# rrahn/libspm

Measured on AMD Instinct MI355X. Metric: Gbases/s scanned, Myers k<=3 |P|=100, higher is better.
Workload: dtype u32

## Files before the change

### include/spm_hip.h

```cpp
#ifndef SPM_HIP_H
#define SPM_HIP_H

#include <stddef.h>
#include <stdint.h>

#ifdef __cplusplus
extern "C" {
#endif

typedef struct spm_ctx spm_ctx;
typedef struct spm_text spm_text;
typedef struct spm_patterns spm_patterns;
typedef struct spm_hits spm_hits;
typedef struct spm_jst spm_jst;
typedef struct spm_jst_hits spm_jst_hits;

enum spm_status {
    SPM_OK = 0,
    SPM_E_INVALID = -1,
    SPM_E_HIP = -2,
    SPM_E_NOMEM = -3,
    SPM_E_UNSUPPORTED = -4,
    SPM_E_OVERFLOW = -5,
    SPM_E_PEER = -6
};

enum spm_algo {
    SPM_ALGO_SHIFTOR = 0,
    SPM_ALGO_MYERS = 1,
    SPM_ALGO_MYERS_PREFIX = 2,
    SPM_ALGO_HORSPOOL = 3
};

enum spm_engine {
    SPM_ENGINE_AUTO = 0,
    SPM_ENGINE_BRUTE = 1,
    SPM_ENGINE_FILTER = 2
};

#define SPM_MAX_NEEDLE 2048u

typedef struct spm_hit {
    uint64_t pos;
    uint32_t pattern;
    int32_t score;
} spm_hit;

typedef struct spm_scan_opts {
    uint32_t engine;
    uint32_t left_context;
    uint64_t pos_offset;
    uint64_t max_hits;
    uint32_t flags;
    uint32_t reserved;
} spm_scan_opts;

#define SPM_SCAN_IGNORE_PACKED 1u
#define SPM_SCAN_DEFER 2u
#define SPM_SCAN_ALIGNABLE 4u

typedef struct spm_scan_stats {
    float ms_total;
    float ms_main;
    float ms_verify;
    uint32_t engine_used;
    uint32_t fell_back;
    uint64_t n_candidates;
    uint64_t n_hits;
    uint32_t main_launches;
    uint32_t n_bands;
    uint32_t fallback_spans;
    uint32_t span_symbols;
    uint64_t fallback_symbols;
} spm_scan_stats;

int spm_hip_init(int device, void *stream, spm_ctx **out);
void spm_hip_destroy(spm_ctx *ctx);
const char *spm_hip_last_error(const spm_ctx *ctx);
int spm_hip_synchronize(spm_ctx *ctx);

int spm_hip_text_upload(spm_ctx *ctx, const uint8_t *ranks, uint64_t n, uint32_t sigma, spm_text **out);
int spm_hip_text_wrap(spm_ctx *ctx, const void *device_ranks, uint64_t n, uint32_t sigma, spm_text **out);
int spm_hip_text_generate(spm_ctx *ctx, uint64_t seed, uint64_t global_begin, uint64_t n, spm_text **out);
int spm_hip_text_generate_repeats(spm_ctx *ctx, uint64_t seed, uint64_t global_begin, uint64_t n, uint32_t repeat_ppm,
                                  spm_text **out);
int spm_hip_text_pack(spm_ctx *ctx, spm_text *text);
int spm_hip_text_is_packed(const spm_text *text);
int spm_hip_text_download(spm_ctx *ctx, const spm_text *text, uint64_t begin, uint64_t n, uint8_t *out);
uint64_t spm_hip_text_length(const spm_text *text);
const void *spm_hip_text_device_ptr(const spm_text *text);
void spm_hip_text_destroy(spm_text *text);

int spm_hip_patterns_create(spm_ctx *ctx, int algo, const uint8_t *ranks_concat, const uint32_t *offsets,
                            uint32_t n_patterns, const uint16_t *k, uint32_t sigma, spm_patterns **out);
void spm_hip_patterns_destroy(spm_patterns *p);
uint64_t spm_hip_patterns_window_size(const spm_patterns *p, uint32_t pattern);
int spm_hip_patterns_filterable(const spm_patterns *p);

int spm_hip_patterns_create_stranded(spm_ctx *ctx, int algo, const uint8_t *ranks_concat, const uint32_t *offsets,
                                     uint32_t n_reads, const uint16_t *k, uint32_t sigma, spm_patterns **out);
uint32_t spm_hip_patterns_strands(const spm_patterns *p);
uint32_t spm_hip_patterns_count(const spm_patterns *p);
int spm_hip_patterns_needle(const spm_patterns *p, uint32_t pattern, uint8_t *out, uint32_t cap, uint32_t *len);

typedef struct spm_build_stats {
    float ms_total;
    float ms_tables;
    float ms_index;
    float ms_upload;
    uint32_t threads;
    uint32_t passes;
    uint32_t dense;
    uint32_t anchor_sixteenths;
    uint64_t keys;
    uint32_t stride, key_len;
    uint64_t bytes_device;
} spm_build_stats;
int spm_hip_patterns_build_stats(const spm_patterns *p, spm_build_stats *out);

size_t spm_hip_patterns_state_stride(const spm_patterns *p);
int spm_hip_patterns_state_init(const spm_patterns *p, void *state);

int spm_hip_scan(spm_ctx *ctx, const spm_text *text, uint64_t begin, uint64_t end, const spm_patterns *patterns,
                 const spm_scan_opts *opts, const void *state_in, void *state_out, spm_hits **out);

int spm_hip_scan_segments(spm_ctx *ctx, const spm_text *text, const uint64_t *seg_offsets, uint64_t n_segments,
                          const spm_patterns *patterns, const spm_scan_opts *opts, spm_hits **out);

int spm_hip_hits_view(spm_hits *hits, const spm_hit **records, uint64_t *n);
int spm_hip_hits_device(spm_hits *hits, const void **device_records, uint64_t *n);
int spm_hip_hits_copy_device(spm_hits *hits, void *device_dst, uint64_t cap, uint64_t *n);
int spm_hip_hits_copy_fused(spm_hits *hits, void *device_dst, uint64_t cap, uint64_t *n);
int spm_hip_hits_copy_fused_device(spm_hits *hits, void *device_dst, uint64_t cap);
int spm_hip_hits_stats(const spm_hits *hits, spm_scan_stats *out);
uint64_t spm_hip_hits_checksum(spm_hits *hits);
void spm_hip_hits_destroy(spm_hits *hits);

typedef struct spm_aln {
    uint64_t begin;
    uint64_t end;
    uint32_t pattern;
    int32_t score;
    uint32_t cigar_off;
    uint32_t cigar_len;
} spm_aln;
typedef struct spm_alns spm_alns;

enum spm_cigar_op { SPM_CIGAR_INS = 1, SPM_CIGAR_DEL = 2, SPM_CIGAR_EQ = 7, SPM_CIGAR_X = 8 };
#define SPM_ALIGN_BEGIN_ONLY 1u

typedef struct spm_align_stats {
    float ms_total;
    float ms_begin;
    float ms_cigar;
    float ms_host;
    uint64_t n_alns;
    uint64_t n_ops;
    uint32_t begin_lane;
    uint32_t begin_wave;
    uint32_t cigar_lane;
    uint32_t cigar_wave;
    uint32_t cigar_wave_global;
    uint32_t reserved[3];
} spm_align_stats;

int spm_hip_hits_align(spm_hits *hits, uint32_t flags, spm_alns **out);
int spm_hip_alns_view(spm_alns *a, const spm_aln **records, uint64_t *n, const uint32_t **ops, uint64_t *n_ops);
int spm_hip_alns_device(spm_alns *a, const void **records, uint64_t *n, const void **ops, uint64_t *n_ops);
int spm_hip_alns_stats(const spm_alns *a, spm_align_stats *out);
void spm_hip_alns_destroy(spm_alns *a);

#define SPM_SELECT_LOCI 1u
#define SPM_SELECT_BEST 2u
#define SPM_SELECT_STRANDS 8u
#define SPM_SELECT_WINDOW_K 0xFFFFFFFFu
typedef struct spm_select_opts {
    uint32_t flags;
    uint32_t window;
    uint32_t strata;
    uint32_t reserved;
} spm_select_opts;
typedef struct spm_select_stats {
    float ms_total;
    float ms_order;
    float ms_select;
    float ms_host;
    uint64_t n_in;
    uint64_t n_loci;
    uint64_t n_out;
    uint32_t key_bits;
    uint32_t reserved;
} spm_select_stats;
int spm_hip_hits_select(spm_hits *hits, const spm_select_opts *opts, spm_hits **out);
int spm_hip_records_select(spm_ctx *ctx, const void *device_records, uint64_t n, const spm_patterns *patterns,
                           const spm_select_opts *opts, spm_hits **out);
int spm_hip_hits_select_stats(const spm_hits *hits, spm_select_stats *out);

typedef struct spm_jst_allele {
    uint64_t pos;
    uint32_t ref_len;
    uint32_t alt_len;
    uint64_t alt_off;
} spm_jst_allele;

typedef struct spm_jst_hit {
    uint64_t pos;
    uint32_t haplotype;
    uint32_t pattern;
    int32_t score;
    uint32_t reserved;
} spm_jst_hit;

typedef struct spm_jst_stats {
    uint64_t haplotype_symbols;
    uint64_t context_symbols;
    uint64_t contexts;
    uint64_t unique_contexts;
    uint64_t n_blocks;
    uint32_t block_len;
    uint32_t window;
    float ms_index;
    float ms_scan;
    float ms_main;
    float ms_verify;
    float ms_fanout;
    uint32_t engine_used;
    uint32_t main_launches;
    uint32_t fell_back;
    uint64_t segment_hits;
    uint64_t candidates;
    uint64_t bands;
} spm_jst_stats;

int spm_hip_jst_create(spm_ctx *ctx, const spm_text *reference, const spm_jst_allele *alleles, uint64_t n_alleles,
                       const uint8_t *alt_pool, uint64_t alt_pool_len, const uint64_t *coverage,
                       uint32_t n_haplotypes, spm_jst **out);
void spm_hip_jst_destroy(spm_jst *jst);
uint64_t spm_hip_jst_haplotype_length(const spm_jst *jst, uint32_t haplotype);
int spm_hip_jst_extract(spm_jst *jst, uint32_t haplotype, uint64_t begin, uint64_t n, uint8_t *out);
int spm_hip_jst_index(spm_jst *jst, uint32_t window, uint32_t block_len, uint64_t block_begin, uint64_t block_end);
int spm_hip_jst_search(spm_jst *jst, const spm_patterns *patterns, const spm_scan_opts *opts, spm_jst_hits **out);
int spm_hip_jst_stats(const spm_jst *jst, spm_jst_stats *out);
int spm_hip_jst_hits_view(spm_jst_hits *hits, const spm_jst_hit **records, uint64_t *n);
int spm_hip_jst_hits_device(spm_jst_hits *hits, const void **device_records, uint64_t *n);
int spm_hip_jst_hits_copy_device(spm_jst_hits *hits, void *device_dst, uint64_t cap, uint64_t *n);
void spm_hip_jst_hits_destroy(spm_jst_hits *hits);

typedef struct spm_jst_aln {
    uint64_t begin;
    uint64_t end;
    uint32_t haplotype;
    uint32_t pattern;
    int32_t score;
    uint32_t cigar_off;
    uint32_t cigar_len;
    uint32_t reserved;
} spm_jst_aln;
typedef struct spm_jst_alns spm_jst_alns;

typedef struct spm_jst_align_stats {
    float ms_total;
    float ms_begin;
    float ms_cigar;
    float ms_fanout;
    float ms_host;
    float ms_worklist;
    uint64_t n_alns;
    uint64_t n_segment_alns;
    uint64_t n_ops;
    uint32_t begin_lane, begin_wave, cigar_lane, cigar_wave, cigar_wave_global;
    uint32_t reserved[3];
} spm_jst_align_stats;

int spm_hip_jst_hits_align(spm_jst_hits *hits, uint32_t flags, spm_jst_alns **out);
int spm_hip_jst_alns_view(spm_jst_alns *a, const spm_jst_aln **records, uint64_t *n, const uint32_t **ops, uint64_t *n_ops);
int spm_hip_jst_alns_device(spm_jst_alns *a, const void **records, uint64_t *n, const void **ops, uint64_t *n_ops);
int spm_hip_jst_alns_stats(const spm_jst_alns *a, spm_jst_align_stats *out);
void spm_hip_jst_alns_destroy(spm_jst_alns *a);

int spm_hip_jst_selection_align(spm_jst_hits *selection, uint32_t flags, spm_jst_alns **out);

typedef struct spm_jst_ref_aln {
    uint64_t ref_begin;
    uint64_t ref_end;
    uint32_t haplotype;
    uint32_t pattern;
    int32_t score;
// ... 183 lines not shown
```

### libspm_amd/capi.py

```python
from __future__ import annotations

import ctypes as C
import os
import subprocess

_PKG = os.path.dirname(os.path.abspath(__file__))
SO_PATH = os.path.join(_PKG, "libspm_hip.so")
CSRC = os.path.join(_PKG, "csrc")

ALGO_SHIFTOR, ALGO_MYERS, ALGO_MYERS_PREFIX, ALGO_HORSPOOL = 0, 1, 2, 3
ENGINE_AUTO, ENGINE_BRUTE, ENGINE_FILTER = 0, 1, 2
SCAN_IGNORE_PACKED = 1
SCAN_DEFER = 2
SCAN_ALIGNABLE = 4
MAX_NEEDLE = 2048


class SpmError(RuntimeError):
    pass


class Hit(C.Structure):
    _fields_ = [("pos", C.c_uint64), ("pattern", C.c_uint32), ("score", C.c_int32)]

# ... 163 lines not shown
        ("n_members", C.c_uint64),
        ("n_ops", C.c_uint64),
        ("n_multi_slot", C.c_uint64),
        ("max_run", C.c_uint64),
    ]


class JstRead(C.Structure):
    _fields_ = [("first_locus", C.c_uint32), ("n_loci", C.c_uint32), ("n_forward", C.c_uint32), ("primary", C.c_uint32),
                ("best", C.c_int32), ("best_ref_score", C.c_int32), ("n_best", C.c_uint32), ("n_next", C.c_uint32)]


class JstReadsStats(C.Structure):
    _fields_ = [
        ("ms_total", C.c_float),
        ("ms_host", C.c_float),
        ("n_reads", C.c_uint64),
        ("n_loci", C.c_uint64),
        ("n_mapped", C.c_uint64),
        ("n_unique", C.c_uint64),
        ("n_multi", C.c_uint64),
    ]


class JstPairOpts(C.Structure):
    _fields_ = [("min_tlen", C.c_uint32), ("max_tlen", C.c_uint32), ("flags", C.c_uint32), ("reserved", C.c_uint32)]


class JstPair(C.Structure):
    _fields_ = [("locus1", C.c_uint32), ("locus2", C.c_uint32), ("tlen", C.c_int32), ("best", C.c_int32),
                ("n_pairs", C.c_uint32), ("n_best", C.c_uint32), ("n_next", C.c_uint32), ("flag1", C.c_uint16), ("flag2", C.c_uint16)]


class JstPairsStats(C.Structure):
    _fields_ = [
        ("ms_total", C.c_float),
        ("ms_host", C.c_float),
        ("n_pairs", C.c_uint64),
        ("n_proper", C.c_uint64),
        ("n_unique", C.c_uint64),
        ("n_multi", C.c_uint64),
        ("n_discordant", C.c_uint64),
        ("n_one_mate", C.c_uint64),
        ("n_unmapped", C.c_uint64),
        ("max_window", C.c_uint64),
    ]


class JstNormalizeStats(C.Structure):
    _fields_ = [
        ("ms_total", C.c_float),
        ("ms_slots", C.c_float),
        ("ms_normalize", C.c_float),
        ("ms_offsets", C.c_float),
        ("ms_gather", C.c_float),
        ("ms_compact", C.c_float),
        ("ms_host", C.c_float),
        ("reserved", C.c_float),
        ("n_alns", C.c_uint64),
        ("n_slots", C.c_uint64),
        ("n_ops_in", C.c_uint64),
        ("n_ops", C.c_uint64),
        ("n_changed", C.c_uint64),
        ("n_steps", C.c_uint64),
        ("n_joined", C.c_uint64),
        ("n_pinned", C.c_uint64),
    ]


ALIGN_BEGIN_ONLY = 1


class SelectOpts(C.Structure):
    _fields_ = [("flags", C.c_uint32), ("window", C.c_uint32), ("strata", C.c_uint32), ("reserved", C.c_uint32)]


class SelectStats(C.Structure):
    _fields_ = [
        ("ms_total", C.c_float),
        ("ms_order", C.c_float),
        ("ms_select", C.c_float),
        ("ms_host", C.c_float),
        ("n_in", C.c_uint64),
        ("n_loci", C.c_uint64),
        ("n_out", C.c_uint64),
        ("key_bits", C.c_uint32),
        ("reserved", C.c_uint32),
    ]


SELECT_LOCI, SELECT_BEST = 1, 2
SELECT_ACROSS = 4
SELECT_STRANDS = 8
SELECT_WINDOW_K = 0xFFFFFFFF
CIGAR_INS, CIGAR_DEL, CIGAR_EQ, CIGAR_X = 1, 2, 7, 8


def build(force: bool = False) -> str:
    srcs = [os.path.join(CSRC, f) for f in os.listdir(CSRC) if f.endswith((".hip", ".hpp", ".cpp"))]
    srcs.append(os.path.join(_PKG, "..", "include", "spm_hip.h"))
    stale = not os.path.exists(SO_PATH) or any(os.path.getmtime(s) > os.path.getmtime(SO_PATH) for s in srcs)
    if force or stale:
        subprocess.check_call(["make", "-C", CSRC, "-s"])
    return SO_PATH


_lib = None


def lib():
    global _lib
    if _lib is not None:
        return _lib
    if not os.path.exists(SO_PATH):
        raise SpmError(f"{SO_PATH} is missing: run `python -c 'import __graft_entry__ as g; g.build()'` "
                       "(hipcc --offload-arch=gfx950). libspm_amd has no CPU fallback.")
    L = C.CDLL(SO_PATH)
    vp, u8p, u32p, u16p = C.c_void_p, C.POINTER(C.c_uint8), C.POINTER(C.c_uint32), C.POINTER(C.c_uint16)
    sig = {
        "spm_hip_init": (C.c_int, [C.c_int, vp, C.POINTER(vp)]),
        "spm_hip_destroy": (None, [vp]),
        "spm_hip_last_error": (C.c_char_p, [vp]),
        "spm_hip_synchronize": (C.c_int, [vp]),
        "spm_hip_text_upload": (C.c_int, [vp, u8p, C.c_uint64, C.c_uint32, C.POINTER(vp)]),
        "spm_hip_text_wrap": (C.c_int, [vp, vp, C.c_uint64, C.c_uint32, C.POINTER(vp)]),
        "spm_hip_text_generate": (C.c_int, [vp, C.c_uint64, C.c_uint64, C.c_uint64, C.POINTER(vp)]),
        "spm_hip_text_generate_repeats": (C.c_int, [vp, C.c_uint64, C.c_uint64, C.c_uint64, C.c_uint32, C.POINTER(vp)]),
        "spm_hip_text_pack": (C.c_int, [vp, vp]),
        "spm_hip_text_is_packed": (C.c_int, [vp]),
        "spm_hip_text_download": (C.c_int, [vp, vp, C.c_uint64, C.c_uint64, u8p]),
        "spm_hip_text_length": (C.c_uint64, [vp]),
        "spm_hip_text_device_ptr": (vp, [vp]),
        "spm_hip_text_destroy": (None, [vp]),
        "spm_hip_patterns_create": (C.c_int, [vp, C.c_int, u8p, u32p, C.c_uint32, u16p, C.c_uint32, C.POINTER(vp)]),
        "spm_hip_patterns_create_stranded": (C.c_int, [vp, C.c_int, u8p, u32p, C.c_uint32, u16p, C.c_uint32, C.POINTER(vp)]),
        "spm_hip_patterns_strands": (C.c_uint32, [vp]),
        "spm_hip_patterns_count": (C.c_uint32, [vp]),
        "spm_hip_patterns_needle": (C.c_int, [vp, C.c_uint32, u8p, C.c_uint32, u32p]),
        "spm_hip_patterns_destroy": (None, [vp]),
        "spm_hip_patterns_window_size": (C.c_uint64, [vp, C.c_uint32]),
        "spm_hip_patterns_filterable": (C.c_int, [vp]),
        "spm_hip_patterns_build_stats": (C.c_int, [vp, C.POINTER(BuildStats)]),
        "spm_hip_patterns_state_stride": (C.c_size_t, [vp]),
        "spm_hip_patterns_state_init": (C.c_int, [vp, vp]),
        "spm_hip_scan": (C.c_int, [vp, vp, C.c_uint64, C.c_uint64, vp, C.POINTER(ScanOpts), vp, vp, C.POINTER(vp)]),
        "spm_hip_scan_segments": (C.c_int, [vp, vp, C.POINTER(C.c_uint64), C.c_uint64, vp, C.POINTER(ScanOpts),
                                            C.POINTER(vp)]),
        "spm_hip_hits_view": (C.c_int, [vp, C.POINTER(C.POINTER(Hit)), C.POINTER(C.c_uint64)]),
        "spm_hip_hits_device": (C.c_int, [vp, C.POINTER(vp), C.POINTER(C.c_uint64)]),
        "spm_hip_hits_copy_device": (C.c_int, [vp, vp, C.c_uint64, C.POINTER(C.c_uint64)]),
        "spm_hip_hits_copy_fused": (C.c_int, [vp, vp, C.c_uint64, C.POINTER(C.c_uint64)]),
        "spm_hip_hits_copy_fused_device": (C.c_int, [vp, vp, C.c_uint64]),
        "spm_hip_hits_stats": (C.c_int, [vp, C.POINTER(ScanStats)]),
        "spm_hip_hits_checksum": (C.c_uint64, [vp]),
        "spm_hip_hits_destroy": (None, [vp]),
        "spm_hip_hits_align": (C.c_int, [vp, C.c_uint32, C.POINTER(vp)]),
        "spm_hip_alns_view": (C.c_int, [vp, C.POINTER(C.POINTER(Aln)), C.POINTER(C.c_uint64), C.POINTER(u32p),
                                        C.POINTER(C.c_uint64)]),
        "spm_hip_alns_device": (C.c_int, [vp, C.POINTER(vp), C.POINTER(C.c_uint64), C.POINTER(vp), C.POINTER(C.c_uint64)]),
        "spm_hip_alns_stats": (C.c_int, [vp, C.POINTER(AlignStats)]),
        "spm_hip_alns_destroy": (None, [vp]),
        "spm_hip_hits_select": (C.c_int, [vp, C.POINTER(SelectOpts), C.POINTER(vp)]),
        "spm_hip_records_select": (C.c_int, [vp, vp, C.c_uint64, vp, C.POINTER(SelectOpts), C.POINTER(vp)]),
        "spm_hip_hits_select_stats": (C.c_int, [vp, C.POINTER(SelectStats)]),
        "spm_hip_synth_pattern": (C.c_uint64, [C.c_uint64, C.c_uint64, C.c_uint64, C.c_uint32, C.c_uint32,
                                               C.c_uint32, u8p]),
        "spm_hip_synth_repeat_pattern": (C.c_uint64, [C.c_uint64, C.c_uint64, C.c_uint64, C.c_uint32, C.c_uint32,
                                                      C.c_uint32, C.c_uint32, C.c_uint32, u8p]),
        "spm_hip_synth_repeat_text": (None, [C.c_uint64, C.c_uint32, C.c_uint64, C.c_uint64, u8p]),
        "spm_hip_mix64": (C.c_uint64, [C.c_uint64]),
        "spm_hip_host_selftest": (C.c_int, [C.c_int, u8p, u32p, C.c_uint32, u16p, C.c_uint32, C.POINTER(C.c_uint64)]),
        "spm_hip_version": (C.c_char_p, []),
        "spm_hip_jst_create": (C.c_int, [vp, vp, C.POINTER(JstAllele), C.c_uint64, u8p, C.c_uint64,
                                         C.POINTER(C.c_uint64), C.c_uint32, C.POINTER(vp)]),
        "spm_hip_jst_destroy": (None, [vp]),
        "spm_hip_jst_haplotype_length": (C.c_uint64, [vp, C.c_uint32]),
        "spm_hip_jst_extract": (C.c_int, [vp, C.c_uint32, C.c_uint64, C.c_uint64, u8p]),
        "spm_hip_jst_index": (C.c_int, [vp, C.c_uint32, C.c_uint32, C.c_uint64, C.c_uint64]),
        "spm_hip_jst_search": (C.c_int, [vp, vp, C.POINTER(ScanOpts), C.POINTER(vp)]),
        "spm_hip_jst_stats": (C.c_int, [vp, C.POINTER(JstStats)]),
        "spm_hip_jst_hits_view": (C.c_int, [vp, C.POINTER(C.POINTER(JstHit)), C.POINTER(C.c_uint64)]),
        "spm_hip_jst_hits_device": (C.c_int, [vp, C.POINTER(vp), C.POINTER(C.c_uint64)]),
        "spm_hip_jst_hits_copy_device": (C.c_int, [vp, vp, C.c_uint64, C.POINTER(C.c_uint64)]),
        "spm_hip_jst_hits_destroy": (None, [vp]),
        "spm_hip_jst_hits_align": (C.c_int, [vp, C.c_uint32, C.POINTER(vp)]),
        "spm_hip_jst_selection_align": (C.c_int, [vp, C.c_uint32, C.POINTER(vp)]),
        "spm_hip_jst_alns_view": (C.c_int, [vp, C.POINTER(C.POINTER(JstAln)), C.POINTER(C.c_uint64), C.POINTER(u32p),
                                            C.POINTER(C.c_uint64)]),
        "spm_hip_jst_alns_device": (C.c_int, [vp, C.POINTER(vp), C.POINTER(C.c_uint64), C.POINTER(vp),
                                              C.POINTER(C.c_uint64)]),
        "spm_hip_jst_alns_stats": (C.c_int, [vp, C.POINTER(JstAlignStats)]),
        "spm_hip_jst_alns_destroy": (None, [vp]),
        "spm_hip_jst_alns_project": (C.c_int, [vp, C.c_uint32, C.POINTER(vp)]),
        "spm_hip_jst_ref_alns_view": (C.c_int, [vp, C.POINTER(C.POINTER(JstRefAln)), C.POINTER(C.c_uint64), C.POINTER(u32p),
                                                C.POINTER(C.c_uint64)]),
        "spm_hip_jst_ref_alns_device": (C.c_int, [vp, C.POINTER(vp), C.POINTER(C.c_uint64), C.POINTER(vp),
                                                  C.POINTER(C.c_uint64)]),
        "spm_hip_jst_ref_alns_stats": (C.c_int, [vp, C.POINTER(JstProjectStats)]),
        "spm_hip_jst_ref_alns_destroy": (None, [vp]),
        "spm_hip_jst_ref_alns_normalize": (C.c_int, [vp, C.c_uint32, C.POINTER(vp)]),
        "spm_hip_jst_ref_alns_normalize_stats": (C.c_int, [vp, C.POINTER(JstNormalizeStats)]),
        "spm_hip_jst_ref_alns_collapse": (C.c_int, [vp, C.c_uint32, C.POINTER(vp)]),
        "spm_hip_jst_ref_loci_view": (C.c_int, [vp, C.POINTER(C.POINTER(JstRefLocus)), C.POINTER(C.c_uint64), C.POINTER(u32p),
                                                C.POINTER(C.c_uint64), C.POINTER(u32p), C.POINTER(C.POINTER(C.c_int32)),
                                                C.POINTER(C.c_uint64)]),
        "spm_hip_jst_ref_loci_device": (C.c_int, [vp, C.POINTER(vp), C.POINTER(C.c_uint64), C.POINTER(vp),
                                                  C.POINTER(C.c_uint64), C.POINTER(vp), C.POINTER(vp), C.POINTER(C.c_uint64)]),
        "spm_hip_jst_ref_loci_map": (C.c_int, [vp, C.POINTER(u32p), C.POINTER(vp), C.POINTER(C.c_uint64)]),
        "spm_hip_jst_ref_loci_stats": (C.c_int, [vp, C.POINTER(JstCollapseStats)]),
        "spm_hip_jst_ref_loci_destroy": (None, [vp]),
        "spm_hip_jst_ref_loci_reads": (C.c_int, [vp, C.c_uint32, C.c_uint32, C.c_uint32, C.POINTER(vp)]),
        "spm_hip_jst_reads_view": (C.c_int, [vp, C.POINTER(C.POINTER(JstRead)), C.POINTER(C.c_uint64)]),
        "spm_hip_jst_reads_device": (C.c_int, [vp, C.POINTER(vp), C.POINTER(C.c_uint64)]),
        "spm_hip_jst_reads_stats": (C.c_int, [vp, C.POINTER(JstReadsStats)]),
        "spm_hip_jst_reads_destroy": (None, [vp]),
        "spm_hip_jst_ref_loci_pairs": (C.c_int, [vp, vp, C.POINTER(JstPairOpts), C.POINTER(vp)]),
        "spm_hip_jst_pairs_view": (C.c_int, [vp, C.POINTER(C.POINTER(JstPair)), C.POINTER(C.c_uint64)]),
        "spm_hip_jst_pairs_device": (C.c_int, [vp, C.POINTER(vp), C.POINTER(C.c_uint64)]),
        "spm_hip_jst_pairs_stats": (C.c_int, [vp, C.POINTER(JstPairsStats)]),
        "spm_hip_jst_pairs_destroy": (None, [vp]),
        "spm_hip_jst_hits_select": (C.c_int, [vp, C.POINTER(SelectOpts), C.POINTER(vp)]),
        "spm_hip_jst_records_select": (C.c_int, [vp, vp, C.c_uint64, vp, C.POINTER(SelectOpts), C.POINTER(vp)]),
        "spm_hip_jst_hits_select_stats": (C.c_int, [vp, C.POINTER(SelectStats)]),
        "spm_hip_comm_unique_id": (C.c_int, [vp]),
        "spm_hip_comm_init": (C.c_int, [vp, vp, C.c_int, C.c_int, C.POINTER(vp)]),
        "spm_hip_comm_destroy": (None, [vp]),
        "spm_hip_gatherv_hits": (C.c_int, [vp, vp, C.c_int, C.POINTER(vp), C.POINTER(C.c_uint64), C.POINTER(C.c_uint64)]),
        "spm_hip_gatherv_jst_hits": (C.c_int, [vp, vp, C.c_int, C.POINTER(vp), C.POINTER(C.c_uint64),
                                               C.POINTER(C.c_uint64)]),
        "spm_hip_gatherv_plan": (C.c_int, [C.POINTER(C.c_uint64), C.c_uint32, C.c_uint32, C.POINTER(C.c_uint64)]),
        "spm_hip_comm_selftest": (C.c_int, [C.c_int, C.c_int, C.c_int, C.c_int, C.c_uint32, C.c_uint64, C.POINTER(C.c_int)]),
        "spm_hip_jst_synth_variants": (C.c_int, [C.c_uint64, C.c_uint64, C.c_uint64, C.c_uint64, C.c_uint32,
                                                 C.POINTER(JstAllele), C.POINTER(C.c_uint64), u8p,
                                                 C.POINTER(C.c_uint64), C.POINTER(C.c_uint64)]),
    }
    for name, (res, args) in sig.items():
        fn = getattr(L, name)
        fn.restype = res
        fn.argtypes = args
    _lib = L
    return L


EXPORTS = [
    "spm_hip_init", "spm_hip_destroy", "spm_hip_last_error", "spm_hip_synchronize", "spm_hip_text_upload",
    "spm_hip_text_wrap", "spm_hip_text_generate", "spm_hip_text_generate_repeats", "spm_hip_text_pack", "spm_hip_text_is_packed",
    "spm_hip_text_download", "spm_hip_text_length",
    "spm_hip_text_device_ptr", "spm_hip_text_destroy", "spm_hip_patterns_create", "spm_hip_patterns_destroy",
    "spm_hip_patterns_create_stranded", "spm_hip_patterns_strands", "spm_hip_patterns_count", "spm_hip_patterns_needle",
    "spm_hip_patterns_window_size", "spm_hip_patterns_filterable", "spm_hip_patterns_build_stats", "spm_hip_patterns_state_stride",
    "spm_hip_patterns_state_init", "spm_hip_scan", "spm_hip_scan_segments", "spm_hip_hits_view", "spm_hip_hits_device",
    "spm_hip_hits_copy_device", "spm_hip_hits_copy_fused", "spm_hip_hits_copy_fused_device", "spm_hip_hits_stats", "spm_hip_hits_checksum", "spm_hip_hits_destroy",
    "spm_hip_hits_align", "spm_hip_alns_view", "spm_hip_alns_device", "spm_hip_alns_stats", "spm_hip_alns_destroy",
    "spm_hip_hits_select", "spm_hip_records_select", "spm_hip_hits_select_stats",
    "spm_hip_synth_pattern",
    "spm_hip_synth_repeat_pattern", "spm_hip_synth_repeat_text", "spm_hip_mix64", "spm_hip_host_selftest", "spm_hip_version",
    "spm_hip_jst_create", "spm_hip_jst_destroy", "spm_hip_jst_haplotype_length", "spm_hip_jst_extract",
    "spm_hip_jst_index", "spm_hip_jst_search", "spm_hip_jst_stats", "spm_hip_jst_hits_view", "spm_hip_jst_hits_device",
    "spm_hip_jst_hits_copy_device", "spm_hip_jst_hits_destroy", "spm_hip_jst_synth_variants",
    "spm_hip_jst_hits_align", "spm_hip_jst_selection_align", "spm_hip_jst_alns_view", "spm_hip_jst_alns_device", "spm_hip_jst_alns_stats",
    "spm_hip_jst_alns_destroy",
    "spm_hip_jst_alns_project", "spm_hip_jst_ref_alns_view", "spm_hip_jst_ref_alns_device", "spm_hip_jst_ref_alns_stats",
    "spm_hip_jst_ref_alns_destroy",
    "spm_hip_jst_ref_alns_normalize", "spm_hip_jst_ref_alns_normalize_stats",
    "spm_hip_jst_ref_alns_collapse", "spm_hip_jst_ref_loci_view", "spm_hip_jst_ref_loci_device", "spm_hip_jst_ref_loci_map",
    "spm_hip_jst_ref_loci_stats", "spm_hip_jst_ref_loci_destroy",
    "spm_hip_jst_ref_loci_reads", "spm_hip_jst_reads_view", "spm_hip_jst_reads_device", "spm_hip_jst_reads_stats",
    "spm_hip_jst_reads_destroy",
    "spm_hip_jst_ref_loci_pairs", "spm_hip_jst_pairs_view", "spm_hip_jst_pairs_device", "spm_hip_jst_pairs_stats",
    "spm_hip_jst_pairs_destroy",
    "spm_hip_jst_hits_select", "spm_hip_jst_records_select", "spm_hip_jst_hits_select_stats",
    "spm_hip_comm_unique_id", "spm_hip_comm_init", "spm_hip_comm_destroy", "spm_hip_gatherv_hits",
    "spm_hip_gatherv_jst_hits", "spm_hip_gatherv_plan", "spm_hip_comm_selftest",
]
```

### libspm_amd/csrc/common.hpp

```cpp
#pragma once

#include <hip/hip_runtime.h>

#include <algorithm>
#include <cstdint>
#include <functional>
#include <cstdio>
#include <string>
#include <utility>
#include <vector>

#include "../../include/spm_hip.h"
#include "scan_plan.hpp"

namespace spm_hip
{

constexpr int kWave = 64;

__device__ __forceinline__ uint64_t uniform_u64(uint64_t v)
{
    return ((uint64_t)(uint32_t)__builtin_amdgcn_readfirstlane((uint32_t)(v >> 32)) << 32) |
           (uint32_t)__builtin_amdgcn_readfirstlane((uint32_t)v);
}

struct error_sink
{
    std::string msg;
};

extern thread_local std::string g_init_error;

}

struct hits_block
{
    spm_hit *d_hits = nullptr;
    unsigned long long *d_count = nullptr;
    uint64_t cap = 0;
    hipEvent_t ev[4] = {nullptr, nullptr, nullptr, nullptr};
    bool zeroed = false;
    unsigned long long *h_c = nullptr;
    hipEvent_t ev_done = nullptr;
};

struct spm_ctx
{
    int device = 0;
    hipStream_t stream = nullptr;
    bool own_stream = false;
    int n_cu = 256;
    std::string err;
    void *d_scratch = nullptr;
    size_t scratch_bytes = 0;
    std::vector<hits_block> pool;
    std::vector<std::pair<void *, uint64_t>> jst_pool;
    ulonglong2 *d_band_tab = nullptr;
    uint64_t band_slots = 0;
    bool band_dirty = false;
    uint32_t *d_table_poison = nullptr;
    uint8_t *h_stage = nullptr;
    size_t stage_half = 0;
    hipEvent_t stage_ev[2] = {nullptr, nullptr};
    unsigned long long *h_counters = nullptr;
};

struct spm_text
{
    spm_ctx *ctx = nullptr;
    uint8_t *d = nullptr;
    uint64_t n = 0;
    uint64_t alloc = 0;
    uint32_t sigma = 4;
    bool owned = false;
    uint32_t *d_packed = nullptr;
    uint64_t packed_words = 0;
};

struct spm_hits : hits_block
{
    spm_ctx *ctx = nullptr;
    uint64_t cand_cap = 0;
    uint64_t band_cap = 0;
    uint64_t n = 0;
    bool counted = false;
    bool hook_final = false;
    unsigned long long fan_count = 0;
    bool sorted_host = false;
    std::vector<spm_hit> host;
    spm_scan_stats stats{};
    bool timed = false;
    void *d_aux[2] = {nullptr, nullptr};
    bool pending = false;
    bool c_on_the_way = false;
    bool d_count_cleared = false;
    const spm_text *d_text = nullptr;
    const struct spm_patterns *d_patterns = nullptr;
    uint64_t d_begin = 0, d_end = 0;
    spm_scan_opts d_opts{};
    const spm_text *al_text = nullptr;
    const struct spm_patterns *al_patterns = nullptr;
    uint64_t al_lo = 0;
    uint64_t al_pos_offset = 0;
    bool al_stateful = false;
    bool al_device_segs = false;
    std::vector<uint64_t> al_segs;
    bool selected = false;
    bool sel_records = false;
    bool sel_timed = false;
    uint64_t sel_n_patterns = 0, sel_bias = 0, sel_max_rel = 0;
    spm_select_stats sel{};
};

struct spm_jst_hits
{
    spm_ctx *ctx = nullptr;
    spm_jst_hit *d = nullptr;
    uint64_t cap = 0;
    uint64_t n = 0;
    bool sorted = false;
    std::vector<spm_jst_hit> host;
    bool alignable = false;
    spm_jst *jst = nullptr;
    const struct spm_patterns *patterns = nullptr;
    uint32_t pat_strands = 0;
    uint64_t generation = 0;
    spm_hits *seg = nullptr;
    uint64_t sel_n_hap = 1, sel_n_patterns = 1, sel_max_pos = 0;
    bool selected = false;
    bool sel_timed = false;
    hipEvent_t sel_ev[3] = {nullptr, nullptr, nullptr};
    spm_select_stats sel{};
};

inline void hits_adopt(spm_hits &h, spm_hits &from)
{
    std::swap(static_cast<hits_block &>(h), static_cast<hits_block &>(from));
    std::swap(h.h_c, from.h_c);
    std::swap(h.ev_done, from.ev_done);
    std::swap(h.d_aux, from.d_aux);
    from.d_count_cleared = h.d_count_cleared;
    h.d_count_cleared = false;
    h.n = from.n;
    h.counted = from.counted;
    h.stats = from.stats;
    h.cand_cap = from.cand_cap;
    h.band_cap = from.band_cap;
    h.timed = from.timed;
    h.sorted_host = false;
    h.host.clear();
}

#define SPM_TRY(call)                                                                                                  \
    do {                                                                                                               \
        const int _rc = (call);                                                                                        \
        if (_rc != SPM_OK)                                                                                             \
            return _rc;                                                                                                \
    } while (0)

struct pass_entry
{
    const uint4 *ht;
    uint32_t ht_mask;
    uint32_t pad;
};

struct dev_scratch
{
    std::vector<void *> owned;
    template <typename T>
    hipError_t alloc(T **p, size_t bytes)
    {
        const hipError_t e = hipMalloc(reinterpret_cast<void **>(p), bytes);
        if (e == hipSuccess)
            owned.push_back(*p);
        return e;
    }
    ~dev_scratch()
    {
        for (void *p : owned)
            hipFree(p);
    }
};

#define SPM_SET_ERR(ctx, ...)                                                                                          \
    do {                                                                                                               \
        char _b[512];                                                                                                  \
        snprintf(_b, sizeof(_b), __VA_ARGS__);                                                                         \
        if (ctx)                                                                                                       \
            (ctx)->err = _b;                                                                                           \
        else                                                                                                           \
            spm_hip::g_init_error = _b;                                                                                \
    } while (0)

#define SPM_HIP_CHECK(ctx, call)                                                                                       \
    do {                                                                                                               \
        hipError_t _e = (call);                                                                                        \
        if (_e != hipSuccess) {                                                                                        \
            SPM_SET_ERR(ctx, "%s failed: %s (%s:%d)", #call, hipGetErrorString(_e), __FILE__, __LINE__);               \
            return SPM_E_HIP;                                                                                          \
        }                                                                                                              \
    } while (0)
```

### libspm_amd/csrc/filter.hpp

```cpp
#pragma once

#include "brute.hpp"
#include "common.hpp"
#include "filter_shared.hpp"
#include "pack.hpp"
#include "hd.hpp"

namespace spm_hip
{

struct survivor
{
    uint32_t key;
    uint32_t t_lo, t_hi;
    uint32_t pad;
};
constexpr uint32_t kSurvInvalid = 0xFFFFFFFFu;

struct band_rec
{
    uint32_t slot;
    uint32_t val;
    uint32_t seg;
    uint32_t band;
};
constexpr uint32_t kBandInvalid = 0xFFFFFFFFu;
constexpr unsigned long long kBandEmpty = ~0ull;

constexpr uint32_t kChunkMax = 1024;
constexpr uint32_t kCandLdsSlot = 4;
constexpr uint32_t kCandRec = 8;

struct filter_params
{
    const uint8_t *text;
    uint64_t text_alloc;
    uint64_t lo, hi;
    uint32_t stride;
    uint32_t bitmap_words;
    uint32_t n_probes;
    uint32_t span_chunks;
    uint32_t span_unit;
    uint32_t dynamic;
    uint32_t key_len;
    uint32_t key_mask;
    uint32_t hash_variant;
    uint32_t lds_words;
    uint32_t chd_slot_mask;
    uint32_t chd_bucket_shift;
    uint32_t chd_disp_off;
    const uint32_t *bitmap;
    uint32_t span_budget;
    uint32_t pass;
    uint32_t anchor_c, anchor_cm;
    uint32_t n_pat, pat_c[kDensePatterns], pat_cm[kDensePatterns];
    uint32_t bucket_shift;
    const uint4 *buckets;
    survivor *surv;
    unsigned long long *counters;
    uint64_t surv_cap;
    uint64_t *ovf_spans;
    uint64_t ovf_cap;
};

__device__ __forceinline__ void wave_count_add(unsigned long long *counter, uint32_t v)
{
    for (int o = 32; o > 0; o >>= 1)
        v += __shfl_xor(v, o);
    if ((threadIdx.x & 63) == 0 && v)
        atomicAdd(counter, (unsigned long long)v);
}

__device__ __forceinline__ void queue_sync()
{
    __builtin_amdgcn_fence(__ATOMIC_RELEASE, "wavefront");
    __builtin_amdgcn_wave_barrier();
}

__device__ __forceinline__ uint32_t chunk_grow(uint32_t size, uint32_t n)
{
    const uint32_t next = size * 2 < kChunkMin ? kChunkMin : (size * 2 > kChunkMax ? kChunkMax : size * 2);
    return next < n ? n : next;
}

__device__ __forceinline__ uint32_t *cand_chunk_of(const filter_params &P, const uint32_t *lds)
{
    const uint32_t wave = (uint32_t)__builtin_amdgcn_readfirstlane(threadIdx.x >> 6);
    return const_cast<uint32_t *>(lds) + P.lds_words + kCandLdsSlot + kCandRec * wave;
}

__device__ __forceinline__ void span_open(const filter_params &P, const uint32_t *lds, uint32_t lane, uint64_t begin)
{
    if (lane == 0) {
        uint32_t *ck = cand_chunk_of(P, lds);
        ck[4] = 0;
        ck[5] = 0;
        ck[6] = (uint32_t)begin;
        ck[7] = (uint32_t)(begin >> 32);
    }
}

__device__ __forceinline__ void span_give_up(const filter_params &P, uint32_t *ck, uint32_t lane)
{
    if (lane == 0) {
        ck[5] = 1;
        const unsigned long long i = atomicAdd(&P.counters[kCntSpansGaveUp], 1ull);
        if (i < P.ovf_cap) {
            P.ovf_spans[2 * i] = ((uint64_t)ck[7] << 32) | ck[6];
            P.ovf_spans[2 * i + 1] = (uint64_t)P.span_chunks * (uint64_t)P.span_unit;
        } else {
            atomicAdd(&P.counters[kCntVoid], 1ull);
        }
    }
    queue_sync();
}

__device__ __forceinline__ void surv_close(const filter_params &P, const uint32_t *ck, uint32_t lane)
{
    const uint32_t used = ck[2], size = ck[3];
    const uint64_t base = ((uint64_t)ck[1] << 32) | ck[0];
    for (uint32_t i = used + lane; i < size; i += 64)
        if (base + i < P.surv_cap) {
            survivor sv;
            sv.key = 0;
            sv.t_lo = 0;
            sv.t_hi = kSurvInvalid;
            sv.pad = 0;
            P.surv[base + i] = sv;
        }
}

__device__ __forceinline__ void emit_survivors(const filter_params &P, bool has, uint32_t key, uint64_t t, uint32_t lane,
                                               const uint32_t *lds)
{
    const uint64_t m = __ballot(has);
    if (m == 0)
        return;
    uint32_t *ck = cand_chunk_of(P, lds);
    const uint32_t n = __popcll(m);
    uint32_t used = (uint32_t)__builtin_amdgcn_readfirstlane(ck[2]);
    const uint32_t size = (uint32_t)__builtin_amdgcn_readfirstlane(ck[3]);
    const uint32_t cnt = (uint32_t)__builtin_amdgcn_readfirstlane(ck[4]) + n;
    if (cnt > P.span_budget) {
        span_give_up(P, ck, lane);
        return;
    }
    if (used + n > size) {
        surv_close(P, ck, lane);
        const uint32_t next = chunk_grow(size, n);
        if (lane == 0) {
            const unsigned long long b = atomicAdd(&P.counters[kCntSurvSlots], (unsigned long long)next);
            ck[0] = (uint32_t)b;
            ck[1] = (uint32_t)(b >> 32);
            ck[2] = 0;
            ck[3] = next;
        }
        used = 0;
        queue_sync();
    }
    const uint64_t cbase = uniform_u64(((uint64_t)ck[1] << 32) | ck[0]);
    if (cbase + used + n > P.surv_cap) {
        span_give_up(P, ck, lane);
        return;
    }
    if (has) {
        survivor sv;
        sv.key = key;
        sv.t_lo = (uint32_t)t;
        sv.t_hi = (uint32_t)(t >> 32);
        sv.pad = P.pass;
        P.surv[cbase + used + __popcll(m & ((1ull << lane) - 1))] = sv;
    }
    if (lane == 0) {
        ck[2] = used + n;
        ck[4] = cnt;
    }
    queue_sync();
}

template <int S, int NWD, int HV, int SIG, bool PK, bool KM>
__device__ __forceinline__ void filter_words(const filter_params &P, const uint32_t (&w)[NWD],
                                             const uint32_t (&prev)[NWD], const uint32_t (&nv)[SIG != 4 ? NWD : 1],
                                             uint64_t gbase, uint32_t lane, const uint32_t *lds, uint32_t idx_mask)
{
    constexpr int NWIN = 16 / S;
    const uint32_t kmask = KM ? P.key_mask : 0xFFFFFFFFu;
    static_assert(NWD * NWIN <= 32, "one mask bit per window of a group");
    uint32_t pos_mask = 0;
    if constexpr (HV == 2) {
        const uint16_t *fp_tab = reinterpret_cast<const uint16_t *>(lds);
        const uint16_t *disp_tab = reinterpret_cast<const uint16_t *>(reinterpret_cast<const uint8_t *>(lds) + P.chd_disp_off);
        uint32_t xs[NWD * NWIN], ds[NWD * NWIN];
#pragma unroll
        for (int u = 0; u < NWD; ++u) {
#pragma unroll
            for (int i = 0; i < NWIN; ++i) {
                const int d = S * (i + 1);
                const uint32_t key = (d == 16 ? w[u] : alignbit(w[u], prev[u], (2 * d) & 31)) & kmask;
                const uint32_t x = chd_hash(key).x;
                xs[u * NWIN + i] = x;
                ds[u * NWIN + i] = disp_tab[x >> P.chd_bucket_shift];
            }
        }
#pragma unroll
        for (int u = 0; u < NWD; ++u) {
#pragma unroll
            for (int i = 0; i < NWIN; ++i) {
                const int d = S * (i + 1);
                const uint32_t key = (d == 16 ? w[u] : alignbit(w[u], prev[u], (2 * d) & 31)) & kmask;
                const uint32_t slot = ((xs[u * NWIN + i] >> 3) + ds[u * NWIN + i] * ((key | 1u) & 0xFFFFFFu)) &
                                      P.chd_slot_mask;
                ds[u * NWIN + i] = fp_tab[slot];
            }
        }
#pragma unroll
        for (int u = 0; u < NWD; ++u) {
#pragma unroll
// ... 84 lines not shown

__device__ __forceinline__ uint32_t anchor_select(uint32_t w, uint32_t prev, uint32_t c, uint32_t cm)
{
    const uint32_t C0 = (c & 3u) * 0x55555555u, M0 = (cm & 3u) * 0x55555555u;
    const uint32_t C1 = (c >> 2) * 0x55555555u, M1 = (cm >> 2) * 0x55555555u;
    const uint32_t X = alignbit(w, prev, 2);
    const uint32_t Y = alignbit(w, prev, 4);
    uint32_t t = ((X ^ C0) & M0) | ((Y ^ C1) & M1);
    t |= t >> 1;
    return ~t & 0x55555555u;
}

template <int NWD>
__device__ __forceinline__ void filter_words_anchored(const filter_params &P, const uint32_t (&w)[NWD], const uint32_t (&prev)[NWD],
                                                      uint64_t gbase, uint32_t lane, const uint32_t *lds)
{
    static_assert(NWD % 2 == 0 || NWD == 1, "words are taken in pairs");
    const uint16_t *fp_tab = reinterpret_cast<const uint16_t *>(lds);
    const uint16_t *disp_tab = reinterpret_cast<const uint16_t *>(reinterpret_cast<const uint8_t *>(lds) + P.chd_disp_off);
#pragma unroll
    for (int j = 0; j < NWD; j += 2) {
        uint32_t todo = anchor_select(w[j], prev[j], P.anchor_c, P.anchor_cm);
        if (j + 1 < NWD)
            todo |= anchor_select(w[j + 1 < NWD ? j + 1 : j], prev[j + 1 < NWD ? j + 1 : j], P.anchor_c, P.anchor_cm) << 1;
        while (__ballot(todo != 0) != 0) {
            const bool act = todo != 0;
            const uint32_t b = act ? (uint32_t)__ffs(todo) - 1u : 0u;
            todo &= todo - 1;
            const uint32_t u = b & 1u, d = (b >> 1) + 1u;
            const uint32_t wu = (j + 1 < NWD && u) ? w[j + 1 < NWD ? j + 1 : j] : w[j];
            const uint32_t pu = (j + 1 < NWD && u) ? prev[j + 1 < NWD ? j + 1 : j] : prev[j];
            const uint32_t key = (uint32_t)((((uint64_t)wu << 32) | pu) >> (2 * d));
            const uint32_t x = chd_hash(key).x;
            const uint32_t dsp = disp_tab[x >> P.chd_bucket_shift];
            const uint32_t slot = ((x >> 3) + dsp * ((key | 1u) & 0xFFFFFFu)) & P.chd_slot_mask;
            const uint32_t f = fp_tab[slot];
            const bool hit = act && ((f ^ key ^ (key >> 16)) & 0xFFFFu) == 0;
            if (__ballot(hit) != 0) {
                if (__builtin_amdgcn_readfirstlane(cand_chunk_of(P, lds)[5]) != 0)
                    return;
                const uint64_t wpos = gbase + (uint64_t)(j + u) * 1024 + (uint64_t)lane * 16;
                const int64_t ts = (int64_t)wpos - 16 + (int64_t)d;
                const bool has = hit && ts >= (int64_t)P.lo && (uint64_t)ts + P.key_len <= P.hi;
                emit_survivors(P, has, key, has ? (uint64_t)ts : 0, lane, lds);
            }
        }
    }
}


__device__ __forceinline__ void stream_stage(const filter_params &P, uint32_t *lds)
{
    for (uint32_t i = threadIdx.x; i < P.lds_words; i += blockDim.x)
        lds[i] = P.bitmap[i];
    if ((threadIdx.x & 63) == 0) {
        uint32_t *ck = lds + P.lds_words + kCandLdsSlot + kCandRec * (threadIdx.x >> 6);
        for (uint32_t i = 0; i < kCandRec; ++i)
            ck[i] = 0;
    }
    __syncthreads();
}

enum class span_draw
{
    run,
    idle,
    done,
};

__device__ __forceinline__ span_draw draw_span(const filter_params &P, uint32_t *lds, uint32_t lane, uint32_t wave_in_wg,
                                               uint32_t waves_per_wg, uint64_t n_spans, uint64_t &sp)
{
    if (P.dynamic == 1) {
        unsigned long long t = 0;
        if (lane == 0)
            t = atomicAdd(&P.counters[kCntSpanHead], 1ull);
        sp = uniform_u64(t);
        return sp >= n_spans ? span_draw::done : span_draw::run;
    }
    __syncthreads();
    if (threadIdx.x == 0) {
        const unsigned long long t = atomicAdd(&P.counters[kCntSpanHead], (unsigned long long)waves_per_wg);
        lds[P.lds_words] = (uint32_t)t;
        lds[P.lds_words + 1] = (uint32_t)(t >> 32);
    }
    __syncthreads();
    const uint64_t base = uniform_u64(((uint64_t)lds[P.lds_words + 1] << 32) | lds[P.lds_words]);
    if (base >= n_spans)
        return span_draw::done;
    sp = base + wave_in_wg;
    return sp >= n_spans ? span_draw::idle : span_draw::run;
}

template <int SIG>
__device__ __forceinline__ uint32_t span_carry_in(const filter_params &P, uint64_t span_base, uint32_t lane, uint32_t &carry_n)
{
    uint32_t carry_in = 0;
    carry_n = 0;
    if (span_base >= 16 && lane == 0) {
        const uint4 before = load_text16(P.text, span_base - 16, P.hi);
        carry_in = pack16_sig<SIG>(before, carry_n);
    }
    carry_n = __builtin_amdgcn_readfirstlane(carry_n);
    return __builtin_amdgcn_readfirstlane(carry_in);
}

__device__ __forceinline__ uint32_t span_carry_in(const filter_params &P, uint64_t span_base, uint32_t lane)
{
    uint32_t no_n;
    return span_carry_in<4>(P, span_base, lane, no_n);
}

__device__ __forceinline__ void pack_with_prev(const uint4 &cur, uint32_t lane, uint32_t &carry_in, uint32_t &w, uint32_t &prev)
{
    w = pack16(cur);
    prev = __builtin_amdgcn_update_dpp(0u, w, 0x138 , 0xF, 0xF, false);
    if (lane == 0)
        prev = carry_in;
    carry_in = __builtin_amdgcn_readlane(w, 63);
}

template <int S, int UU, int HV, int SIG, bool KM, bool AN = false>
__device__ __forceinline__ void filter_group(const filter_params &P, const uint4 (&cur)[UU], uint64_t gbase,
                                             uint32_t &carry_in, uint32_t &carry_n, uint32_t lane,
                                             const uint32_t *lds, uint32_t idx_mask)
{
    uint32_t w[UU], prev[UU];
    uint32_t nv[SIG != 4 ? UU : 1];
#pragma unroll
    for (int u = 0; u < UU; ++u) {
        if constexpr (SIG == 4) {
            pack_with_prev(cur[u], lane, carry_in, w[u], prev[u]);
        } else {
            uint32_t nm = 0;
            w[u] = pack16_sig<SIG>(cur[u], nm);
            prev[u] = __builtin_amdgcn_update_dpp(0u, w[u], 0x138 , 0xF, 0xF, false);
            if (lane == 0)
                prev[u] = carry_in;
            carry_in = __builtin_amdgcn_readlane(w[u], 63);
            uint32_t np = __builtin_amdgcn_update_dpp(0u, nm, 0x138, 0xF, 0xF, false);
            if (lane == 0)
                np = carry_n;
            carry_n = __builtin_amdgcn_readlane(nm, 63);
            nv[u] = (nm << 16) | np;
        }
    }
    if constexpr (AN)
        filter_words_anchored<UU>(P, w, prev, gbase, lane, lds);
    else
        filter_words<S, UU, HV, SIG, false, KM>(P, w, prev, nv, gbase, lane, lds, idx_mask);
}

template <int S, int U, int HV, int SIG, bool KM, bool AN = false>
__global__ __launch_bounds__(((S == 1 && !KM && SIG == 4) || (S == 2 && U == 2)) ? 1024 : 512) void seed_filter_kernel(const filter_params P)
{
    extern __shared__ uint32_t lds[];
    stream_stage(P, lds);

    const uint32_t lane = threadIdx.x & 63;
    const uint32_t waves_per_wg = blockDim.x >> 6;
    const uint32_t wave_in_wg = (uint32_t)__builtin_amdgcn_readfirstlane(threadIdx.x >> 6);
    const uint32_t idx_mask = P.bitmap_words * 32 - 1;

    const stream_geometry G = stream_geometry_of(P.lo, P.hi, 1024, P.span_chunks);
    const uint64_t span = P.span_chunks;
    const uint8_t *lane_text = P.text + G.base0 + (uint64_t)lane * 16;

    uint64_t sp;
    for (;;) {
        const span_draw drawn = draw_span(P, lds, lane, wave_in_wg, waves_per_wg, G.n_spans, sp);
        if (drawn == span_draw::done)
            break;
        if (drawn == span_draw::idle)
            continue;
        const uint64_t c_begin = sp * span;
        const uint64_t c_end = c_begin + span < G.n_chunks ? c_begin + span : G.n_chunks;
        span_open(P, lds, lane, G.base0 + c_begin * 1024);
        uint32_t carry_n;
        uint32_t carry_in = span_carry_in<SIG>(P, G.base0 + c_begin * 1024, lane, carry_n);
        uint64_t ch = c_begin;
        const uint64_t whole_end = c_end < G.n_whole ? c_end : G.n_whole;
        const uint64_t fast_end = c_begin + (whole_end > c_begin ? (whole_end - c_begin) / U * U : 0);
        if (ch < fast_end) {
            uint4 nxt[U];
#pragma unroll
            for (int u = 0; u < U; ++u)
                nxt[u] = load16_stream(lane_text + (ch + u) * 1024);
            for (; ch < fast_end; ch += U) {
                uint4 cur[U];
#pragma unroll
                for (int u = 0; u < U; ++u)
                    cur[u] = nxt[u];
                const bool more = ch + U < fast_end;
                const uint64_t pf = more ? ch + U : ch;
                const uint64_t ustride = more ? 1024 : 0;
#pragma unroll
                for (int u = 0; u < U; ++u)
                    nxt[u] = load16_stream(lane_text + pf * 1024 + (uint64_t)u * ustride);
                if constexpr (S <= 2)
                    __builtin_amdgcn_sched_barrier(0);
                filter_group<S, U, HV, SIG, KM, AN>(P, cur, G.base0 + ch * 1024, carry_in, carry_n, lane, lds, idx_mask);
            }
        }
        for (; ch < c_end; ++ch) {
            uint4 one[1];
            one[0] = load_text16(P.text, (G.base0 + ch * 1024) | ((uint64_t)lane * 16), P.hi);
            filter_group<S, 1, HV, SIG, KM, AN>(P, one, G.base0 + ch * 1024, carry_in, carry_n, lane, lds, idx_mask);
        }
    }
    surv_close(P, cand_chunk_of(P, lds), lane);
}

constexpr uint32_t kDenseQueueCap = 192;
constexpr int kDenseBatches = 3;

template <int NP>
__device__ __forceinline__ uint32_t dense_select(const filter_params &P, uint32_t w, uint32_t prev)
{
    const uint32_t X = alignbit(w, prev, 2);
    const uint32_t Y = alignbit(w, prev, 4);
    uint32_t sel = 0;
#pragma unroll
    for (int i = 0; i < NP; ++i) {
        const uint32_t C0 = (P.pat_c[i] & 3u) * 0x55555555u, M0 = (P.pat_cm[i] & 3u) * 0x55555555u;
        const uint32_t C1 = (P.pat_c[i] >> 2) * 0x55555555u, M1 = (P.pat_cm[i] >> 2) * 0x55555555u;
        uint32_t t = ((X ^ C0) & M0) | ((Y ^ C1) & M1);
        t |= t >> 1;
        sel |= ~t;
    }
    return sel & 0x55555555u;
}

struct dense_queue
{
    uint32_t key[kDenseQueueCap];
    uint32_t off[kDenseQueueCap];
};

__device__ __forceinline__ void dense_drain(const filter_params &P, dense_queue &Q, uint32_t &qn, bool all, uint64_t span_base,
                                            uint32_t lane, const uint32_t *lds)
{
    while (qn >= 64 || (all && qn != 0)) {
        const uint32_t nb_full = qn >> 6;
        uint32_t nb = all ? (qn + 63) >> 6 : nb_full;
        nb = nb > (uint32_t)kDenseBatches ? (uint32_t)kDenseBatches : nb;
        uint32_t key[kDenseBatches], off[kDenseBatches];
        uint4 bk[kDenseBatches];
        bool v[kDenseBatches];
#pragma unroll
        for (int b = 0; b < kDenseBatches; ++b) {
            const int32_t e = (int32_t)qn - 64 * b - 1 - (int32_t)lane;
            v[b] = (uint32_t)b < nb && e >= 0;
            key[b] = 0;
            off[b] = 0;
            bk[b] = make_uint4(0, 0, 0, 0);
            if (v[b]) {
                key[b] = Q.key[e];
                off[b] = Q.off[e];
                bk[b] = P.buckets[dense_bucket(key[b], P.bucket_shift)];
            }
        }
        qn = qn > 64 * nb ? qn - 64 * nb : 0;
#pragma unroll
        for (int b = 0; b < kDenseBatches; ++b) {
            if ((uint32_t)b >= nb)
                break;
            const uint32_t f2 = dense_fp(key[b]) * 0x00010001u;
            const uint32_t x0 = bk[b].x ^ f2, x1 = bk[b].y ^ f2, x2 = bk[b].z ^ f2, x3 = bk[b].w ^ f2;
            const uint32_t z = ((x0 - 0x00010001u) & ~x0) | ((x1 - 0x00010001u) & ~x1) | ((x2 - 0x00010001u) & ~x2) |
                               ((x3 - 0x00010001u) & ~x3);
            const bool hit = v[b] && ((z & 0x80008000u) != 0 || (bk[b].w >> 16) == kDenseAcceptAll);
            if (__ballot(hit) != 0) {
                if (__builtin_amdgcn_readfirstlane(cand_chunk_of(P, lds)[5]) == 0) {
                    const int64_t ts = (int64_t)span_base + (int64_t)off[b] - 16;
                    const bool has = hit && ts >= (int64_t)P.lo && (uint64_t)ts + P.key_len <= P.hi;
                    emit_survivors(P, has, key[b], has ? (uint64_t)ts : 0, lane, lds);
                }
            }
        }
    }
}

template <int UU, int NP, int S, bool KM>
__device__ __forceinline__ void dense_group(const filter_params &P, const uint4 (&cur)[UU], uint64_t gbase, uint64_t span_base,
                                            uint32_t &carry_in, uint32_t lane, const uint32_t *lds, dense_queue &Q, uint32_t &qn)
{
    static_assert(UU % 2 == 0 || UU == 1, "words are taken in pairs");
    uint32_t w[UU], prev[UU];
#pragma unroll
    for (int u = 0; u < UU; ++u)
        pack_with_prev(cur[u], lane, carry_in, w[u], prev[u]);
    const uint32_t goff = (uint32_t)(gbase - span_base) + lane * 16;
#pragma unroll
    for (int j = 0; j < UU; j += 2) {
        constexpr bool pair = UU > 1;
        const uint32_t w0 = w[j], p0 = prev[j], w1 = w[pair ? j + 1 : j], p1 = prev[pair ? j + 1 : j];
        const uint32_t kmask = KM ? P.key_mask : 0xFFFFFFFFu;
        static_assert(kDenseBloomBits == 20, "the word address below takes bits 5..19 of the index");
        uint32_t pm = 0;
        if constexpr (S == 0) {
            uint32_t todo = dense_select<NP>(P, w0, p0);
            if (pair)
                todo |= dense_select<NP>(P, w1, p1) << 1;
            while (todo != 0) {
                const uint32_t b = (uint32_t)__ffs(todo) - 1u;
                todo &= todo - 1;
                const bool odd = (b & 1u) != 0;
                const uint64_t both = ((uint64_t)(odd ? w1 : w0) << 32) | (odd ? p1 : p0);
                const uint32_t key = (uint32_t)(both >> ((b & ~1u) + 2u));
                const uint32_t h = key ^ (key >> 13);
                const uint32_t word = *reinterpret_cast<const uint32_t *>(reinterpret_cast<const uint8_t *>(lds) + ((h >> 3) & 0x1FFFCu));
                pm |= __builtin_amdgcn_ubfe(word, h, 1) << b;
            }
        } else {
#pragma unroll
            for (int u = 0; u < (pair ? 2 : 1); ++u) {
#pragma unroll
                for (int d = S; d <= 16; d += S) {
                    const uint32_t wu = u ? w1 : w0, pu = u ? p1 : p0;
                    const uint32_t key = (d == 16 ? wu : alignbit(wu, pu, (2 * d) & 31)) & kmask;
                    const uint32_t h = key ^ (key >> 13);
                    const uint32_t word = *reinterpret_cast<const uint32_t *>(reinterpret_cast<const uint8_t *>(lds) + ((h >> 3) & 0x1FFFCu));
                    pm |= __builtin_amdgcn_ubfe(word, h, 1) << (2 * (d - 1) + u);
                }
            }
        }
        while (__ballot(pm != 0) != 0) {
            const bool pos = pm != 0;
            const uint32_t b = pos ? (uint32_t)__ffs(pm) - 1u : 0u;
            pm &= pm - 1;
            const bool odd = (b & 1u) != 0;
            const uint64_t both = ((uint64_t)(odd ? w1 : w0) << 32) | (odd ? p1 : p0);
            const uint32_t key = (uint32_t)(both >> ((b & ~1u) + 2u)) & kmask;
            const uint64_t mm = __ballot(pos);
            if (pos) {
                const uint32_t q = qn + __popcll(mm & ((1ull << lane) - 1));
                Q.key[q] = key;
                Q.off[q] = goff + (uint32_t)j * 1024u + (odd ? 1024u : 0u) + (b >> 1) + 1u;
            }
            qn += __popcll(mm);
            queue_sync();
            if (qn > kDenseQueueCap - 64)
                dense_drain(P, Q, qn, false, span_base, lane, lds);
        }
    }
}

template <int U, int NP, int S = 0, bool KM = false>
__global__ __launch_bounds__(1024) void seed_filter_dense_kernel(const filter_params P)
{
    extern __shared__ uint32_t lds[];
    stream_stage(P, lds);

    const uint32_t lane = threadIdx.x & 63;
    const uint32_t waves_per_wg = blockDim.x >> 6;
    const uint32_t wave_in_wg = (uint32_t)__builtin_amdgcn_readfirstlane(threadIdx.x >> 6);
    dense_queue &Q = *reinterpret_cast<dense_queue *>(lds + P.lds_words + kCandLdsSlot + kCandRec * 16 +
                                                      (sizeof(dense_queue) / 4) * wave_in_wg);
    uint32_t qn = 0;

    const stream_geometry G = stream_geometry_of(P.lo, P.hi, 1024, P.span_chunks);
// ... 8 lines not shown
        if (drawn == span_draw::idle)
            continue;
        const uint64_t c_begin = sp * span;
        const uint64_t c_end = c_begin + span < G.n_chunks ? c_begin + span : G.n_chunks;
        const uint64_t span_base = G.base0 + c_begin * 1024;
        span_open(P, lds, lane, span_base);
        uint32_t carry_in = span_carry_in(P, span_base, lane);
        uint64_t ch = c_begin;
        const uint64_t whole_end = c_end < G.n_whole ? c_end : G.n_whole;
        const uint64_t fast_end = c_begin + (whole_end > c_begin ? (whole_end - c_begin) / U * U : 0);
        if (ch < fast_end) {
            uint4 nxt[U];
#pragma unroll
            for (int u = 0; u < U; ++u)
                nxt[u] = load16_stream(lane_text + (ch + u) * 1024);
            for (; ch < fast_end; ch += U) {
                uint4 cur[U];
#pragma unroll
                for (int u = 0; u < U; ++u)
                    cur[u] = nxt[u];
                const bool more = ch + U < fast_end;
                const uint64_t pf = more ? ch + U : ch;
                const uint64_t ustride = more ? 1024 : 0;
#pragma unroll
                for (int u = 0; u < U; ++u)
                    nxt[u] = load16_stream(lane_text + pf * 1024 + (uint64_t)u * ustride);
                __builtin_amdgcn_sched_barrier(0);
                dense_group<U, NP, S, KM>(P, cur, G.base0 + ch * 1024, span_base, carry_in, lane, lds, Q, qn);
            }
        }
        for (; ch < c_end; ++ch) {
            uint4 one[1];
            one[0] = load_text16(P.text, G.base0 + ch * 1024 + (uint64_t)lane * 16, P.hi);
            dense_group<1, NP, S, KM>(P, one, G.base0 + ch * 1024, span_base, carry_in, lane, lds, Q, qn);
        }
        dense_drain(P, Q, qn, true, span_base, lane, lds);
    }
    surv_close(P, cand_chunk_of(P, lds), lane);
}

template <int S, int U2, int HV, bool KM>
__global__ __launch_bounds__(1024) void seed_filter_packed_kernel(const filter_params P, const uint4 *__restrict__ shadow)
{
    extern __shared__ uint32_t lds[];
    stream_stage(P, lds);

    constexpr int NWD = 4 * U2;
    const uint32_t lane = threadIdx.x & 63;
    const uint32_t waves_per_wg = blockDim.x >> 6;
    const uint32_t wave_in_wg = (uint32_t)__builtin_amdgcn_readfirstlane(threadIdx.x >> 6);
    const uint32_t idx_mask = P.bitmap_words * 32 - 1;

    const stream_geometry G = stream_geometry_of(P.lo, P.hi, 4096, P.span_chunks);
    const uint64_t span = P.span_chunks;
    const uint4 *lane_src = shadow + (G.base0 / 64) + lane;

    uint64_t sp;
    for (;;) {
        const span_draw drawn = draw_span(P, lds, lane, wave_in_wg, waves_per_wg, G.n_spans, sp);
        if (drawn == span_draw::done)
            break;
        if (drawn == span_draw::idle)
            continue;
        const uint64_t c_begin = sp * span;
        const uint64_t c_end = c_begin + span < G.n_chunks ? c_begin + span : G.n_chunks;
        const uint64_t fast_end = c_begin + (c_end - c_begin + U2 - 1) / U2 * U2;
        span_open(P, lds, lane, G.base0 + c_begin * 4096);
        uint32_t carry_in = 0;
        {
            const uint64_t first_word = (G.base0 + c_begin * 4096) / 16;
            if (first_word > 0 && lane == 0)
                carry_in = reinterpret_cast<const uint32_t *>(shadow)[first_word - 1];
            carry_in = __builtin_amdgcn_readfirstlane(carry_in);
        }
        uint4 nxt[U2];
#pragma unroll
        for (int u = 0; u < U2; ++u)
            nxt[u] = load16_stream(reinterpret_cast<const uint8_t *>(lane_src + (c_begin + u) * 64));
        for (uint64_t ch = c_begin; ch < fast_end; ch += U2) {
            uint4 cur[U2];
#pragma unroll
            for (int u = 0; u < U2; ++u)
                cur[u] = nxt[u];
            const bool more = ch + U2 < fast_end;
            const uint64_t pf = more ? ch + U2 : ch;
            const uint64_t ustride = more ? 64 : 0;
#pragma unroll
            for (int u = 0; u < U2; ++u)
                nxt[u] = load16_stream(reinterpret_cast<const uint8_t *>(lane_src + pf * 64 + (uint64_t)u * ustride));
            __builtin_amdgcn_sched_barrier(0);
            uint32_t w[NWD], prev[NWD];
            const uint32_t nv[1] = {0};
#pragma unroll
            for (int u = 0; u < U2; ++u) {
                w[4 * u + 0] = cur[u].x;
                w[4 * u + 1] = cur[u].y;
                w[4 * u + 2] = cur[u].z;
                w[4 * u + 3] = cur[u].w;
                uint32_t p0 = __builtin_amdgcn_update_dpp(0u, cur[u].w, 0x138 , 0xF, 0xF, false);
                if (lane == 0)
                    p0 = carry_in;
                carry_in = __builtin_amdgcn_readlane(cur[u].w, 63);
                prev[4 * u + 0] = p0;
                prev[4 * u + 1] = cur[u].x;
                prev[4 * u + 2] = cur[u].y;
                prev[4 * u + 3] = cur[u].z;
            }
            filter_words<S, NWD, HV, 4, true, KM>(P, w, prev, nv, G.base0 + ch * 4096, lane, lds, idx_mask);
        }
    }
    surv_close(P, cand_chunk_of(P, lds), lane);
}

struct verify_params
{
    const uint8_t *text;
    uint64_t text_alloc;
    uint64_t ctx_begin;
    uint64_t scan_begin;
    uint64_t scan_end;
    uint64_t pos_offset;
    const band_rec *bands;
    const unsigned long long *counters;
    uint32_t band_counter;
    uint32_t preselected;
    uint64_t band_cap;
    ulonglong2 *band_tab;
    uint32_t table_mask, band_bits;
    uint32_t runs;
    const uint8_t *surplus;
    uint32_t Bw;
    uint32_t overlap;
    uint32_t max_m;
    const uint32_t *peq32;
    uint32_t sigma;
    uint32_t nw_table;
    uint32_t max_k;
    const int32_t *m;
    const int32_t *k;
    uint32_t report_begin;
    uint32_t max_span;
    uint32_t wave_text;
    unsigned long long *seen;
    uint32_t seen_mask;
    spm_hit *hits;
    unsigned long long *hit_counter;
    uint64_t hit_cap;
    unsigned long long *overflow;
    const uint64_t *seg_offsets;
    uint64_t n_segments;
    const uint32_t *seg_owned;
};

struct resolve_params
{
    const survivor *surv;
    unsigned long long *counters;
    uint64_t surv_cap;
    const pass_entry *passes;
    const uint4 *entries;
    uint32_t key_len;
    uint32_t flank_check;
    uint32_t pieces_check;
    const uint8_t *text;
    uint64_t text_alloc;
    const uint8_t *needle_ranks;
    const uint32_t *needle_offsets;
    const uint16_t *seed_q;
    const int32_t *m, *k;
    uint64_t hay_begin, hay_end;
    const uint64_t *seg_offsets;
    uint64_t n_segments;
    uint32_t Bw, overlap, max_m;
    uint32_t band_bits;
    ulonglong2 *band_tab;
    uint32_t table_mask;
    band_rec *bands;
    uint64_t band_cap;
    const uint32_t *needle_pk;
    const uint32_t *pk_offsets;
    uint32_t exact_hits;
    uint32_t report_begin;
    uint64_t scan_begin, scan_end;
    uint64_t pos_offset;
    const uint32_t *seg_owned;
    unsigned long long *seen;
    uint32_t seen_mask;
    spm_hit *hits;
    unsigned long long *hit_counter, *overflow;
    uint64_t hit_cap;
    uint32_t *table_poison;
};

__device__ __forceinline__ unsigned long long band_value(unsigned long long stored, bool counting)
{
    return counting ? (unsigned long long)(uint32_t)(stored + 1ull) : ~stored;
}
__device__ __forceinline__ void band_release(ulonglong2 *tab, uint32_t slot)
{
    tab[slot] = make_ulonglong2(kBandEmpty, ~0ull);
}

__device__ __forceinline__ uint4 load_bytes16(const uint8_t *p)
{
    uint4 v;
    __builtin_memcpy(&v, p, 16);
    return v;
}

__device__ __forceinline__ uint4 load_bytes16_guarded(const uint8_t *base, uint64_t idx, uint64_t limit)
{
    if (idx + 16 <= limit)
        return load_bytes16(base + idx);
    uint32_t w[4] = {0xFFFFFFFFu, 0xFFFFFFFFu, 0xFFFFFFFFu, 0xFFFFFFFFu};
    for (int b = 0; b < 16; ++b)
        if (idx + b < limit)
            w[b >> 2] = (w[b >> 2] & ~(0xFFu << (8 * (b & 3)))) | ((uint32_t)base[idx + b] << (8 * (b & 3)));
    return make_uint4(w[0], w[1], w[2], w[3]);
}

__device__ __forceinline__ uint32_t diff16(const uint4 a, const uint4 b, uint32_t n)
{
    const uint32_t d[4] = {a.x ^ b.x, a.y ^ b.y, a.z ^ b.z, a.w ^ b.w};
    uint32_t r = 0;
#pragma unroll
    for (uint32_t i = 0; i < 4; ++i) {
        const uint32_t have = n > 4 * i ? n - 4 * i : 0;
        const uint32_t mask = have >= 4 ? 0xFFFFFFFFu : (have == 0 ? 0u : (1u << (8 * have)) - 1);
        r |= d[i] & mask;
    }
    return r;
}

__device__ __forceinline__ bool seed_intact(const resolve_params &P, uint64_t t, uint32_t val, uint32_t r, uint32_t q_whole,
                                            int64_t hay_b, int64_t hay_e)
{
    if (!P.needle_ranks)
        return true;
    const uint32_t pat = val >> 11, x = val & 0x7FF;
    struct
    {
        uint32_t q;
    } sp{q_whole ? q_whole : P.seed_q[pat]};
    const uint32_t o = x - r;
    const int64_t ts = (int64_t)t - (int64_t)r;
    if (ts < hay_b || ts + (int64_t)sp.q > hay_e)
        return false;
    const uint8_t *nd = P.needle_ranks + P.needle_offsets[pat] + o;
    for (uint32_t i = 0; i < sp.q; i += 16) {
        const uint32_t n = sp.q - i < 16 ? sp.q - i : 16;
        if (diff16(load_bytes16_guarded(P.text, (uint64_t)ts + i, P.text_alloc), load_bytes16(nd + i), n))
            return false;
    }
    return true;
}

constexpr uint32_t kPieceRoundsShift = 21, kPieceMissingShift = 28;

__device__ __forceinline__ bool pieces_apply(const resolve_params &P, uint64_t t, uint32_t val, uint32_t m, uint32_t k, int64_t hay_b,
                                             int64_t hay_e)
{
    if (!P.pieces_check || k == 0 || k > 7 || m < 32)
        return false;
    const int64_t d = (int64_t)t - (int64_t)(val & 0x7FF);
    return d - (int64_t)k >= hay_b && d + (int64_t)(m + k) <= hay_e;
}

__device__ __forceinline__ uint32_t pieces_visit(const resolve_params &P, uint64_t t, uint32_t val, uint32_t &rng, uint32_t m, uint32_t k)
{
    const uint32_t pat = val >> 11, x = val & 0x7FF;
    const uint32_t n_rounds = m >> 4;
    uint32_t done = (rng >> kPieceRoundsShift) & 0x7F, missing = (rng >> kPieceMissingShift) & 7;
    const bool ascending = 2 * x >= m;
    const uint32_t todo = n_rounds - done < 2 ? n_rounds - done : 2;
    const uint32_t r_lo = ascending ? done : n_rounds - done - todo;
    const uint32_t *pk = P.needle_pk + P.pk_offsets[pat] + r_lo;
    const uint32_t nw0 = pk[0], nw1 = todo == 2 ? pk[1] : 0;
    const uint64_t w0 = (uint64_t)((int64_t)t - (int64_t)x + (int64_t)(16 * r_lo) - (int64_t)k);
    const uint32_t c0 = pack16(load_bytes16_guarded(P.text, w0, P.text_alloc));
    const uint32_t c1 = pack16(load_bytes16_guarded(P.text, w0 + 16, P.text_alloc));
    const uint32_t c2 = todo == 2 ? pack16(load_bytes16_guarded(P.text, w0 + 32, P.text_alloc)) : 0;
#pragma unroll
    for (uint32_t rr = 0; rr < 2; ++rr) {
        if (rr < todo) {
            const uint32_t two = rr ? nw1 : nw0;
            const uint64_t win = rr ? ((uint64_t)c1 | ((uint64_t)c2 << 32)) : ((uint64_t)c0 | ((uint64_t)c1 << 32));
#pragma unroll
            for (uint32_t j = 0; j < 2; ++j) {
                const uint32_t piece = (two >> (16 * j)) & 0xFFFFu;
                bool found = false;
                for (uint32_t sh = 0; sh <= 2 * k; ++sh)
                    found = found || (((uint32_t)(win >> (2 * (8 * j + sh))) & 0xFFFFu) == piece);
                missing += found ? 0u : 1u;
            }
        }
    }
    if (missing > k)
        return 0;
    done += todo;
    if (done >= n_rounds)
        return 2;
    rng = (rng & ~((0x7Fu << kPieceRoundsShift) | (7u << kPieceMissingShift))) | (done << kPieceRoundsShift) |
          (missing << kPieceMissingShift);
    return 1;
}

struct text64
{
    uint64_t lo, hi;
    bool ok;
};

__device__ __forceinline__ uint32_t syms16(const text64 &W, uint32_t first)
{
    if (first >= 32)
        return (uint32_t)(W.hi >> (2 * (first - 32)));
    return (uint32_t)(W.lo >> (2 * first)) | (first ? (uint32_t)(W.hi << (2 * (32 - first)) ) : 0u);
}

__device__ __forceinline__ bool seed_sig_ok(const text64 &W, uint32_t sig, uint32_t r, uint32_t n, uint32_t H)
{
    if (n == 0)
        return true;
    const uint32_t rb = r < 16 ? r : 16;
    const uint32_t nl = rb < n ? rb : n;
    uint32_t got = nl ? syms16(W, 16 - rb) : 0u;
    if (nl < 16) {
        got &= (1u << (2 * nl)) - 1;
        got |= syms16(W, 16 + H) << (2 * nl);
    }
    const uint32_t mask = n >= 16 ? 0xFFFFFFFFu : ((1u << (2 * n)) - 1);
    return ((got ^ sig) & mask) == 0;
}

constexpr uint32_t kPairCap = 128;
struct pair_queue
{
    uint32_t t_lo[kPairCap], t_hi[kPairCap], val[kPairCap], rng[kPairCap], seg[kPairCap];
};
struct band_queue
{
    uint32_t key_lo[kPairCap], key_hi[kPairCap], run_lo[kPairCap], run_hi[kPairCap];
    uint32_t elect[128];
};

struct band_chunk
{
    uint64_t base;
    uint32_t used, size, draws;
};
constexpr uint32_t kDenseDraws = 4;

__device__ __forceinline__ void insert_bands(const resolve_params &R, band_queue &B, uint32_t first, uint32_t n,
                                             uint32_t lane, band_chunk &C)
{
    bool act = lane < n;
    unsigned long long bkey = 0, run = 0;
    if (act)
        bkey = ((unsigned long long)B.key_hi[first + lane] << 32) | B.key_lo[first + lane];
    if (!R.overlap) {
        const uint32_t h = (uint32_t)mix64(bkey) & 127u;
        if (act)
            B.elect[h] = lane;
        queue_sync();
        const uint32_t w = act ? B.elect[h] : lane;
        const unsigned long long wkey = ((unsigned long long)B.key_hi[first + w] << 32) | B.key_lo[first + w];
        const bool follower = act && w != lane && wkey == bkey;
        if (follower) {
            atomicOr(&B.run_lo[first + w], B.run_lo[first + lane]);
            atomicOr(&B.run_hi[first + w], B.run_hi[first + lane]);
            act = false;
        }
        queue_sync();
    }
    if (act)
        run = ((unsigned long long)B.run_hi[first + lane] << 32) | B.run_lo[first + lane];
    bool claimed = false;
    uint32_t s2 = (uint32_t)mix64(bkey) & R.table_mask;
    if (act) {
        bool placed = false;
        for (uint32_t tries = 0; tries < 8192 && !placed; ++tries) {
            if ((tries & 31u) == 31u && __hip_atomic_load(&R.counters[kCntVoid], __ATOMIC_RELAXED, __HIP_MEMORY_SCOPE_AGENT) != 0)
                break;
            const unsigned long long o = atomicCAS(&R.band_tab[s2].x, kBandEmpty, bkey);
            if (o == kBandEmpty) {
                claimed = true;
                placed = true;
            } else if (o == bkey) {
                placed = true;
            } else {
                s2 = (s2 + 1) & R.table_mask;
            }
        }
        if (!placed) {
            atomicAdd(&R.counters[kCntVoid], 1ull);
            *R.table_poison = 1u;
        }
        else if (R.overlap)
            atomicAdd(&R.band_tab[s2].y, 1ull);
        else
            atomicAnd(&R.band_tab[s2].y, ~run);
    }
    const uint64_t mm = __ballot(claimed);
    if (mm == 0)
        return;
    const uint32_t nn = __popcll(mm);
    if (C.used + nn > C.size) {
        for (uint32_t q = C.used + lane; q < C.size; q += 64)
            if (C.base + q < R.band_cap)
                R.bands[C.base + q].val = kBandInvalid;
        uint32_t next = chunk_grow(C.size, nn);
        if (C.draws < kDenseDraws) {
            next = nn;
            ++C.draws;
        }
        unsigned long long b = 0;
        if (lane == 0)
            b = atomicAdd(&R.counters[kCntBandSlots], (unsigned long long)next);
        C.base = uniform_u64(b);
        C.used = 0;
        C.size = next;
    }
    if (claimed) {
        const uint64_t idx = C.base + C.used + __popcll(mm & ((1ull << lane) - 1));
        if (idx < R.band_cap) {
            band_rec br;
            br.slot = s2;
            br.val = (uint32_t)(bkey >> 43) << 11;
            br.seg = (uint32_t)((bkey & ((1ull << 43) - 1)) >> R.band_bits);
            br.band = (uint32_t)(bkey & ((1ull << R.band_bits) - 1));
            R.bands[idx] = br;
        } else {
            atomicAdd(&R.counters[kCntVoid], 1ull);
            *R.table_poison = 1u;
        }
    }
    C.used += nn;
}

__device__ __forceinline__ unsigned long long wave_reserve_hits(unsigned long long *counter, uint32_t mine)
{
    const uint32_t lane = threadIdx.x & 63;
    uint32_t incl = mine;
#pragma unroll
    for (int o = 1; o < 64; o <<= 1) {
        const uint32_t up = (uint32_t)__shfl_up((int)incl, o);
        if (lane >= (uint32_t)o)
            incl += up;
    }
    const uint32_t total = (uint32_t)__shfl((int)incl, 63);
    unsigned long long base = 0;
    if (total != 0) {
        if (lane == 0)
            base = atomicAdd(counter, (unsigned long long)total);
        base = uniform_u64(base);
    }
    return base + (incl - mine);
}

__device__ __forceinline__ bool seen_insert_raw(unsigned long long *seen, uint32_t seen_mask, unsigned long long *overflow,
                                                uint32_t pat, int64_t e)
{
    const unsigned long long key = ((unsigned long long)pat << 40) | (unsigned long long)e;
    uint32_t slot = (uint32_t)(mix64(key)) & seen_mask;
    for (uint32_t tries = 0; tries < 64; ++tries) {
        if (tries == 4 && __hip_atomic_load(overflow, __ATOMIC_RELAXED, __HIP_MEMORY_SCOPE_AGENT) != 0)
            return false;
        const unsigned long long old = atomicCAS(&seen[slot], ~0ull, key);
        if (old == ~0ull)
            return true;
        if (old == key)
            return false;
        slot = (slot + 1) & seen_mask;
    }
    atomicAdd(overflow, 1ull);
    return false;
}

struct resolve_wave
{
    pair_queue *Q;
    band_queue *B;
    uint32_t qn, bn;
    band_chunk C;
    uint32_t n_cand;
};

__device__ __forceinline__ void check_pairs(const resolve_params &R, resolve_wave &S, uint32_t n, uint32_t lane)
{
    pair_queue &Q = *S.Q;
    band_queue &B = *S.B;
    S.qn -= n;
    const uint32_t first = S.qn;
    bool live = lane < n;
    uint64_t t = 0, seg = 0;
    uint32_t val = 0, rng = 0;
    int64_t sb = (int64_t)R.hay_begin, se = (int64_t)R.hay_end;
    if (live) {
        const uint32_t i = first + lane;
        t = ((uint64_t)Q.t_hi[i] << 32) | Q.t_lo[i];
        val = Q.val[i];
        rng = Q.rng[i];
        seg = Q.seg[i];
        if (R.seg_offsets) {
            sb = (int64_t)R.seg_offsets[seg];
            se = (int64_t)R.seg_offsets[seg + 1];
        }
    }
    queue_sync();
    bool through = live;
    const uint32_t pat = val >> 11;
    if (live && !(rng & kRngRun)) {
        if (!(rng & kSeedChecked)) {
            live = seed_intact(R, t, val, (rng >> 16) & 0x1F, (rng & kRngWhole) ? R.key_len + ((rng >> 5) & 0x1F) : 0u, sb, se);
            rng |= kSeedChecked;
        }
        through = live;
        if (live && R.pieces_check) {
            const uint32_t m = (uint32_t)R.m[pat], k = (uint32_t)R.k[pat];
            if (pieces_apply(R, t, val, m, k, sb, se)) {
                const uint32_t v = pieces_visit(R, t, val, rng, m, k);
                live = v != 0;
                through = v == 2;
            }
        }
    }
    {
        const bool back = live && !through;
        const uint64_t mm = __ballot(back);
        if (back) {
            const uint32_t q = S.qn + __popcll(mm & ((1ull << lane) - 1));
            Q.t_lo[q] = (uint32_t)t;
            Q.t_hi[q] = (uint32_t)(t >> 32);
            Q.val[q] = val;
            Q.rng[q] = rng;
            Q.seg[q] = (uint32_t)seg;
        }
        S.qn += __popcll(mm);
    }
    int64_t b_cur = 0, b_last = -1, d_lo = 0, d_hi = 0;
    if (R.exact_hits) {
        bool fresh = false;
        int64_t e = 0;
        if (live && through) {
            ++S.n_cand;
            e = (int64_t)t - (int64_t)(val & 0x7FF) + (int64_t)R.m[pat];
            int64_t own_b = (int64_t)R.scan_begin, own_e = (int64_t)R.scan_end;
            if (R.seg_offsets) {
                own_b = R.seg_owned ? sb + (int64_t)R.seg_owned[seg] : sb;
                own_e = se;
            }
            fresh = e >= own_b + 1 && e <= own_e && (!R.seen || seen_insert_raw(R.seen, R.seen_mask, R.overflow, pat, e));
        }
        const unsigned long long idx = wave_reserve_hits(R.hit_counter, fresh ? 1u : 0u);
        if (fresh && idx < R.hit_cap) {
            spm_hit h;
            h.pos = (R.report_begin ? (uint64_t)(e - (int64_t)R.m[pat]) : (uint64_t)e) + R.pos_offset;
            h.pattern = pat;
            h.score = 0;
            R.hits[idx] = h;
        }
        queue_sync();
        return;
    }
    if (live && through) {
        ++S.n_cand;
        d_hi = (int64_t)t - (int64_t)(val & 0x7FF) - sb + (int64_t)R.max_m;
        d_lo = d_hi - (int64_t)((rng & kRngRun) ? (rng & 0x7FF) : 0u);
        b_cur = d_lo / (int64_t)R.Bw;
        b_last = d_hi / (int64_t)R.Bw;
        if (R.overlap && b_cur > 0 && d_lo - b_cur * (int64_t)R.Bw <= (int64_t)R.k[pat])
            --b_cur;
        if ((uint64_t)b_last >> R.band_bits) {
            atomicAdd(&R.counters[kCntVoid], 1ull);
            b_last = b_cur - 1;
        }
    }
    for (;;) {
        const bool have = b_cur <= b_last;
        const uint64_t mm = __ballot(have);
        if (mm == 0)
            break;
        if (have) {
            const unsigned long long bkey =
                ((unsigned long long)pat << 43) | ((unsigned long long)seg << R.band_bits) | (unsigned long long)b_cur;
            const int64_t b0 = b_cur * (int64_t)R.Bw;
            const uint32_t o_lo = (uint32_t)(d_lo > b0 ? d_lo - b0 : 0);
            const uint32_t o_hi = (uint32_t)(d_hi < b0 + (int64_t)R.Bw - 1 ? d_hi - b0 : (int64_t)R.Bw - 1);
            const unsigned long long run = (o_hi - o_lo >= 63 ? ~0ull : ((1ull << (o_hi - o_lo + 1)) - 1)) << o_lo;
            const uint32_t q = S.bn + __popcll(mm & ((1ull << lane) - 1));
            B.key_lo[q] = (uint32_t)bkey;
            B.key_hi[q] = (uint32_t)(bkey >> 32);
            B.run_lo[q] = (uint32_t)run;
            B.run_hi[q] = (uint32_t)(run >> 32);
        }
        S.bn += __popcll(mm);
        queue_sync();
        if (S.bn >= 64) {
            S.bn -= 64;
            insert_bands(R, B, S.bn, 64, lane, S.C);
            queue_sync();
        }
        ++b_cur;
    }
    queue_sync();
}

__global__ __launch_bounds__(256) void resolve_kernel(const resolve_params R)
{
    __shared__ pair_queue pair_queues[4];
    __shared__ band_queue band_queues[4];
    unsigned long long n = R.counters[kCntSurvSlots];
    if (blockIdx.x == 0 && threadIdx.x == 0) {
        atomicAdd(&R.counters[kCntUnreadSurvSum], n);
        atomicMax(&R.counters[kCntUnreadSurvMax], n);
    }
    if (n > R.surv_cap)
        n = R.surv_cap;
    if (!R.exact_hits && __hip_atomic_load(R.table_poison, __ATOMIC_RELAXED, __HIP_MEMORY_SCOPE_AGENT) != 0) {
        if (blockIdx.x == 0 && threadIdx.x == 0)
            atomicAdd(&R.counters[kCntVoid], 1ull);
        return;
    }
    const uint32_t lane = threadIdx.x & 63;
    resolve_wave S;
    S.Q = &pair_queues[threadIdx.x >> 6];
    S.B = &band_queues[threadIdx.x >> 6];
    S.qn = 0;
    S.bn = 0;
// ... 769 lines not shown
```

### libspm_amd/csrc/hits.hip

```cpp
#include "internal.hpp"
#include "hd.hpp"

static int hits_count(spm_hits *h)
{
    spm_ctx *ctx = h->ctx;
    if (h->pending) {
        const int rc = spm_complete_deferred(h);
        if (rc != SPM_OK)
            return rc;
    }
    if (!h->counted) {
        unsigned long long *c = ctx->h_counters;
        SPM_HIP_CHECK(ctx, hipMemcpyAsync(c, h->d_count, kCntReadBackCount * sizeof(unsigned long long), hipMemcpyDeviceToHost, ctx->stream));
        SPM_HIP_CHECK(ctx, hipStreamSynchronize(ctx->stream));
        h->n = c[kCntHits];
        h->counted = true;
    }
    if (h->n > h->cap) {
        SPM_SET_ERR(ctx, "scan produced %llu hits but the buffer holds %llu; raise spm_scan_opts.max_hits",
                    (unsigned long long)h->n, (unsigned long long)h->cap);
        return SPM_E_OVERFLOW;
    }
    return SPM_OK;
}
// ... 8 lines not shown
    if (!h->sorted_host) {
        h->host.resize(h->n);
        if (h->n) {
            SPM_HIP_CHECK(h->ctx, hipMemcpyAsync(h->host.data(), h->d_hits, h->n * sizeof(spm_hit),
                                                 hipMemcpyDeviceToHost, h->ctx->stream));
            SPM_HIP_CHECK(h->ctx, hipStreamSynchronize(h->ctx->stream));
        }
        std::sort(h->host.begin(), h->host.end(), [](const spm_hit &a, const spm_hit &b) {
            return a.pattern != b.pattern ? a.pattern < b.pattern : (int64_t)a.pos < (int64_t)b.pos;
        });
        h->sorted_host = true;
    }
    *records = h->host.data();
    *n = h->n;
    return SPM_OK;
}

extern "C" int spm_hip_hits_device(spm_hits *h, const void **device_records, uint64_t *n)
{
    if (!h || !device_records || !n)
        return SPM_E_INVALID;
    int rc = hits_count(h);
    if (rc != SPM_OK)
        return rc;
    *device_records = h->d_hits;
    *n = h->n;
    return SPM_OK;
}

extern "C" int spm_hip_hits_copy_device(spm_hits *h, void *device_dst, uint64_t cap, uint64_t *n)
{
    if (!h || !n || (cap && !device_dst))
        return SPM_E_INVALID;
    int rc = hits_count(h);
    if (rc != SPM_OK)
        return rc;
    *n = h->n;
    const uint64_t c = std::min(h->n, cap);
    if (c)
        SPM_HIP_CHECK(h->ctx, hipMemcpyAsync(device_dst, h->d_hits, c * sizeof(spm_hit), hipMemcpyDeviceToDevice,
                                             h->ctx->stream));
    return SPM_OK;
}

__global__ __launch_bounds__(256) void hits_fused_copy_kernel(uint4 *__restrict__ dst, const uint4 *__restrict__ src,
                                                                unsigned long long n, unsigned long long n_copy)
{
    const uint64_t i = (uint64_t)blockIdx.x * blockDim.x + threadIdx.x;
    if (i == 0)
        dst[0] = make_uint4((uint32_t)n, (uint32_t)(n >> 32), 0u, 0u);
    for (uint64_t r = i; r < n_copy; r += (uint64_t)gridDim.x * blockDim.x)
        dst[1 + r] = src[r];
}

extern "C" int spm_hip_hits_copy_fused(spm_hits *h, void *device_dst, uint64_t cap, uint64_t *n)
{
    if (!h || !n || !device_dst)
        return SPM_E_INVALID;
    int rc = hits_count(h);
    if (rc != SPM_OK)
        return rc;
    *n = h->n;
    if ((uintptr_t)device_dst & 15) {
        SPM_SET_ERR(h->ctx, "spm_hip_hits_copy_fused: the destination must be 16-byte aligned");
        return SPM_E_INVALID;
    }
    const uint64_t c = std::min(h->n, cap);
    const unsigned grid = (unsigned)std::max<uint64_t>(1, std::min<uint64_t>((c + 255) / 256, (uint64_t)h->ctx->n_cu * 4));
    hipLaunchKernelGGL(hits_fused_copy_kernel, dim3(grid), dim3(256), 0, h->ctx->stream, static_cast<uint4 *>(device_dst),
                       reinterpret_cast<const uint4 *>(h->d_hits), (unsigned long long)h->n, (unsigned long long)c);
    SPM_HIP_CHECK(h->ctx, hipGetLastError());
    return SPM_OK;
}

__global__ __launch_bounds__(256) void hits_fused_copy_device_kernel(uint4 *__restrict__ dst, const uint4 *__restrict__ src,
                                                                       unsigned long long *__restrict__ counters,
                                                                       unsigned long long *__restrict__ host_c,
                                                                       unsigned long long cap, unsigned long long hit_cap,
                                                                       unsigned long long cand_cap)
{
    const unsigned long long n = counters[kCntHits];
    const unsigned long long status = scan_needs_host(counters, cand_cap, n, hit_cap) ? 1ull : 0ull;
    const unsigned long long n_copy = n < cap ? (n < hit_cap ? n : hit_cap) : cap;
    const uint64_t i = (uint64_t)blockIdx.x * blockDim.x + threadIdx.x;
    if (i == 0)
        dst[0] = make_uint4((uint32_t)n, (uint32_t)(n >> 32), (uint32_t)status, 0u);
    if (blockIdx.x == 0 && threadIdx.x < kCntReadBack && host_c)
        host_c[threadIdx.x] = counters[threadIdx.x];
    for (uint64_t r = i; r < n_copy; r += (uint64_t)gridDim.x * blockDim.x)
        dst[1 + r] = src[r];
    if (host_c) {
        __syncthreads();
        __shared__ unsigned int last;
        if (threadIdx.x == 0) {
            __threadfence();
            last = atomicAdd(&counters[kCntTicket], 1ull) == (unsigned long long)gridDim.x - 1 ? 1u : 0u;
        }
        __syncthreads();
        if (last && threadIdx.x < kCntBlock)
            counters[threadIdx.x] = 0;
    }
}

extern "C" int spm_hip_hits_copy_fused_device(spm_hits *h, void *device_dst, uint64_t cap)
{
    if (!h || !device_dst || ((uintptr_t)device_dst & 15))
        return SPM_E_INVALID;
    if (h->pending && h->c_on_the_way) {
        const int rc = hits_count(h);
        if (rc != SPM_OK && rc != SPM_E_OVERFLOW)
            return rc;
    }
    if (!h->pending && h->counted) {
        const uint64_t c = std::min(h->n, std::min<uint64_t>(cap, h->cap));
        const unsigned g1 = (unsigned)std::max<uint64_t>(1, std::min<uint64_t>((c + 255) / 256, (uint64_t)h->ctx->n_cu * 4));
        hipLaunchKernelGGL(hits_fused_copy_kernel, dim3(g1), dim3(256), 0, h->ctx->stream, static_cast<uint4 *>(device_dst),
                           reinterpret_cast<const uint4 *>(h->d_hits), (unsigned long long)h->n, (unsigned long long)c);
        SPM_HIP_CHECK(h->ctx, hipGetLastError());
        return SPM_OK;
    }
    const unsigned grid = (unsigned)std::max<uint64_t>(1, std::min<uint64_t>((std::min<uint64_t>(cap, h->cap) + 255) / 256, (uint64_t)h->ctx->n_cu));
    unsigned long long *host_c = h->pending ? h->h_c : nullptr;
    hipLaunchKernelGGL(hits_fused_copy_device_kernel, dim3(grid), dim3(256), 0, h->ctx->stream, static_cast<uint4 *>(device_dst),
                       reinterpret_cast<const uint4 *>(h->d_hits), h->d_count, host_c, (unsigned long long)cap,
                       (unsigned long long)h->cap, (unsigned long long)(h->cand_cap ? h->cand_cap : ~0ull));
    SPM_HIP_CHECK(h->ctx, hipGetLastError());
    if (host_c) {
        SPM_HIP_CHECK(h->ctx, hipEventRecord(h->ev_done, h->ctx->stream));
        h->c_on_the_way = true;
        h->d_count_cleared = true;
    }
    return SPM_OK;
}

extern "C" int spm_hip_hits_stats(const spm_hits *hc, spm_scan_stats *out)
{
    if (!hc || !out)
        return SPM_E_INVALID;
    spm_hits *h = const_cast<spm_hits *>(hc);
    int rc = hits_count(h);
    if (rc != SPM_OK && rc != SPM_E_OVERFLOW)
        return rc;
    if (h->timed) {
        SPM_HIP_CHECK(h->ctx, hipEventSynchronize(h->ev[3]));
        hipEventElapsedTime(&h->stats.ms_total, h->ev[0], h->ev[3]);
        hipEventElapsedTime(&h->stats.ms_main, h->ev[1], h->ev[2]);
        hipEventElapsedTime(&h->stats.ms_verify, h->ev[2], h->ev[3]);
    }
    h->stats.n_hits = h->n;
    *out = h->stats;
    return SPM_OK;
}

extern "C" uint64_t spm_hip_hits_checksum(spm_hits *h)
{
    const spm_hit *r = nullptr;
    uint64_t n = 0;
    if (spm_hip_hits_view(h, &r, &n) != SPM_OK)
        return 0;
    uint64_t s = 0;
    for (uint64_t i = 0; i < n; ++i)
        s += mix64(r[i].pos ^ ((uint64_t)r[i].pattern << 40) ^ ((uint64_t)(uint32_t)r[i].score << 58));
    return s;
}

extern "C" void spm_hip_hits_destroy(spm_hits *h)
{
    if (!h)
        return;
    if (h->pending)
        (void)spm_complete_deferred(h);
    if (h->d_aux[0] || h->d_aux[1]) {
        if (h->ctx)
            hipStreamSynchronize(h->ctx->stream);
        hipFree(h->d_aux[0]);
        hipFree(h->d_aux[1]);
    }
    if (h->ctx && h->d_hits && h->d_count && h->ev[3] && h->ctx->pool.size() < 8) {
        hits_block b = *h;
        b.zeroed = h->d_count_cleared || hipMemsetAsync(b.d_count, 0, kCntBlock * sizeof(unsigned long long), h->ctx->stream) == hipSuccess;
        h->ctx->pool.push_back(b);
    } else {
        if (h->ctx)
            hipStreamSynchronize(h->ctx->stream);
        hipFree(h->d_hits);
        hipFree(h->d_count);
        for (int i = 0; i < 4; ++i)
            if (h->ev[i])
                hipEventDestroy(h->ev[i]);
        if (h->h_c)
            hipHostFree(h->h_c);
        if (h->ev_done)
            hipEventDestroy(h->ev_done);
    }
    delete h;
}


void spm_warm_hits_kernels()
{
    hipFuncAttributes a;
    (void)hipFuncGetAttributes(&a, (const void *)hits_fused_copy_kernel);
}
```

### libspm_amd/csrc/internal.hpp

```cpp
#pragma once

#include <algorithm>
#include <chrono>
#include <cmath>
#include <cstdlib>
#include <cstring>
#include <memory>

#include "common.hpp"
#include "index_types.hpp"

using namespace spm_hip;

struct spm_patterns : spm_hip::seed_index
{
    spm_ctx *ctx = nullptr;
    int algo = 0;
    uint32_t n = 0;
    uint32_t strands = 1;
    uint32_t sigma = 4;
    std::vector<uint8_t> ranks;
    std::vector<uint32_t> offsets;
    std::vector<int32_t> m, k;
    uint32_t n_groups = 0;
    uint32_t max_m = 0;
    uint32_t max_window = 0;
    uint32_t max_k = 0;
    uint32_t NW = 1;
    bool is_myers() const { return algo == SPM_ALGO_MYERS || algo == SPM_ALGO_MYERS_PREFIX; }
    void *d_arena = nullptr;
    uint32_t *d_peq = nullptr;
    uint32_t *d_peq_bot = nullptr;
    uint32_t *d_peq_verify = nullptr;
    uint32_t *d_hp0 = nullptr;
    int32_t *d_m = nullptr;
    int32_t *d_k = nullptr;
    mutable uint64_t cand_hint = 0;
    uint8_t *d_surplus = nullptr;
    uint8_t *d_ranks = nullptr;
    uint32_t *d_offsets = nullptr;
    uint32_t *d_needle_pk = nullptr;
    uint32_t *d_pk_offsets = nullptr;
    uint16_t *d_seed_q = nullptr;
    pass_entry *d_pass_tab = nullptr;
    uint4 *d_entries = nullptr;
    mutable uint64_t hit_hint = 0;
    mutable bool scanned = false;
    mutable int exact_whole = -1;
    mutable uint64_t band_hint = 0;
    spm_build_stats build{};
    mutable void *d_align = nullptr;
    mutable const uint64_t *d_al_rpeq = nullptr;
    mutable const uint32_t *d_al_rpeq_off = nullptr;
    mutable const uint8_t *d_al_ranks = nullptr;
    mutable const uint32_t *d_al_offsets = nullptr;
};

using clk = std::chrono::steady_clock;
inline float ms_since(clk::time_point t) { return std::chrono::duration<float, std::milli>(clk::now() - t).count(); }
inline hipError_t select_stats_close(bool &timed, hipEvent_t begin, hipEvent_t ordered, hipEvent_t end, spm_select_stats &s)
{
    const hipError_t e = timed ? hipEventSynchronize(end) : hipSuccess;
    if (!timed || e != hipSuccess)
        return e;
    hipEventElapsedTime(&s.ms_total, begin, end);
    hipEventElapsedTime(&s.ms_order, begin, ordered);
    hipEventElapsedTime(&s.ms_select, ordered, end);
    timed = false;
    return hipSuccess;
}

inline bool spm_trace_on() { return trace_on(); }


struct scan_tuning
{
    int cand_cap = 0;
    int brute_cutoff = 1;
    int verify_wave_min_words = 8;
    int span_budget = 0;
    int verify_runs = 1;
    int verify_runs_min_bands = 65536;
    int band_cap = 0;
    static scan_tuning from_env()
    {
        scan_tuning T;
        T.cand_cap = env_int("SPM_HIP_FILTER_CAND_CAP", 0);
        T.brute_cutoff = env_int("SPM_HIP_BRUTE_CUTOFF", 1);
        T.verify_wave_min_words = env_int("SPM_HIP_VERIFY_WAVE_MIN_WORDS", 8);
        T.span_budget = env_int("SPM_HIP_FILTER_SPAN_BUDGET", 0);
        T.verify_runs = env_int("SPM_HIP_VERIFY_RUNS", 1);
        T.verify_runs_min_bands = env_int("SPM_HIP_VERIFY_RUNS_MIN_BANDS", 65536);
        T.band_cap = env_int("SPM_HIP_FILTER_BAND_CAP", 0);
        return T;
    }
};

struct scan_args
{
    spm_ctx *ctx;
    const spm_text *text;
    uint64_t begin, end, ctx_begin;
    const spm_patterns *ps;
    spm_scan_opts opts;
    spm_hits *hits;
    scan_tuning tune;
    const uint64_t *seg_offsets = nullptr;
    uint64_t n_segments = 0;
    const uint64_t *d_seg_offsets = nullptr;
    const uint32_t *d_seg_owned = nullptr;
};

struct scan_state
{
    retry_state retry;
    filter_result filt;
    const uint64_t *segs = nullptr;
    std::vector<uint64_t> seg_host;
    const std::vector<uint64_t> *tiles = nullptr;
};

void state_to_internal(const spm_patterns *p, const void *state, std::vector<uint32_t> &out);
void state_from_internal(const spm_patterns *p, const std::vector<uint32_t> &in, void *state);
int text_alloc(spm_ctx *ctx, uint64_t n, uint32_t sigma, spm_text **out);
int ensure_scratch(spm_ctx *ctx, size_t bytes);
int run_brute(const scan_args &A, const scan_state &S, uint64_t begin, uint64_t end, uint64_t ctx_begin,
              const uint32_t *d_state_in, uint32_t *d_state_out, bool report, bool single_tile);
int run_filter(const scan_args &A, const retry_state &R, filter_result &out);
int scan_impl(spm_ctx *ctx, const spm_text *text, uint64_t begin, uint64_t end, const spm_patterns *patterns,
              const spm_scan_opts *opts_in, const void *state_in, void *state_out, const uint64_t *seg_offsets,
              uint64_t n_segments, spm_hits **out, const uint64_t *d_seg_offsets = nullptr,
              const uint32_t *d_seg_owned = nullptr, const std::function<int(spm_hits *)> *after_launch = nullptr);

struct align_work
{
    const spm_patterns *ps = nullptr;
    const spm_text *text = nullptr;
    uint64_t pos_offset = 0;
    const spm_hit *hits = nullptr;
    uint64_t n = 0;
    const uint64_t *lo = nullptr;
    const uint32_t *cig_off = nullptr;
    bool begin_only = false;
    spm_aln *d_recs = nullptr;
    uint32_t *d_ops = nullptr;
    uint64_t n_ops = 0;
    spm_aln *h_recs = nullptr;
    uint32_t *h_ops = nullptr;
    const char *who = "";
};
int align_run(spm_ctx *ctx, const align_work &W, spm_align_stats &stats);
int spm_align_tables(const spm_patterns *ps);

template <class R, class W = uint32_t, class S = int32_t> struct pool_src
{
    const R *recs;
    uint64_t n;
    const W *ops;
    uint64_t n_ops;
    const W *members = nullptr;
    const S *member_scores = nullptr;
    uint64_t n_members = 0;
};
template <class R, class W, class S>
int pool_out(const pool_src<R, W, S> &src, const R **records, uint64_t *n, const W **ops, uint64_t *n_ops,
             const W **members = nullptr, const S **member_scores = nullptr, uint64_t *n_members = nullptr)
{
    if (!records || !n)
        return SPM_E_INVALID;
    *records = src.recs;
    *n = src.n;
    if (ops)
        *ops = src.ops;
    if (n_ops)
        *n_ops = src.n_ops;
    if (members)
        *members = src.members;
    if (member_scores)
        *member_scores = src.member_scores;
    if (n_members)
        *n_members = src.n_members;
    return SPM_OK;
}

void spm_warm_text_kernels();
void spm_warm_brute_kernels();
void spm_warm_filter_kernels();
void spm_warm_hits_kernels();
void spm_warm_jst_kernels();
void spm_warm_align_kernels();

int spm_complete_deferred(spm_hits *h);
```

### libspm_amd/csrc/scan.hip

```cpp
#include "internal.hpp"
#include "filter_shared.hpp"

int ensure_scratch(spm_ctx *ctx, size_t bytes)
{
    if (ctx->scratch_bytes >= bytes)
        return SPM_OK;
    const auto t0 = clk::now();
    if (ctx->d_scratch) {
        SPM_HIP_CHECK(ctx, hipStreamSynchronize(ctx->stream));
        SPM_HIP_CHECK(ctx, hipFree(ctx->d_scratch));
        ctx->d_scratch = nullptr;
        ctx->scratch_bytes = 0;
    }
    size_t want = bytes + bytes / 4;
    hipError_t e = hipMalloc(&ctx->d_scratch, want);
    if (e != hipSuccess) {
        (void)hipGetLastError();
        want = bytes;
        SPM_HIP_CHECK(ctx, hipMalloc(&ctx->d_scratch, want));
    }
    ctx->scratch_bytes = want;
    if (spm_trace_on())
        fprintf(stderr, "[spm_hip] scratch (survivor / band lists, dedupe set) grows to %.1f MiB: %.2f ms\n", want / 1048576.0, ms_since(t0));
    return SPM_OK;
}

extern "C" int spm_hip_scan(spm_ctx *ctx, const spm_text *text, uint64_t begin, uint64_t end,
                            const spm_patterns *patterns, const spm_scan_opts *opts_in, const void *state_in,
                            void *state_out, spm_hits **out)
{
    return scan_impl(ctx, text, begin, end, patterns, opts_in, state_in, state_out, nullptr, 0, out);
}

extern "C" int spm_hip_scan_segments(spm_ctx *ctx, const spm_text *text, const uint64_t *seg_offsets,
                                     uint64_t n_segments, const spm_patterns *patterns, const spm_scan_opts *opts_in,
                                     spm_hits **out)
{
    if (!ctx || !text || !seg_offsets || n_segments == 0) {
        SPM_SET_ERR(ctx, "spm_hip_scan_segments: invalid argument");
        return SPM_E_INVALID;
    }
    for (uint64_t s = 0; s < n_segments; ++s)
        if (seg_offsets[s + 1] < seg_offsets[s] || seg_offsets[s + 1] > text->n) {
            SPM_SET_ERR(ctx, "spm_hip_scan_segments: offsets must ascend and stay inside the text");
            return SPM_E_INVALID;
        }
    spm_scan_opts o{};
    if (opts_in)
        o = *opts_in;
    o.left_context = 0;
    return scan_impl(ctx, text, seg_offsets[0], seg_offsets[n_segments], patterns, &o, nullptr, nullptr, seg_offsets,
                     n_segments, out);
}

namespace
{
int acquire_hits(spm_ctx *ctx, spm_hits *H)
{
    for (size_t i = 0; i < ctx->pool.size(); ++i)
        if (ctx->pool[i].cap == H->cap) {
            static_cast<hits_block &>(*H) = ctx->pool[i];
            ctx->pool.erase(ctx->pool.begin() + i);
            if (!H->zeroed)
                SPM_HIP_CHECK(ctx, hipMemsetAsync(H->d_count, 0, kCntBlock * sizeof(unsigned long long), ctx->stream));
            return SPM_OK;
        }
    const auto ta = clk::now();
    SPM_HIP_CHECK(ctx, hipMalloc(&H->d_hits, std::max<uint64_t>(H->cap, 1) * sizeof(spm_hit)));
    if (spm_trace_on())
        fprintf(stderr, "[spm_hip] a new hit buffer (%llu records): %.2f ms\n", (unsigned long long)H->cap, ms_since(ta));
    SPM_HIP_CHECK(ctx, hipMalloc(&H->d_count, kCntBlock * sizeof(unsigned long long)));
    for (int i = 0; i < 4; ++i)
        SPM_HIP_CHECK(ctx, hipEventCreate(&H->ev[i]));
    SPM_HIP_CHECK(ctx, hipMemsetAsync(H->d_count, 0, kCntBlock * sizeof(unsigned long long), ctx->stream));
    return SPM_OK;
}

int choose_engine(spm_ctx *ctx, const spm_patterns *patterns, const spm_scan_opts &opts, uint64_t range, bool stateful,
                  bool segmented, uint64_t state_prefix, bool &use_filter)
{
    const bool want_filter = opts.engine == SPM_ENGINE_FILTER || (opts.engine == SPM_ENGINE_AUTO && !patterns->fidx.empty());
    if (opts.engine == SPM_ENGINE_FILTER && patterns->fidx.empty()) {
        SPM_SET_ERR(ctx, "spm_hip_scan: the seed filter does not apply to this needle set");
        return SPM_E_UNSUPPORTED;
    }
    use_filter = want_filter && patterns->n > 0 && range > 0;
    if (stateful && use_filter &&
        (segmented || range <= state_prefix || (opts.engine != SPM_ENGINE_FILTER && range < (1u << 18))))
        use_filter = false;
    if (opts.engine == SPM_ENGINE_FILTER && !use_filter && patterns->n > 0 && range > 0) {
        SPM_SET_ERR(ctx, "spm_hip_scan: the seed filter does not apply to this stateful scan (chunk shorter than a window)");
        return SPM_E_UNSUPPORTED;
    }
    return SPM_OK;
}

void take_stats(spm_hits *h, const unsigned long long *c)
{
    h->stats.n_candidates = c[kCntPairs];
    h->stats.n_bands = (uint32_t)std::min<unsigned long long>(c[kCntBandsVerified], 0xFFFFFFFFull);
}

struct scan_call
{
    const scan_args &A;
    spm_ctx *ctx;
    const spm_patterns *ps;
    spm_hits *H;
    uint64_t begin, end;
    const void *state_in;
    void *state_out;
    bool has_state, stateful, segmented;
    uint64_t state_prefix, tail_begin;
    const std::function<int(spm_hits *)> *after_launch;
    scan_state S{};

    int finish_trivial()
    {
        SPM_HIP_CHECK(ctx, hipEventRecord(H->ev[1], ctx->stream));
        SPM_HIP_CHECK(ctx, hipEventRecord(H->ev[2], ctx->stream));
        SPM_HIP_CHECK(ctx, hipEventRecord(H->ev[3], ctx->stream));
        H->stats.engine_used = SPM_ENGINE_BRUTE;
        if (state_in && state_out && state_out != state_in)
            memcpy(state_out, state_in, spm_hip_patterns_state_stride(ps) * ps->n);
        else if (state_out && !state_in)
            spm_hip_patterns_state_init(ps, state_out);
        return SPM_OK;
    }

    int clear_counters(bool forget_launches = true)
    {
        SPM_HIP_CHECK(ctx, hipMemsetAsync(H->d_count, 0, kCntBlock * sizeof(unsigned long long), ctx->stream));
        if (forget_launches)
            H->stats.main_launches = 0;
        return SPM_OK;
    }

    int host_segments()
    {
        if (S.segs || !A.d_seg_offsets)
            return SPM_OK;
        S.seg_host.resize(A.n_segments + 1);
        SPM_HIP_CHECK(ctx, hipMemcpyAsync(S.seg_host.data(), A.d_seg_offsets, (A.n_segments + 1) * sizeof(uint64_t),
                                          hipMemcpyDeviceToHost, ctx->stream));
        SPM_HIP_CHECK(ctx, hipStreamSynchronize(ctx->stream));
        S.segs = S.seg_host.data();
        return SPM_OK;
    }

    int defer_completion()
    {
        if (!H->h_c)
            SPM_HIP_CHECK(ctx, hipHostMalloc(&H->h_c, kCntBlock * sizeof(unsigned long long), hipHostMallocDefault));
        if (!H->ev_done)
            SPM_HIP_CHECK(ctx, hipEventCreateWithFlags(&H->ev_done, hipEventDisableTiming));
        H->pending = true;
        H->c_on_the_way = false;
        H->d_count_cleared = false;
        ctx->band_dirty = false;
        H->d_text = A.text;
        H->d_patterns = ps;
        H->d_begin = begin;
        H->d_end = end;
        H->d_opts = A.opts;
        return SPM_OK;
    }

    int span_fallback(unsigned long long *c)
    {
        const uint64_t n_ovf = c[kCntSpansGaveUp];
        std::vector<uint64_t> ov(2 * n_ovf);
        SPM_HIP_CHECK(ctx, hipMemcpyAsync(ov.data(), S.filt.d_ovf, ov.size() * sizeof(uint64_t), hipMemcpyDeviceToHost, ctx->stream));
        SPM_HIP_CHECK(ctx, hipStreamSynchronize(ctx->stream));
        const fallback_plan F = plan_fallback(ov.data(), n_ovf, A.begin, end, ps->max_window, (uint64_t)ctx->n_cu, ps->n_groups);
        if (segmented)
            SPM_TRY(host_segments());
        std::vector<uint64_t> tab;
        fallback_tiles(F, A.ctx_begin, segmented ? S.segs : nullptr, A.n_segments, tab);
        H->stats.fallback_spans = (uint32_t)std::min<uint64_t>(n_ovf, 0xFFFFFFFFu);
        if (!tab.empty()) {
            if (tab.size() / 3 > 0xFFFFFFFFull) {
                SPM_SET_ERR(ctx, "span-local fallback: too many tiles");
                return SPM_E_UNSUPPORTED;
            }
            S.tiles = &tab;
            const int rc = run_brute(A, S, begin, end, A.ctx_begin, nullptr, nullptr, true, false);
            S.tiles = nullptr;
            SPM_TRY(rc);
            H->stats.main_launches--;
            SPM_HIP_CHECK(ctx, hipEventRecord(H->ev[3], ctx->stream));
            SPM_HIP_CHECK(ctx, hipMemcpyAsync(c, H->d_count, kCntReadBackRescan * sizeof(unsigned long long), hipMemcpyDeviceToHost, ctx->stream));
            SPM_HIP_CHECK(ctx, hipStreamSynchronize(ctx->stream));
        }
        H->stats.fallback_symbols = F.total;
        return SPM_OK;
    }

    int filter_attempts(bool &use_filter, bool &deferred)
    {
        unsigned long long *c = ctx->h_counters;
        for (int round = 0, attempt = 0; round < 3;) {
            SPM_TRY(run_filter(A, S.retry, S.filt));
            H->cand_cap = S.filt.cand_cap;
            H->band_cap = S.filt.band_cap;
            if ((A.opts.flags & SPM_SCAN_DEFER) && round == 0 && attempt == 0 && !stateful && !segmented && !after_launch) {
                deferred = true;
                return defer_completion();
            }
            if (after_launch && !stateful)
                SPM_TRY((*after_launch)(H));
            SPM_HIP_CHECK(ctx, hipMemcpyAsync(c, H->d_count, kCntReadBack * sizeof(unsigned long long), hipMemcpyDeviceToHost, ctx->stream));
            SPM_HIP_CHECK(ctx, hipStreamSynchronize(ctx->stream));
            if (c[kCntVoid] == 0)
                ctx->band_dirty = false;
            scan_decision d = decide_scan(c, S.filt, H->cap, S.retry, attempt, A.tune.cand_cap);
            if (d.what == scan_outcome::more_room) {
                if (spm_trace_on())
                    fprintf(stderr, "[spm_hip] scan attempt %d starts over:%s%s%s (survivor slots drawn %llu of %llu, band slots %llu of %llu, "
                                    "overflow flags %llu, spans that gave up %llu)\n",
                            attempt, d.more_surv ? " survivor list too small" : "", d.more_bands ? " band list too small" : "",
                            d.more_seen ? " dedupe set too small" : "", c[kCntSurvSlots], (unsigned long long)H->cand_cap,
                            c[kCntBandSlots], (unsigned long long)H->band_cap, c[kCntVoid], c[kCntSpansGaveUp]);
                S.retry = d.next;
                ++attempt;
                SPM_TRY(clear_counters());
                continue;
            }
            take_stats(H, c);
            if (scan_clean(c, H->cand_cap))
                raise_hints(*ps, c);
            const bool rescan = d.what == scan_outcome::span_fallback;
            if (rescan) {
                SPM_TRY(span_fallback(c));
                d = decide_scan(c, S.filt, H->cap, S.retry, attempt, A.tune.cand_cap, true);
            }
            S.retry = d.next;
            switch (d.what) {
            case scan_outcome::brute_fallback:
                H->stats.fell_back = 1;
                use_filter = false;
                return clear_counters(false);
            case scan_outcome::with_seen:
            case scan_outcome::with_full_seen:
                SPM_TRY(clear_counters());
                ++round;
                attempt = 0;
                continue;
            case scan_outcome::final_hits:
            case scan_outcome::caller_overflow:
                H->n = c[kCntHits];
                H->counted = true;
                if (!rescan && d.what == scan_outcome::final_hits && after_launch && !stateful) {
                    H->hook_final = true;
                    H->fan_count = c[kCntFanOut];
                }
                return SPM_OK;
            case scan_outcome::more_room:
            case scan_outcome::span_fallback:
                return SPM_E_INVALID;
            }
        }
        return SPM_OK;
    }

    dev_scratch state_mem;
    uint32_t *d_in = nullptr, *d_out = nullptr;
    size_t st_words = 0;
    std::vector<uint32_t> h_in;
    int state_open()
    {
        if (!stateful)
            return SPM_OK;
        st_words = (size_t)ps->n_groups * (ps->is_myers() ? 2 * ps->NW + 1 : ps->NW) * 64;
        SPM_HIP_CHECK(ctx, state_mem.alloc(&d_in, st_words * 4 * 2));
        d_out = d_in + st_words;
        if (has_state) {
            state_to_internal(ps, state_in, h_in);
            SPM_HIP_CHECK(ctx, hipMemcpyAsync(d_in, h_in.data(), st_words * 4, hipMemcpyHostToDevice, ctx->stream));
        }
        return SPM_OK;
    }
    int state_close(bool have, bool aside)
    {
        if (state_out && !have) {
            SPM_TRY(run_brute(A, S, tail_begin, end, tail_begin, has_state && tail_begin == begin ? d_in : nullptr, d_out, false, true));
            H->stats.main_launches -= aside ? 1 : 0;
        }
        SPM_HIP_CHECK(ctx, hipEventRecord(H->ev[3], ctx->stream));
        std::vector<uint32_t> h_out(state_out ? st_words : 0);
        if (state_out)
            SPM_HIP_CHECK(ctx, hipMemcpyAsync(h_out.data(), d_out, st_words * 4, hipMemcpyDeviceToHost, ctx->stream));
        if (d_in)
            SPM_HIP_CHECK(ctx, hipStreamSynchronize(ctx->stream));
        if (state_out)
            state_from_internal(ps, h_out, state_out);
        return SPM_OK;
    }

    int stateful_remainder()
    {
        SPM_TRY(state_open());
        if (has_state) {
            SPM_TRY(run_brute(A, S, begin, begin + state_prefix, begin, d_in, nullptr, true, true));
            H->stats.main_launches--;
            H->counted = false;
        }
        return state_close(false, true);
    }

    int brute_engine()
    {
        H->stats.engine_used = SPM_ENGINE_BRUTE;
        H->stats.span_symbols = 0;
        SPM_TRY(state_open());
        SPM_HIP_CHECK(ctx, hipEventRecord(H->ev[1], ctx->stream));
        const uint64_t range = end - begin;
        const bool prefix = ps->algo == SPM_ALGO_MYERS_PREFIX;
        const uint64_t warm = ps->max_window > 0 ? ps->max_window - 1 : 0;
        const uint64_t pass_begin = begin - std::min(warm, begin - A.ctx_begin);
        const bool one_pass_state = state_out && (prefix || (range <= (1u << 16) && (has_state || pass_begin <= tail_begin)));
        SPM_TRY(host_segments());
        SPM_TRY(run_brute(A, S, begin, end, A.ctx_begin, has_state ? d_in : nullptr, one_pass_state ? d_out : nullptr, true,
                          one_pass_state));
        SPM_HIP_CHECK(ctx, hipEventRecord(H->ev[2], ctx->stream));
        return state_close(one_pass_state, false);
    }

    void trace(clk::time_point t_call) const
    {
        spm_scan_stats st{};
        spm_hip_hits_stats(H, &st);
        fprintf(stderr, "[spm_hip] scan [%llu, %llu)%s: engine %s%s, %u main launch(es); %.3f ms (main %.3f, verification %.3f); "
                        "%llu seed-checked pairs, %u bands, %llu hits%s; host %.3f ms\n",
                (unsigned long long)begin, (unsigned long long)end, segmented ? " segmented" : "",
                st.engine_used == SPM_ENGINE_FILTER ? (ps->filter_dense ? "filter (dense pass)" : "filter") : "brute",
                st.fell_back ? " after a whole-scan fallback" : "", st.main_launches, st.ms_total, st.ms_main, st.ms_verify,
                (unsigned long long)st.n_candidates, st.n_bands, (unsigned long long)st.n_hits,
                st.fallback_spans ? " (spans re-scanned by the brute-force kernel)" : "", ms_since(t_call));
    }
};

}

int scan_impl(spm_ctx *ctx, const spm_text *text, uint64_t begin, uint64_t end, const spm_patterns *patterns,
              const spm_scan_opts *opts_in, const void *state_in, void *state_out, const uint64_t *seg_offsets,
              uint64_t n_segments, spm_hits **out, const uint64_t *d_seg_offsets, const uint32_t *d_seg_owned,
              const std::function<int(spm_hits *)> *after_launch)
{
    if (!ctx || !text || !patterns || !out || begin > end || end > text->n) {
        SPM_SET_ERR(ctx, "spm_hip_scan: invalid argument");
        return SPM_E_INVALID;
    }
    if (patterns->sigma != text->sigma) {
        SPM_SET_ERR(ctx, "spm_hip_scan: text sigma %u != pattern sigma %u", text->sigma, patterns->sigma);
        return SPM_E_INVALID;
    }
    spm_scan_opts opts{};
    if (opts_in)
        opts = *opts_in;
    const auto t_call = clk::now();
    SPM_HIP_CHECK(ctx, hipSetDevice(ctx->device));

    std::unique_ptr<spm_hits, void (*)(spm_hits *)> H(new spm_hits, spm_hip_hits_destroy);
    H->ctx = ctx;
    H->cap = opts.max_hits ? opts.max_hits : (1ull << 20);
    SPM_TRY(acquire_hits(ctx, H.get()));
    H->al_text = text;
    H->al_patterns = patterns;
    H->al_lo = opts.left_context ? 0 : begin;
    H->al_pos_offset = opts.pos_offset;
    H->al_stateful = state_in != nullptr;
    H->al_device_segs = d_seg_offsets != nullptr && seg_offsets == nullptr;
    if (seg_offsets)
        H->al_segs.assign(seg_offsets, seg_offsets + n_segments + 1);

    const bool has_state = state_in != nullptr, stateful = has_state || state_out != nullptr;
    const bool segmented = seg_offsets || d_seg_offsets;
    const uint64_t state_prefix = has_state && patterns->max_window > 0 ? patterns->max_window - 1 : 0;
    bool use_filter = false;
    SPM_TRY(choose_engine(ctx, patterns, opts, end - begin, stateful, segmented, state_prefix, use_filter));
    const bool chunk = use_filter && has_state;
    const scan_args A{ctx, text, chunk ? begin + state_prefix : begin, end, chunk || !opts.left_context ? begin : 0, patterns, opts,
                      H.get(), scan_tuning::from_env(), seg_offsets, n_segments, d_seg_offsets, d_seg_owned};
    const uint64_t tail_len = 2ull * patterns->max_m + 4;
    const uint64_t tail_begin = std::max(has_state ? begin : A.ctx_begin, end > tail_len ? end - tail_len : 0);
    scan_call C{A, ctx, patterns, H.get(), begin, end, state_in, state_out, has_state, stateful, segmented, state_prefix, tail_begin,
                after_launch};
    C.S.segs = seg_offsets;

    SPM_HIP_CHECK(ctx, hipEventRecord(H->ev[0], ctx->stream));
    H->timed = true;
    const bool past_prefix_hits = patterns->algo == SPM_ALGO_MYERS_PREFIX && !stateful &&
                                  begin - A.ctx_begin >= patterns->max_window;
    if (patterns->n == 0 || past_prefix_hits || (end == begin && (has_state || !state_out || A.ctx_begin == begin))) {
        SPM_TRY(C.finish_trivial());
        *out = H.release();
        return SPM_OK;
    }
    if (use_filter) {
        H->stats.engine_used = SPM_ENGINE_FILTER;
        bool deferred = false;
        SPM_TRY(C.filter_attempts(use_filter, deferred));
        if (deferred) {
            *out = H.release();
            return SPM_OK;
        }
    }
    if (use_filter && stateful)
        SPM_TRY(C.stateful_remainder());
    if (!use_filter)
        SPM_TRY(C.brute_engine());
    if (spm_trace_on())
        C.trace(t_call);
    *out = H.release();
    return SPM_OK;
}


int spm_complete_deferred(spm_hits *h)
{
    if (!h->pending)
        return SPM_OK;
    spm_ctx *ctx = h->ctx;
    h->pending = false;
    if (!h->c_on_the_way) {
        SPM_HIP_CHECK(ctx, hipMemcpyAsync(h->h_c, h->d_count, kCntReadBack * sizeof(unsigned long long), hipMemcpyDeviceToHost, ctx->stream));
        SPM_HIP_CHECK(ctx, hipEventRecord(h->ev_done, ctx->stream));
        h->c_on_the_way = true;
    }
    SPM_HIP_CHECK(ctx, hipEventSynchronize(h->ev_done));
    const unsigned long long *c = h->h_c;
    take_stats(h, c);
    const bool clean = scan_clean(c, h->cand_cap);
    if (c[kCntVoid] != 0)
        ctx->band_dirty = true;
    if (clean || (c[kCntHits] > h->cap && c[kCntVoid] == 0)) {
        if (clean)
            raise_hints(*h->d_patterns, c);
        h->n = c[kCntHits];
        h->counted = true;
        return SPM_OK;
    }
    spm_scan_opts o = h->d_opts;
    o.flags &= ~SPM_SCAN_DEFER;
    spm_hits *again = nullptr;
    const int rc = scan_impl(ctx, h->d_text, h->d_begin, h->d_end, h->d_patterns, &o, nullptr, nullptr, nullptr, 0, &again);
    if (rc != SPM_OK)
        return rc;
    hits_adopt(*h, *again);
    spm_hip_hits_destroy(again);
    return SPM_OK;
}
```

### libspm_amd/csrc/scan_filter.hip

```cpp
#include "internal.hpp"
#include "filter.hpp"

namespace
{
template <typename K, typename... Args>
void launch(K kernel, dim3 grid, uint32_t threads, size_t lds, hipStream_t s, Args... args)
{
    hipFuncSetAttribute((const void *)kernel, hipFuncAttributeMaxDynamicSharedMemorySize, (int)lds);
    hipLaunchKernelGGL(kernel, grid, dim3(threads), lds, s, args...);
}

using filter_kernel = void (*)(filter_params);
using packed_kernel = void (*)(filter_params, const uint4 *);

template <int S, int U, bool KM>
filter_kernel sparse_kernel(uint32_t hv, uint32_t sigma)
{
    if (hv == 2 && sigma == 5)
        return seed_filter_kernel<S, U, 2, 5, KM>;
    if (hv == 2 && sigma == 15)
        return seed_filter_kernel<S, U, 2, 15, KM>;
    if (hv == 1 && sigma == 4)
        return seed_filter_kernel<S, U, 1, 4, KM>;
    if constexpr (S >= 4)
        if (hv == 2 && sigma == 4)
            return seed_filter_kernel<S, U, 2, 4, KM>;
    return nullptr;
}

filter_kernel select_filter_kernel(const filter_index &F, uint32_t sigma, bool km)
{
    if (F.dense) {
        switch (F.n_pat) {
        case 0:
        case 1: return seed_filter_dense_kernel<4, 1>;
        case 2: return seed_filter_dense_kernel<4, 2>;
        case 3: return seed_filter_dense_kernel<4, 3>;
        default: return nullptr;
        }
    }
    if (F.hash_variant == 4) {
        if (F.stride == 1)
            return km ? seed_filter_dense_kernel<4, 1, 1, true> : seed_filter_dense_kernel<4, 1, 1, false>;
        if (F.stride == 2)
            return km ? seed_filter_dense_kernel<4, 1, 2, true> : seed_filter_dense_kernel<4, 1, 2, false>;
        return nullptr;
    }
    switch (F.stride) {
    case 16: return km ? nullptr : sparse_kernel<16, 8, false>(F.hash_variant, sigma);
    case 8: return km ? nullptr : sparse_kernel<8, 8, false>(F.hash_variant, sigma);
    case 4: return km ? nullptr : sparse_kernel<4, 8, false>(F.hash_variant, sigma);
    case 2: return km ? sparse_kernel<2, 2, true>(F.hash_variant, sigma) : sparse_kernel<2, 2, false>(F.hash_variant, sigma);
    case 1:
        if (F.anchor_cm != 0 && F.hash_variant == 2 && sigma == 4 && !km)
            return seed_filter_kernel<1, 4, 2, 4, false, true>;
        return km ? sparse_kernel<1, 2, true>(F.hash_variant, sigma) : sparse_kernel<1, 2, false>(F.hash_variant, sigma);
    default: return nullptr;
    }
}

packed_kernel select_packed_kernel(uint32_t stride, bool km)
{
    if (km)
        return nullptr;
    switch (stride) {
    case 16: return seed_filter_packed_kernel<16, 4, 2, false>;
    case 8: return seed_filter_packed_kernel<8, 4, 2, false>;
    case 4: return seed_filter_packed_kernel<4, 2, 2, false>;
    default: return nullptr;
    }
}

template <int NWN>
void launch_verify_nw(const verify_params &V, dim3 grid, hipStream_t s)
{
    uint32_t threads = 256;
    const size_t per_thread = (size_t)(V.sigma + 1) * NWN * 4 + 2 * 16;
    while (threads > 64 && per_thread * threads > 128 * 1024)
        threads >>= 1;
    const size_t lds = per_thread * threads + (size_t)(threads / 64) * kHitStage * sizeof(spm_hit);
    launch(verify_kernel<NWN>, grid, threads, lds, s, V);
}

template <int G>
void launch_verify_wave_g(verify_params V, const uint32_t *peq_bot, uint32_t max_m, dim3 grid, hipStream_t s)
{
    grid.x *= 4;
    const uint32_t n_slots = 2 * V.max_k + 1 + V.max_span;
    V.wave_text = ((max_m + V.max_k + n_slots + 16 + 15) & ~15u) + 16;
    const size_t per_group = ((n_slots * 2 + 15) & ~15u) + V.wave_text;
    launch(verify_wave_kernel<G, 1>, grid, 64, (64 / G) * per_group, s, V, peq_bot);
}

void launch_verify_wave(uint32_t n_blocks, const verify_params &V, const uint32_t *peq_bot, uint32_t max_m, dim3 grid,
                        hipStream_t s)
{
    if (n_blocks <= 8)
        launch_verify_wave_g<8>(V, peq_bot, max_m, grid, s);
    else if (n_blocks <= 16)
        launch_verify_wave_g<16>(V, peq_bot, max_m, grid, s);
    else if (n_blocks <= 32)
        launch_verify_wave_g<32>(V, peq_bot, max_m, grid, s);
    else
        launch_verify_wave_g<64>(V, peq_bot, max_m, grid, s);
}

void launch_verify(uint32_t nwn, const verify_params &V, dim3 grid, hipStream_t s)
{
    switch (nwn) {
    case 1: launch_verify_nw<1>(V, grid, s); break;
    case 2: launch_verify_nw<2>(V, grid, s); break;
    case 3: launch_verify_nw<3>(V, grid, s); break;
    case 4: launch_verify_nw<4>(V, grid, s); break;
    case 5: launch_verify_nw<5>(V, grid, s); break;
    case 6: launch_verify_nw<6>(V, grid, s); break;
    case 7: launch_verify_nw<7>(V, grid, s); break;
    case 8: launch_verify_nw<8>(V, grid, s); break;
    case 16: launch_verify_nw<16>(V, grid, s); break;
    case 32: launch_verify_nw<32>(V, grid, s); break;
    default: launch_verify_nw<64>(V, grid, s); break;
    }
}

}

int ensure_band_table(spm_ctx *ctx, uint64_t slots)
{
    if (ctx->band_slots >= slots && !ctx->band_dirty)
        return SPM_OK;
    if (ctx->band_slots < slots) {
        const auto t0 = clk::now();
        if (ctx->d_band_tab) {
            SPM_HIP_CHECK(ctx, hipStreamSynchronize(ctx->stream));
            hipFree(ctx->d_band_tab);
            ctx->d_band_tab = nullptr;
            ctx->band_slots = 0;
        }
        SPM_HIP_CHECK(ctx, hipMalloc(&ctx->d_band_tab, slots * sizeof(ulonglong2)));
        ctx->band_slots = slots;
        if (spm_trace_on())
            fprintf(stderr, "[spm_hip] band table grows to %.1f MiB: %.2f ms\n", slots * sizeof(ulonglong2) / 1048576.0, ms_since(t0));
    }
    SPM_HIP_CHECK(ctx, hipMemsetAsync(ctx->d_band_tab, 0xFF, ctx->band_slots * sizeof(ulonglong2), ctx->stream));
    SPM_HIP_CHECK(ctx, hipMemsetAsync(ctx->d_table_poison, 0, 4, ctx->stream));
    ctx->band_dirty = false;
    return SPM_OK;
}

namespace
{
static_assert(sizeof(survivor) == kSurvivorBytes && sizeof(band_rec) == kBandRecBytes, "scan_plan.hpp sizes the lists");

struct filter_run
{
    const scan_args &A;
    const retry_state &retry;
    spm_ctx *ctx;
    const spm_patterns *ps;
    spm_hits *H;
    filter_sizes Z;
    survivor *surv = nullptr;
    unsigned long long *seen = nullptr;
    band_rec *bands = nullptr;
    uint64_t *ovf = nullptr;
    const uint64_t *d_seg = nullptr;
    uint64_t n_seg = 0;
    uint32_t seg_bits = 0;
    bool exact_hits = false, skip_seen = false;

    int lay_out()
    {
        SPM_TRY(ensure_scratch(ctx, Z.surv_bytes + Z.seen_bytes + Z.band_bytes + Z.ovf_bytes));
        exact_hits = ps->max_k == 0 && !Z.overlap && ps->filter_max_range == 0 && ps->d_ranks;
        if (exact_hits && ps->exact_whole < 0) {
            bool whole = true;
            for (uint32_t p = 0; p < ps->n && whole; ++p)
                whole = ps->seed_n[p] == 1 && ps->seed_q[p] == (uint32_t)ps->m[p];
            ps->exact_whole = whole ? 1 : 0;
        }
        exact_hits = exact_hits && ps->exact_whole == 1;
        if (!exact_hits)
            SPM_TRY(ensure_band_table(ctx, Z.band_slots));
        surv = (survivor *)ctx->d_scratch;
        seen = (unsigned long long *)((uint8_t *)surv + Z.surv_bytes);
        bands = (band_rec *)((uint8_t *)seen + Z.seen_bytes);
        ovf = (uint64_t *)((uint8_t *)bands + Z.band_bytes);
        skip_seen = exact_hits && !retry.need_seen;
        if (!skip_seen)
            SPM_HIP_CHECK(ctx, hipMemsetAsync(seen, 0xFF, Z.seen_bytes, ctx->stream));
        if (!exact_hits)
            ctx->band_dirty = true;
        return SPM_OK;
    }

    int launch_passes()
    {
        filter_params P{};
        P.text = A.text->d;
        P.text_alloc = A.text->owned ? A.text->alloc : A.text->n;
        const uint64_t reach = ps->max_window;
        P.lo = A.begin >= A.ctx_begin + reach ? A.begin - reach : A.ctx_begin;
        P.hi = A.end;
        P.surv = surv;
        P.counters = H->d_count;
        P.surv_cap = Z.surv_cap;
        P.ovf_spans = ovf;
        P.ovf_cap = kOvfCap;
        for (size_t fi = 0; fi < ps->fidx.size(); ++fi) {
            const filter_index &F = ps->fidx[fi];
            P.stride = F.stride;
            P.key_len = F.key_len;
            P.key_mask = F.key_len >= 16 ? 0xFFFFFFFFu : ((1u << (2 * F.key_len)) - 1);
            P.bitmap_words = F.hash_variant == 2 ? 1024 : F.bitmap_words;
            P.lds_words = F.lds_words;
            P.chd_slot_mask = F.chd_slot_mask;
            P.chd_bucket_shift = F.chd_bucket_shift;
            P.chd_disp_off = F.chd_disp_off;
            P.n_probes = F.n_probes;
            P.bitmap = F.d_bitmap;
            P.pass = (uint32_t)fi;
            P.anchor_c = F.anchor_c;
            P.anchor_cm = F.anchor_cm;
            P.n_pat = F.n_pat;
            for (uint32_t i = 0; i < kDensePatterns; ++i) {
                P.pat_c[i] = F.pat_c[i];
                P.pat_cm[i] = F.pat_cm[i];
            }
            P.bucket_shift = F.bucket_shift;
            P.buckets = reinterpret_cast<const uint4 *>(F.d_buckets);
            if (fi > 0)
                SPM_HIP_CHECK(ctx, hipMemsetAsync(H->d_count + kCntSpanHead, 0, sizeof(unsigned long long), ctx->stream));
            const bool km = F.key_len < 16;
            const bool bits = F.hash_variant == 4;
            const bool use_packed = F.hash_variant == 2 && A.text->d_packed && ps->sigma == 4 && F.stride >= 2 &&
                                    !(A.opts.flags & SPM_SCAN_IGNORE_PACKED);
            const bool wide_ok = use_packed || F.stride == 2 || (F.stride == 1 && !km && ps->sigma == 4);
            const uint32_t threads = (F.dense || bits || wide_ok) ? 1024 : 512;
            const size_t lds = (size_t)F.lds_words * 4 + 16 + 16 * kCandRec * 4 + ((F.dense || bits) ? 16 * sizeof(dense_queue) : 0);
            const uint32_t wg_per_cu = (uint32_t)std::max<size_t>(1, std::min<size_t>((160 * 1024) / lds, 2048 / threads));
            const uint32_t grid = ctx->n_cu * wg_per_cu;
            const uint64_t n_waves = (uint64_t)grid * (threads / 64);
            const span_plan span = plan_span(stream_geometry_of(P.lo, P.hi, 1024).n_chunks, n_waves, 1024);
            P.span_chunks = span.span_chunks;
            P.span_unit = 1024;
            const int sb = A.tune.span_budget;
            P.span_budget = sb > 0 ? (uint32_t)sb : (uint32_t)std::max<uint64_t>(256, (uint64_t)span.span_chunks * 1024 / 4);
            P.dynamic = span.dynamic;
            P.hash_variant = F.hash_variant;
            H->stats.span_symbols = P.span_chunks * P.span_unit;
            if (use_packed) {
                filter_params Q = P;
                const span_plan pspan = plan_span(stream_geometry_of(Q.lo, Q.hi, 4096).n_chunks, n_waves, 4096);
                Q.span_chunks = pspan.span_chunks;
                Q.span_unit = 4096;
                if (sb <= 0)
                    Q.span_budget = (uint32_t)std::max<uint64_t>(256, (uint64_t)pspan.span_chunks * 4096 / 4);
                Q.dynamic = pspan.dynamic;
                H->stats.span_symbols = Q.span_chunks * Q.span_unit;
                const packed_kernel k = select_packed_kernel(F.stride, km);
                if (!k) {
                    SPM_SET_ERR(ctx, "internal: no packed filter kernel for stride %u, key length %u", F.stride, F.key_len);
                    return SPM_E_UNSUPPORTED;
                }
                launch(k, dim3(grid), threads, lds, ctx->stream, Q, reinterpret_cast<const uint4 *>(A.text->d_packed));
            } else {
                const filter_kernel k = select_filter_kernel(F, ps->sigma, km);
                if (!k) {
                    SPM_SET_ERR(ctx, "internal: no filter kernel for stride %u, key length %u, sigma %u, hash variant %u, %u patterns",
                                F.stride, F.key_len, ps->sigma, F.hash_variant, F.n_pat);
                    return SPM_E_UNSUPPORTED;
                }
                launch(k, dim3(grid), threads, lds, ctx->stream, P);
            }
            SPM_HIP_CHECK(ctx, hipGetLastError());
            H->stats.main_launches++;
        }
        return SPM_OK;
    }

    template <typename Params>
    void fill_shared(Params &X) const
    {
        X.text = A.text->d;
        X.text_alloc = A.text->owned ? A.text->alloc : A.text->n;
        X.scan_begin = A.begin;
        X.scan_end = A.end;
        X.pos_offset = A.opts.pos_offset;
        X.counters = H->d_count;
        X.bands = bands;
        X.band_cap = Z.band_cap;
        X.band_tab = ctx->d_band_tab;
        X.table_mask = (uint32_t)(Z.band_slots - 1);
        X.band_bits = 43 - seg_bits;
        X.Bw = Z.Bw;
        X.overlap = Z.overlap ? 1u : 0u;
        X.max_m = ps->max_m;
        X.m = ps->d_m;
        X.k = ps->d_k;
        X.report_begin = ps->is_myers() ? 0 : 1;
        X.seen_mask = (uint32_t)(Z.seen_slots - 1);
        X.hits = H->d_hits;
        X.hit_counter = H->d_count + kCntHits;
        X.overflow = H->d_count + kCntVoid;
        X.hit_cap = H->cap;
        X.seg_offsets = d_seg;
        X.n_segments = n_seg;
        X.seg_owned = A.d_seg_owned;
    }

    int launch_resolve()
    {
        if (A.d_seg_offsets) {
            d_seg = A.d_seg_offsets;
            n_seg = A.n_segments;
        } else if (A.seg_offsets) {
            uint64_t *d = nullptr;
            SPM_HIP_CHECK(ctx, hipMalloc(&d, (A.n_segments + 1) * sizeof(uint64_t)));
            hipFree(H->d_aux[1]);
            H->d_aux[1] = d;
            SPM_HIP_CHECK(ctx, hipMemcpyAsync(d, A.seg_offsets, (A.n_segments + 1) * sizeof(uint64_t),
                                              hipMemcpyHostToDevice, ctx->stream));
            d_seg = d;
            n_seg = A.n_segments;
        }
        while (n_seg && (1ull << seg_bits) < n_seg + 1)
            ++seg_bits;
        resolve_params R{};
        fill_shared(R);
        R.surv = surv;
        R.surv_cap = Z.surv_cap;
        R.passes = ps->d_pass_tab;
        R.entries = ps->d_entries;
        R.key_len = ps->filter_key_len;
        R.needle_ranks = ps->d_ranks;
        R.needle_offsets = ps->d_offsets;
        R.seed_q = ps->d_seed_q;
        R.flank_check = (ps->sigma == 4 && !Z.overlap && R.needle_ranks) ? 1u : 0u;
        R.pieces_check = R.flank_check;
        R.hay_begin = A.ctx_begin;
        R.hay_end = A.end;
        R.needle_pk = ps->d_needle_pk;
        R.pk_offsets = ps->d_pk_offsets;
        R.exact_hits = exact_hits ? 1u : 0u;
        R.seen = skip_seen ? nullptr : seen;
        R.table_poison = ctx->d_table_poison;
        const uint64_t surv_expect = ps->cand_hint ? 2 * ps->cand_hint : Z.surv_cap;
        const uint64_t rmax = (uint64_t)ctx->n_cu * 5;
        const uint64_t per_wg = (surv_expect + 255) / 256 <= rmax ? 256 : 1024;
        const uint32_t rgrid = (uint32_t)std::min<uint64_t>(rmax, std::max<uint64_t>(ctx->n_cu / 2, (surv_expect + per_wg - 1) / per_wg));
        hipLaunchKernelGGL(resolve_kernel, dim3(rgrid), dim3(256), 0, ctx->stream, R);
        SPM_HIP_CHECK(ctx, hipGetLastError());
        return SPM_OK;
    }

    int launch_bands(bool runs)
    {
        verify_params V{};
        fill_shared(V);
        V.ctx_begin = A.ctx_begin;
        V.surplus = ps->d_surplus;
        V.peq32 = ps->d_peq_verify ? ps->d_peq_verify : ps->d_peq;
        V.sigma = ps->sigma;
        V.nw_table = ps->NW;
        V.max_k = ps->max_k;
        V.max_span = Z.max_span;
        V.seen = seen;
        V.band_counter = kCntBandSlots;
        band_rec *kept = bands + Z.band_cap;
        if (runs) {
            hipLaunchKernelGGL(band_runs_kernel, dim3(ctx->n_cu * 8), dim3(256), 0, ctx->stream, V, bands, kept, H->d_count + kCntRunHeads);
            SPM_HIP_CHECK(ctx, hipGetLastError());
            V.runs = 1;
            V.bands = kept;
            V.band_counter = kCntRunHeads;
        }
        if (Z.overlap) {
            hipLaunchKernelGGL(band_select_kernel, dim3(ctx->n_cu * 2), dim3(256), 0, ctx->stream, V, kept, H->d_count + kCntBandsSelected);
            SPM_HIP_CHECK(ctx, hipGetLastError());
            V.bands = kept;
            V.band_counter = kCntBandsSelected;
            V.preselected = 1;
        }
        if (exact_hits) {
        } else if (Z.use_wave) {
            launch_verify_wave(Z.nwn, V, ps->d_peq_bot, ps->max_m, dim3(ctx->n_cu * 16), ctx->stream);
        } else {
            const uint32_t nwn = Z.nwn > 8 ? ps->NW : Z.nwn;
            const uint64_t band_expect = ps->band_hint ? 2 * ps->band_hint : Z.band_cap;
            const uint32_t vgrid = (uint32_t)std::min<uint64_t>((uint64_t)ctx->n_cu * 4, std::max<uint64_t>(ctx->n_cu / 2, (band_expect + 255) / 256));
            launch_verify(nwn, V, dim3(vgrid), ctx->stream);
        }
        SPM_HIP_CHECK(ctx, hipGetLastError());
        if (runs) {
            hipLaunchKernelGGL(band_release_kernel, dim3(ctx->n_cu * 8), dim3(256), 0, ctx->stream, V, bands, (uint32_t)kCntBandSlots);
            SPM_HIP_CHECK(ctx, hipGetLastError());
        }
        return SPM_OK;
    }
};

}

int run_filter(const scan_args &A, const retry_state &R, filter_result &out)
{
    spm_ctx *ctx = A.ctx;
    spm_hits *H = A.hits;
    filter_run F{A, R, ctx, A.ps, H, size_filter(*A.ps, A.tune, A.end - A.begin, (uint64_t)ctx->n_cu, H->cap, R)};
    const filter_sizes &Z = F.Z;
    SPM_TRY(F.lay_out());
    const bool runs = !Z.overlap && !F.exact_hits && !Z.use_wave && Z.Bw <= 32 && !R.need_seen && A.tune.verify_runs != 0 &&
                      A.ps->band_hint >= (uint64_t)std::max(0, A.tune.verify_runs_min_bands);
    out = {F.seen, (uint32_t)(Z.seen_slots - 1), F.ovf, F.skip_seen || runs, Z.surv_cap, Z.band_cap};
    SPM_HIP_CHECK(ctx, hipEventRecord(H->ev[1], ctx->stream));
    SPM_TRY(F.launch_passes());
    SPM_HIP_CHECK(ctx, hipEventRecord(H->ev[2], ctx->stream));
    SPM_TRY(F.launch_resolve());
    SPM_TRY(F.launch_bands(runs));
    SPM_HIP_CHECK(ctx, hipEventRecord(H->ev[3], ctx->stream));
    return SPM_OK;
}


void spm_warm_filter_kernels()
{
    hipFuncAttributes a;
    (void)hipFuncGetAttributes(&a, (const void *)resolve_kernel);
}
```

### libspm_amd/csrc/scan_plan.hpp

```cpp
#pragma once

#include <algorithm>
#include <cassert>
#include <cmath>
#include <cstddef>
#include <utility>
#include <vector>

#include "hd.hpp"

namespace spm_hip
{

enum scan_counter : int
{
    kCntHits = 0,
    kCntSurvSlots = 1,
    kCntVoid = 2,
    kCntBandSlots = 3,
    kCntSpanHead = 4,
    kCntPairs = 5,
    kCntSpansGaveUp = 6,
    kCntBandsVerified = 7,
    kCntUnreadSurvSum = 8,
    kCntUnreadSurvMax = 9,
    kCntBandsSelected = 10,
    kCntRunHeads = 11,
    kCntFanOut = 12,
    kCntStateOnly = 13,
    kCntTicket = 15,
};
constexpr int kCntBlock = 16;
constexpr int kCntReadBack = 13;
constexpr int kCntReadBackRescan = 8;
constexpr int kCntReadBackCount = 4;
constexpr int kLandFanOut = 13;

SPM_HD inline bool scan_needs_host(const unsigned long long *c, unsigned long long cand_cap, const unsigned long long &n = 0,
                                   unsigned long long hit_cap = 0)
{
    return c[kCntVoid] != 0 || c[kCntSpansGaveUp] != 0 || c[kCntSurvSlots] > cand_cap || n > hit_cap;
}
SPM_HD inline bool scan_clean(const unsigned long long *c, unsigned long long cand_cap) { return !scan_needs_host(c, cand_cap); }

template <typename Set>
inline void raise_hints(const Set &ps, const unsigned long long *c)
{
    ps.cand_hint = std::max<uint64_t>(ps.cand_hint, c[kCntSurvSlots]);
    ps.hit_hint = std::max<uint64_t>(ps.hit_hint, c[kCntHits]);
    ps.band_hint = std::max<uint64_t>(ps.band_hint, c[kCntBandSlots]);
    ps.scanned = true;
}

struct retry_state
{
    uint64_t cand_cap_override = 0;
    uint64_t band_scale = 0;
    bool seen_full = false;
    bool need_seen = false;
};
struct filter_result
{
    unsigned long long *d_seen = nullptr;
    uint32_t seen_mask = 0;
    uint64_t *d_ovf = nullptr;
    bool seen_skipped = false;
    uint64_t cand_cap = 0, band_cap = 0;
};
enum class scan_outcome
{
    final_hits,
    caller_overflow,
    more_room,
    with_seen,
    with_full_seen,
    span_fallback,
    brute_fallback,
};
struct scan_decision
{
    scan_outcome what = scan_outcome::final_hits;
    retry_state next;
    bool more_surv = false, more_bands = false, more_seen = false;
};
constexpr uint64_t kSurvMax = 1ull << 27;
constexpr uint64_t kBandMax = 1ull << 28;

inline scan_decision decide_scan(const unsigned long long *c, const filter_result &ran, uint64_t hit_cap, const retry_state &rs,
                                 int attempt, int cand_cap_knob, bool rescanned = false)
{
    scan_decision d;
    d.next = rs;
    if (c[kCntHits] <= hit_cap && attempt < 2 && !rescanned) {
        d.more_surv = c[kCntSurvSlots] > ran.cand_cap && ran.cand_cap < kSurvMax && !cand_cap_knob;
        d.more_bands = c[kCntVoid] != 0 && c[kCntBandSlots] > ran.band_cap && ran.band_cap < kBandMax;
        d.more_seen = c[kCntVoid] != 0 && !rs.seen_full && !d.more_bands && c[kCntBandSlots] <= ran.band_cap;
        if (d.more_surv || d.more_bands || d.more_seen) {
            d.what = scan_outcome::more_room;
            if (d.more_surv)
                d.next.cand_cap_override = std::min<uint64_t>(
                    kSurvMax, std::max<uint64_t>(c[kCntSurvSlots] + c[kCntSurvSlots] / 8 + 4096, 4 * ran.cand_cap));
            if (d.more_bands)
                d.next.band_scale = std::max<uint64_t>(1, rs.band_scale) *
                                    std::max<uint64_t>(2, (c[kCntBandSlots] + ran.band_cap - 1) / ran.band_cap + 1);
            if (d.more_seen || c[kCntHits] > ((uint64_t)ran.seen_mask + 1) / 8)
                d.next.seen_full = true;
            return d;
        }
    }
    if (c[kCntHits] > hit_cap)
        d.what = scan_outcome::caller_overflow;
    else if (c[kCntVoid] != 0 && rescanned && !rs.seen_full) {
        d.what = scan_outcome::with_full_seen;
        d.next.seen_full = true;
    } else if (c[kCntVoid] != 0)
        d.what = scan_outcome::brute_fallback;
    else if (c[kCntSpansGaveUp] != 0 && !rescanned) {
        d.what = ran.seen_skipped ? scan_outcome::with_seen : scan_outcome::span_fallback;
        d.next.need_seen |= ran.seen_skipped;
    }
    return d;
}

inline void append_tiles(std::vector<uint64_t> &tab, uint64_t lo, uint64_t hi, uint64_t hay_lo, uint64_t warm, uint64_t tile)
{
    for (; lo < hi; lo += tile) {
        tab.push_back(lo >= hay_lo + warm ? lo - warm : hay_lo);
        tab.push_back(lo);
        tab.push_back(std::min(lo + tile, hi));
    }
}

constexpr uint64_t kOvfCap = 1ull << 17;

struct fallback_plan
{
    std::vector<std::pair<uint64_t, uint64_t>> ranges;
    uint64_t total = 0;
    uint64_t warm = 0, tile = 0;
};
inline fallback_plan plan_fallback(const uint64_t *ov, uint64_t n_ovf, uint64_t begin, uint64_t end, uint32_t max_window,
                                   uint64_t n_cu, uint32_t n_groups)
{
    fallback_plan F;
    std::vector<std::pair<uint64_t, uint64_t>> rg;
    rg.reserve(n_ovf);
    for (uint64_t i = 0; i < n_ovf; ++i) {
        const uint64_t b = ov[2 * i], len = ov[2 * i + 1];
        const uint64_t lo = std::max<uint64_t>(begin, b >= 16 ? b - 16 : 0);
        const uint64_t hi = std::min<uint64_t>(end, b + len + max_window);
        if (lo < hi)
            rg.emplace_back(lo, hi);
    }
    std::sort(rg.begin(), rg.end());
    for (const auto &r : rg) {
        if (!F.ranges.empty() && r.first <= F.ranges.back().second)
            F.ranges.back().second = std::max(F.ranges.back().second, r.second);
        else
            F.ranges.push_back(r);
    }
    for (const auto &r : F.ranges)
        F.total += r.second - r.first;
    F.warm = max_window > 0 ? max_window - 1 : 0;
    const uint64_t want_tiles = n_cu * 32 / std::max(1u, n_groups) + 1;
    F.tile = std::max<uint64_t>(std::max<uint64_t>(1024, (F.warm * 8 + 255) & ~255ull), (F.total / want_tiles + 255) & ~255ull);
    F.tile = std::min<uint64_t>(F.tile, 1u << 20);
    return F;
}
inline void fallback_tiles(const fallback_plan &F, uint64_t ctx_begin, const uint64_t *segs, uint64_t n_segments,
                           std::vector<uint64_t> &tab)
{
    for (const auto &r : F.ranges) {
        if (!segs) {
            append_tiles(tab, r.first, r.second, ctx_begin, F.warm, F.tile);
            continue;
        }
        uint64_t sidx = (uint64_t)(std::upper_bound(segs, segs + n_segments + 1, r.first) - segs);
        sidx = sidx ? sidx - 1 : 0;
        for (; sidx < n_segments && segs[sidx] < r.second; ++sidx)
            append_tiles(tab, std::max(r.first, segs[sidx]), std::min(r.second, segs[sidx + 1]), segs[sidx], F.warm, F.tile);
    }
}

struct stream_geometry
{
    uint64_t base0;
    uint64_t n_chunks;
    uint64_t n_whole;
    uint64_t n_spans;
};
SPM_HD inline stream_geometry stream_geometry_of(uint64_t lo, uint64_t hi, uint32_t unit, uint32_t span_chunks = 1)
{
    stream_geometry G;
    G.base0 = lo & ~(uint64_t)(unit - 1);
    G.n_chunks = (hi - G.base0 + (unit - 1)) / unit;
    G.n_whole = (hi - G.base0) / unit;
    G.n_spans = (G.n_chunks + span_chunks - 1) / span_chunks;
    return G;
}

struct span_plan
{
    uint32_t span_chunks = 0;
    uint32_t dynamic = 0;
};
inline span_plan plan_span(uint64_t n_chunks, uint64_t n_waves, uint32_t unit)
{
    assert(unit == 1024 || unit == 4096);
    span_plan S;
    if (unit == 4096) {
        uint64_t pspan = n_chunks / (n_waves * 8) + 1;
        pspan = std::min<uint64_t>(std::max<uint64_t>(pspan, 4), 4096);
        pspan = (pspan + 3) & ~3ull;
        S.span_chunks = (uint32_t)pspan;
        S.dynamic = pspan >= 48 ? 1u : 2u;
        assert(S.dynamic == 1 || S.dynamic == 2);
        return S;
    }
    uint64_t span = n_chunks / (n_waves * 32) + 1;
    if (span < 64)
        span = std::max<uint64_t>(span, std::min<uint64_t>(64, n_chunks / (n_waves * 4) + 1));
    span = std::min<uint64_t>(std::max<uint64_t>(span, 8), 4096);
    span = (span + 7) & ~7ull;
    S.span_chunks = (uint32_t)span;
    S.dynamic = span >= 192 ? 1u : 2u;
    assert(S.dynamic == 1 || S.dynamic == 2);
    return S;
}

constexpr uint32_t kChunkMin = 32;
constexpr size_t kSurvivorBytes = 16, kBandRecBytes = 16;

struct filter_sizes
{
    uint64_t surv_cap = 0, band_cap = 0, band_slots = 0, seen_slots = 0;
    uint32_t nwn = 1, Bw = 32, max_span = 31;
    bool use_wave = false;
    bool overlap = false;
    size_t surv_bytes = 0, seen_bytes = 0, band_bytes = 0, ovf_bytes = 0;
};

template <typename Set, typename Tune>
inline filter_sizes size_filter(const Set &ps, const Tune &tune, uint64_t symbols, uint64_t n_cu, uint64_t hit_cap, const retry_state &R)
{
    filter_sizes Z;
    const uint64_t kmax = ps.max_k;
    uint64_t est = std::max<uint64_t>(4096, 8ull * ps.n * (kmax + 1));
    est = std::max<uint64_t>(est, symbols / (ps.scanned ? 4096 : 2048));
    double chance = 0;
    for (const auto &F : ps.fidx)
        chance += (double)symbols / std::max(1u, F.stride) * (double)F.n_keys / std::pow(4.0, (double)F.key_len);
    est = std::max<uint64_t>(est, (uint64_t)(2.0 * chance));
    est = std::max<uint64_t>(est, ps.cand_hint + ps.cand_hint / 4);
    Z.surv_cap = std::min(2 * est + n_cu * 16 * kChunkMin, kSurvMax);
    if (R.cand_cap_override)
        Z.surv_cap = R.cand_cap_override;
    if (tune.cand_cap > 0)
        Z.surv_cap = (uint64_t)tune.cand_cap;
    const uint64_t band_want = std::max<uint64_t>(Z.surv_cap / 4, 2 * ps.band_hint);
    Z.band_cap = std::max<uint64_t>(band_want, 4096) * (R.band_scale ? R.band_scale : 1) + n_cu * 32 * kChunkMin;
    if (tune.band_cap > 0 && !R.band_scale)
        Z.band_cap = (uint64_t)tune.band_cap;
    Z.band_slots = 1u << 12;
    while (Z.band_slots < 2 * Z.band_cap)
        Z.band_slots <<= 1;
    Z.nwn = std::max(1u, (ps.max_m + 31) / 32);
    const int wave_min = tune.verify_wave_min_words;
    Z.use_wave = ps.d_peq_bot && wave_min > 0 && Z.nwn >= (uint32_t)wave_min && ps.sigma <= 5;
    Z.overlap = ps.d_surplus != nullptr;
    Z.Bw = 32;
    if (Z.overlap) {
        Z.Bw = (ps.max_k + 1) * (Z.use_wave ? 4 : 1);
        if (Z.Bw + ps.max_k > 2047)
            Z.Bw = ps.max_k + 1;
    }
    Z.max_span = Z.Bw - 1 + (Z.overlap ? ps.max_k + 1 : 0);
    uint64_t want_seen = std::min<uint64_t>(Z.band_cap * (2 * kmax + 1 + Z.max_span), std::max<uint64_t>(hit_cap, 1));
    if (!R.seen_full)
        want_seen = std::min<uint64_t>(want_seen, ps.scanned ? std::max<uint64_t>(1u << 18, 4 * ps.hit_hint) : (1ull << 22));
    Z.seen_slots = 1u << 16;
    while (Z.seen_slots < 2 * want_seen)
        Z.seen_slots <<= 1;
    Z.surv_bytes = Z.surv_cap * kSurvivorBytes;
    Z.seen_bytes = Z.seen_slots * sizeof(unsigned long long);
    Z.band_bytes = Z.band_cap * kBandRecBytes * 2;
    Z.ovf_bytes = kOvfCap * 2 * sizeof(uint64_t);
    return Z;
}

}
```

### libspm_amd/engine.py

```python
from __future__ import annotations

import ctypes as C

import numpy as np

from . import capi

HIT_DTYPE = np.dtype([("pos", "<u8"), ("pattern", "<u4"), ("score", "<i4")])
ALN_DTYPE = np.dtype([("begin", "<u8"), ("end", "<u8"), ("pattern", "<u4"), ("score", "<i4"), ("cigar_off", "<u4"),
                      ("cigar_len", "<u4")])
_CIGAR_CHAR = {capi.CIGAR_INS: "I", capi.CIGAR_DEL: "D", capi.CIGAR_EQ: "=", capi.CIGAR_X: "X"}


def _check(rc, ctx_handle):
    if rc != 0:
        msg = capi.lib().spm_hip_last_error(ctx_handle)
        raise capi.SpmError(f"libspm_hip error {rc}: {msg.decode() if msg else ''}")


class Context:
    def __init__(self, device: int = 0, stream: int | None = None):
        self._h = C.c_void_p()
        rc = capi.lib().spm_hip_init(device, C.c_void_p(stream) if stream else None, C.byref(self._h))
        if rc != 0:
# ... 60 lines not shown
        h = C.c_void_p()
        create = capi.lib().spm_hip_patterns_create_stranded if both_strands else capi.lib().spm_hip_patterns_create
        _check(create(self._h, algo, cat.ctypes.data_as(C.POINTER(C.c_uint8)), offs.ctypes.data_as(C.POINTER(C.c_uint32)),
                      len(needles), ks.ctypes.data_as(C.POINTER(C.c_uint16)), sigma, C.byref(h)), self._h)
        return PatternSet(self, h, algo, (2 if both_strands else 1) * len(needles))


class Text:
    def __init__(self, ctx, h, sigma):
        self.ctx, self._h, self.sigma = ctx, h, sigma
        self._keepalive = None

    def __len__(self):
        return int(capi.lib().spm_hip_text_length(self._h))

    @property
    def device_ptr(self) -> int:
        return int(capi.lib().spm_hip_text_device_ptr(self._h) or 0)

    def pack(self):
        _check(capi.lib().spm_hip_text_pack(self.ctx._h, self._h), self.ctx._h)
        return self

    @property
    def packed(self) -> bool:
        return bool(capi.lib().spm_hip_text_is_packed(self._h))

    def download(self, begin: int, n: int) -> np.ndarray:
        out = np.empty(n, dtype=np.uint8)
        _check(capi.lib().spm_hip_text_download(self.ctx._h, self._h, begin, n,
                                                out.ctypes.data_as(C.POINTER(C.c_uint8))), self.ctx._h)
        return out

    def close(self):
        if self._h:
            if self.ctx._h:
                capi.lib().spm_hip_text_destroy(self._h)
            self._h = C.c_void_p()

    def __del__(self):
        try:
            self.close()
        except Exception:
            pass


class PatternSet:
    def __init__(self, ctx, h, algo, n):
        self.ctx, self._h, self.algo, self.n = ctx, h, algo, n

    def __len__(self):
        return int(capi.lib().spm_hip_patterns_count(self._h))

    @property
    def strands(self) -> int:
        return int(capi.lib().spm_hip_patterns_strands(self._h))

    def needle(self, p: int) -> np.ndarray:
        n = C.c_uint32()
        capi.lib().spm_hip_patterns_needle(self._h, p, None, 0, C.byref(n))
        out = np.empty(n.value, dtype=np.uint8)
        rc = capi.lib().spm_hip_patterns_needle(self._h, p, out.ctypes.data_as(C.POINTER(C.c_uint8)), n.value, C.byref(n))
        if rc != 0:
            raise capi.SpmError(f"spm_hip_patterns_needle: no needle {p} in a set of {len(self)}")
        return out

    def window_size(self, p: int = 0) -> int:
        return int(capi.lib().spm_hip_patterns_window_size(self._h, p))

    @property
    def filterable(self) -> bool:
        return bool(capi.lib().spm_hip_patterns_filterable(self._h))

    def build_stats(self) -> capi.BuildStats:
        st = capi.BuildStats()
        _check(capi.lib().spm_hip_patterns_build_stats(self._h, C.byref(st)), self.ctx._h)
        return st

    def state_stride(self) -> int:
        return int(capi.lib().spm_hip_patterns_state_stride(self._h))

    def initial_state(self) -> np.ndarray:
        st = np.zeros(self.state_stride() * max(1, self.n), dtype=np.uint8)
        _check(capi.lib().spm_hip_patterns_state_init(self._h, st.ctypes.data), self.ctx._h)
        return st

    def close(self):
        if self._h:
            if self.ctx._h:
                capi.lib().spm_hip_patterns_destroy(self._h)
            self._h = C.c_void_p()

    def __del__(self):
        try:
            self.close()
        except Exception:
            pass


class Hits:
    def __init__(self, ctx, h, text=None, pats=None):
        self.ctx, self._h, self._text, self._pats = ctx, h, text, pats

    def view(self) -> np.ndarray:
        rec = C.POINTER(capi.Hit)()
        n = C.c_uint64()
        _check(capi.lib().spm_hip_hits_view(self._h, C.byref(rec), C.byref(n)), self.ctx._h)
        if n.value == 0:
            return np.zeros(0, dtype=HIT_DTYPE)
        buf = (capi.Hit * n.value).from_address(C.addressof(rec.contents))
        return np.frombuffer(buf, dtype=HIT_DTYPE).copy()

    def device(self):
        p = C.c_void_p()
        n = C.c_uint64()
        _check(capi.lib().spm_hip_hits_device(self._h, C.byref(p), C.byref(n)), self.ctx._h)
        return int(p.value or 0), int(n.value)

    def copy_to(self, device_ptr: int, cap: int) -> int:
        n = C.c_uint64()
        _check(capi.lib().spm_hip_hits_copy_device(self._h, C.c_void_p(device_ptr), cap, C.byref(n)), self.ctx._h)
        return int(n.value)

    def copy_fused(self, device_ptr: int, cap: int) -> int:
        n = C.c_uint64()
        _check(capi.lib().spm_hip_hits_copy_fused(self._h, C.c_void_p(device_ptr), cap, C.byref(n)), self.ctx._h)
        return int(n.value)

    def copy_fused_device(self, device_ptr: int, cap: int) -> None:
        _check(capi.lib().spm_hip_hits_copy_fused_device(self._h, C.c_void_p(device_ptr), cap), self.ctx._h)

    def align(self, begin_only: bool = False) -> "Alignments":
        a = C.c_void_p()
        _check(capi.lib().spm_hip_hits_align(self._h, capi.ALIGN_BEGIN_ONLY if begin_only else 0, C.byref(a)),
               self.ctx._h)
        return Alignments(self.ctx, a)

    def select(self, loci: bool = True, window: int | None = None, best: int | None = None, strands: bool = False) -> "Hits":
        opts = _select_opts(loci, window, best, strands=strands)
        h = C.c_void_p()
        _check(capi.lib().spm_hip_hits_select(self._h, C.byref(opts), C.byref(h)), self.ctx._h)
        return Hits(self.ctx, h, self._text, self._pats)

    def select_stats(self) -> capi.SelectStats:
        s = capi.SelectStats()
        _check(capi.lib().spm_hip_hits_select_stats(self._h, C.byref(s)), self.ctx._h)
        return s

    def stats(self) -> capi.ScanStats:
        s = capi.ScanStats()
        _check(capi.lib().spm_hip_hits_stats(self._h, C.byref(s)), self.ctx._h)
        return s

    def checksum(self) -> int:
        return int(capi.lib().spm_hip_hits_checksum(self._h))

    def close(self):
        if self._h:
            if self.ctx._h:
                capi.lib().spm_hip_hits_destroy(self._h)
            self._h = C.c_void_p()

    def __del__(self):
        try:
            self.close()
        except Exception:
            pass


def _as_array(ptr, n, ctype, dtype):
    if n == 0:
        return np.zeros(0, dtype=dtype)
    buf = (ctype * n).from_address(C.addressof(ptr.contents))
    return np.frombuffer(buf, dtype=dtype).copy()


class _RecordPool:
    _PREFIX = _REC = _DTYPE = _STATS = None

    def __init__(self, ctx, h):
        self.ctx, self._h = ctx, h

    def _call(self, name, *args):
        _check(getattr(capi.lib(), f"spm_hip_{self._PREFIX}_{name}")(self._h, *args), self.ctx._h)

    def _raw(self):
        rec, ops = C.POINTER(self._REC)(), C.POINTER(C.c_uint32)()
        n, n_ops = C.c_uint64(), C.c_uint64()
        self._call("view", C.byref(rec), C.byref(n), C.byref(ops), C.byref(n_ops))
        return rec, n.value, ops, n_ops.value

    def __len__(self):
        return self._raw()[1]

    def view(self) -> np.ndarray:
        r = self._raw()
        return _as_array(r[0], r[1], self._REC, self._DTYPE)

    @property
    def ops(self) -> np.ndarray:
        r = self._raw()
        return _as_array(r[2], r[3], C.c_uint32, np.uint32)

    def _device(self):
        r, o = C.c_void_p(), C.c_void_p()
        n, n_ops = C.c_uint64(), C.c_uint64()
        self._call("device", C.byref(r), C.byref(n), C.byref(o), C.byref(n_ops))
        return int(r.value or 0), int(n.value), int(o.value or 0), int(n_ops.value)

    def _cigar(self, i, records, ops) -> str:
        r = (self.view() if records is None else records)[i]
        o = self.ops if ops is None else ops
        words = o[int(r["cigar_off"]):int(r["cigar_off"]) + int(r["cigar_len"])]
        return "".join(f"{int(w) >> 4}{_CIGAR_CHAR[int(w) & 15]}" for w in words)

    def _stats(self):
        s = self._STATS()
        self._call("stats", C.byref(s))
        return s

    def close(self):
        if self._h:
            if self.ctx._h:
                getattr(capi.lib(), f"spm_hip_{self._PREFIX}_destroy")(self._h)
            self._h = C.c_void_p()

    def __del__(self):
        try:
            self.close()
        except Exception:
            pass


class Alignments(_RecordPool):
    _PREFIX, _REC, _DTYPE, _STATS = "alns", capi.Aln, ALN_DTYPE, capi.AlignStats

    def device(self):
        return self._device()

    def cigar(self, i: int, records: np.ndarray | None = None, ops: np.ndarray | None = None) -> str:
        return self._cigar(i, records, ops)

    def stats(self) -> capi.AlignStats:
        return self._stats()


def scan(ctx: Context, text: Text, pats: PatternSet, begin: int = 0, end: int | None = None, *,
         engine: int = capi.ENGINE_AUTO, left_context: bool = False, pos_offset: int = 0, max_hits: int = 0,
         state_in: np.ndarray | None = None, want_state: bool = False, flags: int = 0):
    end = len(text) if end is None else end
    opts = capi.ScanOpts(engine=engine, left_context=1 if left_context else 0, pos_offset=pos_offset,
                         max_hits=max_hits, flags=flags, reserved=0)
    h = C.c_void_p()
    st_in = state_in.ctypes.data if state_in is not None else None
    st_out = None
    if want_state:
        st_out = np.zeros(pats.state_stride() * max(1, pats.n), dtype=np.uint8)
    _check(capi.lib().spm_hip_scan(ctx._h, text._h, begin, end, pats._h, C.byref(opts), st_in,
                                   st_out.ctypes.data if st_out is not None else None, C.byref(h)), ctx._h)
    hits = Hits(ctx, h, text, pats)
    return (hits, st_out) if want_state else hits


def _select_opts(loci, window, best, across=False, strands=False) -> capi.SelectOpts:
    flags = ((capi.SELECT_LOCI if loci else 0) | (capi.SELECT_BEST if best is not None else 0)
             | (capi.SELECT_ACROSS if across else 0) | (capi.SELECT_STRANDS if strands else 0))
    return capi.SelectOpts(flags=flags, window=capi.SELECT_WINDOW_K if window is None else int(window),
                           strata=0 if best is None else int(best), reserved=0)


def select_records(ctx: Context, device_ptr: int, n: int, pats: PatternSet | None = None, *, loci: bool = True,
                   window: int | None = None, best: int | None = None, strands: bool = False) -> Hits:
    opts = _select_opts(loci, window, best, strands=strands)
    h = C.c_void_p()
    _check(capi.lib().spm_hip_records_select(ctx._h, C.c_void_p(device_ptr), n, pats._h if pats is not None else None,
                                             C.byref(opts), C.byref(h)), ctx._h)
    return Hits(ctx, h, None, pats)


def scan_segments(ctx: Context, text: Text, pats: PatternSet, seg_offsets, *, engine: int = capi.ENGINE_AUTO,
                  max_hits: int = 0, flags: int = 0) -> Hits:
    offs = np.ascontiguousarray(seg_offsets, dtype=np.uint64)
    opts = capi.ScanOpts(engine=engine, left_context=0, pos_offset=0, max_hits=max_hits, flags=flags, reserved=0)
    h = C.c_void_p()
    _check(capi.lib().spm_hip_scan_segments(ctx._h, text._h, offs.ctypes.data_as(C.POINTER(C.c_uint64)),
                                            len(offs) - 1, pats._h, C.byref(opts), C.byref(h)), ctx._h)
    return Hits(ctx, h, text, pats)


def synth_pattern(seed_text: int, seed_pat: int, n_total: int, p: int, L: int, kmax: int):
    out = np.empty(L, dtype=np.uint8)
    o = capi.lib().spm_hip_synth_pattern(seed_text, seed_pat, n_total, p, L, kmax,
                                         out.ctypes.data_as(C.POINTER(C.c_uint8)))
    return out, int(o)


def synth_repeat_pattern(seed_text: int, seed_pat: int, n_total: int, p: int, L: int, kmax: int, repeat_ppm: int,
                         across_every: int = 8):
    out = np.empty(L, dtype=np.uint8)
    o = capi.lib().spm_hip_synth_repeat_pattern(seed_text, seed_pat, n_total, p, L, kmax, repeat_ppm, across_every,
                                                out.ctypes.data_as(C.POINTER(C.c_uint8)))
    return out, int(o)


def synth_repeat_text(seed: int, repeat_ppm: int, begin: int, n: int) -> np.ndarray:
    out = np.empty(n, dtype=np.uint8)
# ... 369 lines not shown
```

Baseline: 6436.

## Finish seed survivors inline in filter kernel with wave-level Myers verification

Adds an inline finish step to the seed filter kernel for stride>=4, hash variant 2, sigma 4 instances. At the end of each span, a wave reads back its own recent survivors, does the hash lookup, seed and piece checks, groups diagonals, and runs a small Myers verification directly on the text, writing hits. The aim is to skip the separate resolve and band-verify passes and their global survivor and band traffic for simple single-pass scans. The cost is extra registers and code in the filter kernel, and a gate that restricts the path to small patterns (<=4 words, k<=15), few survivors and no overlap or runs.

```diff
diff --git a/include/spm_hip.h b/include/spm_hip.h
--- a/include/spm_hip.h
+++ b/include/spm_hip.h
@@ -133,6 +133,7 @@
 int spm_hip_hits_copy_fused(spm_hits *hits, void *device_dst, uint64_t cap, uint64_t *n);
 int spm_hip_hits_copy_fused_device(spm_hits *hits, void *device_dst, uint64_t cap);
 int spm_hip_hits_stats(const spm_hits *hits, spm_scan_stats *out);
+int spm_hip_hits_inline_pairs(const spm_hits *hits, uint64_t *out);
 uint64_t spm_hip_hits_checksum(spm_hits *hits);
 void spm_hip_hits_destroy(spm_hits *hits);
 
diff --git a/libspm_amd/capi.py b/libspm_amd/capi.py
--- a/libspm_amd/capi.py
+++ b/libspm_amd/capi.py
@@ -339,6 +339,7 @@
         "spm_hip_hits_copy_fused": (C.c_int, [vp, vp, C.c_uint64, C.POINTER(C.c_uint64)]),
         "spm_hip_hits_copy_fused_device": (C.c_int, [vp, vp, C.c_uint64]),
         "spm_hip_hits_stats": (C.c_int, [vp, C.POINTER(ScanStats)]),
+        "spm_hip_hits_inline_pairs": (C.c_int, [vp, C.POINTER(C.c_uint64)]),
         "spm_hip_hits_checksum": (C.c_uint64, [vp]),
         "spm_hip_hits_destroy": (None, [vp]),
         "spm_hip_hits_align": (C.c_int, [vp, C.c_uint32, C.POINTER(vp)]),
@@ -437,7 +438,7 @@
     "spm_hip_patterns_create_stranded", "spm_hip_patterns_strands", "spm_hip_patterns_count", "spm_hip_patterns_needle",
     "spm_hip_patterns_window_size", "spm_hip_patterns_filterable", "spm_hip_patterns_build_stats", "spm_hip_patterns_state_stride",
     "spm_hip_patterns_state_init", "spm_hip_scan", "spm_hip_scan_segments", "spm_hip_hits_view", "spm_hip_hits_device",
-    "spm_hip_hits_copy_device", "spm_hip_hits_copy_fused", "spm_hip_hits_copy_fused_device", "spm_hip_hits_stats", "spm_hip_hits_checksum", "spm_hip_hits_destroy",
+    "spm_hip_hits_copy_device", "spm_hip_hits_copy_fused", "spm_hip_hits_copy_fused_device", "spm_hip_hits_stats", "spm_hip_hits_inline_pairs", "spm_hip_hits_checksum", "spm_hip_hits_destroy",
     "spm_hip_hits_align", "spm_hip_alns_view", "spm_hip_alns_device", "spm_hip_alns_stats", "spm_hip_alns_destroy",
     "spm_hip_hits_select", "spm_hip_records_select", "spm_hip_hits_select_stats",
     "spm_hip_synth_pattern",
diff --git a/libspm_amd/csrc/common.hpp b/libspm_amd/csrc/common.hpp
--- a/libspm_amd/csrc/common.hpp
+++ b/libspm_amd/csrc/common.hpp
@@ -89,6 +89,7 @@
     bool sorted_host = false;
     std::vector<spm_hit> host;
     spm_scan_stats stats{};
+    uint64_t n_inline = 0;
     bool timed = false;
     void *d_aux[2] = {nullptr, nullptr};
     bool pending = false;
@@ -144,6 +145,7 @@
     h.n = from.n;
     h.counted = from.counted;
     h.stats = from.stats;
+    h.n_inline = from.n_inline;
     h.cand_cap = from.cand_cap;
     h.band_cap = from.band_cap;
     h.timed = from.timed;
diff --git a/libspm_amd/csrc/filter.hpp b/libspm_amd/csrc/filter.hpp
--- a/libspm_amd/csrc/filter.hpp
+++ b/libspm_amd/csrc/filter.hpp
@@ -30,6 +30,46 @@
 constexpr uint32_t kChunkMax = 1024;
 constexpr uint32_t kCandLdsSlot = 4;
 constexpr uint32_t kCandRec = 8;
+
+struct resolve_params
+{
+    const survivor *surv;
+    unsigned long long *counters;
+    uint64_t surv_cap;
+    const pass_entry *passes;
+    const uint4 *entries;
+    uint32_t key_len;
+    uint32_t flank_check;
+    uint32_t pieces_check;
+    const uint8_t *text;
+    uint64_t text_alloc;
+    const uint8_t *needle_ranks;
+    const uint32_t *needle_offsets;
+    const uint16_t *seed_q;
+    const int32_t *m, *k;
+    uint64_t hay_begin, hay_end;
+    const uint64_t *seg_offsets;
+    uint64_t n_segments;
+    uint32_t Bw, overlap, max_m;
+    uint32_t band_bits;
+    ulonglong2 *band_tab;
+    uint32_t table_mask;
+    band_rec *bands;
+    uint64_t band_cap;
+    const uint32_t *needle_pk;
+    const uint32_t *pk_offsets;
+    uint32_t exact_hits;
+    uint32_t report_begin;
+    uint64_t scan_begin, scan_end;
+    uint64_t pos_offset;
+    const uint32_t *seg_owned;
+    unsigned long long *seen;
+    uint32_t seen_mask;
+    spm_hit *hits;
+    unsigned long long *hit_counter, *overflow;
+    uint64_t hit_cap;
+    uint32_t *table_poison;
+};
 
 struct filter_params
 {
@@ -63,6 +103,20 @@
     uint64_t ovf_cap;
 };
 
+struct filter_params_inline : filter_params
+{
+    uint32_t inline_finish;
+    uint32_t fin_nw_table;
+    const uint32_t *fin_peq32;
+    resolve_params fin;
+};
+template <int S, int HV, int SIG, bool KM, bool AN>
+constexpr bool kInlineInstance = S >= 4 && HV == 2 && SIG == 4 && !KM && !AN;
+template <int S, int HV, int SIG, bool KM, bool AN>
+using filter_params_of = std::conditional_t<kInlineInstance<S, HV, SIG, KM, AN>, filter_params_inline, filter_params>;
+
+__device__ void span_finish();
+
 __device__ __forceinline__ void wave_count_add(unsigned long long *counter, uint32_t v)
 {
     for (int o = 32; o > 0; o >>= 1)
@@ -453,7 +507,7 @@
 }
 
 template <int S, int U, int HV, int SIG, bool KM, bool AN = false>
-__global__ __launch_bounds__(((S == 1 && !KM && SIG == 4) || (S == 2 && U == 2)) ? 1024 : 512) void seed_filter_kernel(const filter_params P)
+__global__ __launch_bounds__(((S == 1 && !KM && SIG == 4) || (S == 2 && U == 2)) ? 1024 : 512) void seed_filter_kernel(const filter_params_of<S, HV, SIG, KM, AN> P)
 {
     extern __shared__ uint32_t lds[];
     stream_stage(P, lds);
@@ -508,6 +562,8 @@
             one[0] = load_text16(P.text, (G.base0 + ch * 1024) | ((uint64_t)lane * 16), P.hi);
             filter_group<S, 1, HV, SIG, KM, AN>(P, one, G.base0 + ch * 1024, carry_in, carry_n, lane, lds, idx_mask);
         }
+        if constexpr (kInlineInstance<S, HV, SIG, KM, AN>)
+            span_finish();
     }
     surv_close(P, cand_chunk_of(P, lds), lane);
 }
@@ -822,45 +878,6 @@
     const uint32_t *seg_owned;
 };
 
-struct resolve_params
-{
-    const survivor *surv;
-    unsigned long long *counters;
-    uint64_t surv_cap;
-    const pass_entry *passes;
-    const uint4 *entries;
-    uint32_t key_len;
-    uint32_t flank_check;
-    uint32_t pieces_check;
-    const uint8_t *text;
-    uint64_t text_alloc;
-    const uint8_t *needle_ranks;
-    const uint32_t *needle_offsets;
-    const uint16_t *seed_q;
-    const int32_t *m, *k;
-    uint64_t hay_begin, hay_end;
-    const uint64_t *seg_offsets;
-    uint64_t n_segments;
-    uint32_t Bw, overlap, max_m;
-    uint32_t band_bits;
-    ulonglong2 *band_tab;
-    uint32_t table_mask;
-    band_rec *bands;
-    uint64_t band_cap;
-    const uint32_t *needle_pk;
-    const uint32_t *pk_offsets;
-    uint32_t exact_hits;
-    uint32_t report_begin;
-    uint64_t scan_begin, scan_end;
-    uint64_t pos_offset;
-    const uint32_t *seg_owned;
-    unsigned long long *seen;
-    uint32_t seen_mask;
-    spm_hit *hits;
-    unsigned long long *hit_counter, *overflow;
-    uint64_t hit_cap;
-    uint32_t *table_poison;
-};
 
 __device__ __forceinline__ unsigned long long band_value(unsigned long long stored, bool counting)
 {
@@ -1145,6 +1162,257 @@
     }
     atomicAdd(overflow, 1ull);
     return false;
+}
+
+__device__ __forceinline__ uint32_t wave_max_u32(uint32_t v)
+{
+    for (int o = 32; o > 0; o >>= 1)
+        v = max(v, (uint32_t)__shfl_xor((int)v, o));
+    return (uint32_t)__builtin_amdgcn_readfirstlane(v);
+}
+
+__device__ __forceinline__ int64_t shfl_i64(int64_t v, int src)
+{
+    const uint32_t lo = (uint32_t)__shfl((int)(uint32_t)v, src), hi = (uint32_t)__shfl((int)(uint32_t)((uint64_t)v >> 32), src);
+    return (int64_t)(((uint64_t)hi << 32) | lo);
+}
+
+__device__ __forceinline__ void span_finish_open(const filter_params_inline &P, const uint32_t *lds, uint32_t lane);
+
+__device__ __forceinline__ void span_finish()
+{
+    auto args = __builtin_amdgcn_kernarg_segment_ptr();
+    asm volatile("" : "+s"(args));
+    const filter_params_inline &P = *(const filter_params_inline *)args;
+    if (__builtin_expect(P.inline_finish != 0, 0)) {
+        extern __shared__ uint32_t lds[];
+        span_finish_open(P, lds, threadIdx.x & 63);
+    }
+}
+
+__device__ __forceinline__ void span_finish_open(const filter_params_inline &P, const uint32_t *lds, uint32_t lane)
+{
+    const resolve_params &R = P.fin;
+    const uint32_t *ck = cand_chunk_of(P, lds);
+    const uint32_t cnt = (uint32_t)__builtin_amdgcn_readfirstlane(ck[4]);
+    if (__builtin_amdgcn_readfirstlane(ck[5]) != 0 || cnt == 0 || cnt > kInlineMaxSurvivors)
+        return;
+    const uint32_t used = (uint32_t)__builtin_amdgcn_readfirstlane(ck[2]);
+    const uint64_t cbase = uniform_u64(((uint64_t)ck[1] << 32) | ck[0]);
+    const uint32_t take = cnt < used ? cnt : used;
+    const uint64_t slot = cbase + used - take + lane;
+    bool mine = lane < take && slot < P.surv_cap;
+    __builtin_amdgcn_fence(__ATOMIC_RELEASE, "agent");
+    uint32_t key = 0, pad = 0;
+    uint64_t t = 0;
+    if (mine) {
+        uint32_t *sv = reinterpret_cast<uint32_t *>(P.surv + slot);
+        key = __hip_atomic_load(sv + 0, __ATOMIC_RELAXED, __HIP_MEMORY_SCOPE_AGENT);
+        const uint32_t t_lo = __hip_atomic_load(sv + 1, __ATOMIC_RELAXED, __HIP_MEMORY_SCOPE_AGENT);
+        const uint32_t t_hi = __hip_atomic_load(sv + 2, __ATOMIC_RELAXED, __HIP_MEMORY_SCOPE_AGENT);
+        pad = __hip_atomic_load(sv + 3, __ATOMIC_RELAXED, __HIP_MEMORY_SCOPE_AGENT);
+        t = ((uint64_t)t_hi << 32) | t_lo;
+        mine = t_hi != kSurvInvalid;
+    }
+    const int64_t hay_b = (int64_t)R.hay_begin, hay_e = (int64_t)R.hay_end;
+    text64 W;
+    W.lo = 0;
+    W.hi = 0;
+    W.ok = false;
+    uint32_t first = 0, ecnt = 0;
+    if (mine) {
+        if (R.flank_check && (int64_t)t - 16 >= hay_b && (int64_t)t + 48 <= hay_e && t + 48 <= R.text_alloc) {
+            const uint8_t *p = R.text + (t - 16);
+            W.lo = (uint64_t)pack16(load_bytes16(p)) | ((uint64_t)pack16(load_bytes16(p + 16)) << 32);
+            W.hi = (uint64_t)pack16(load_bytes16(p + 32)) | ((uint64_t)pack16(load_bytes16(p + 48)) << 32);
+            W.ok = true;
+        }
+        const pass_entry T = R.passes[pad];
+        uint32_t hs = ht_hash(key) & T.ht_mask;
+        for (;;) {
+            const uint4 d = T.ht[hs];
+            if (d.z == 0)
+                break;
+            if (d.x == key) {
+                first = d.y;
+                ecnt = d.z;
+                break;
+            }
+            hs = (hs + 1) & T.ht_mask;
+        }
+        if (ecnt > kInlineMaxEntries)
+            mine = false;
+        for (uint32_t j = 0; mine && j < ecnt; ++j)
+            if (R.entries[first + j].z & kRngRun)
+                mine = false;
+    }
+    if (!mine)
+        ecnt = 0;
+    uint32_t n_pairs = 0, n_groups = 0;
+    const uint32_t jmax = wave_max_u32(ecnt);
+    for (uint32_t j = 0; j < jmax; ++j) {
+        bool through = false;
+        uint32_t val = 0;
+        if (j < ecnt) {
+            const uint4 e = R.entries[first + j];
+            val = e.x;
+            const uint32_t r0 = e.z & 0x1F, ns = (e.z >> 5) & 0x1F;
+            const bool whole = (e.z & kRngWhole) != 0;
+            bool live = true, checked = false;
+            if (W.ok) {
+                live = seed_sig_ok(W, e.y, r0, ns, R.key_len);
+                checked = live && whole;
+            }
+            if (live && !checked)
+                live = seed_intact(R, t, val, r0, whole ? R.key_len + ns : 0u, hay_b, hay_e);
+            if (live && R.pieces_check) {
+                const uint32_t m = (uint32_t)R.m[val >> 11], k = (uint32_t)R.k[val >> 11];
+                if (pieces_apply(R, t, val, m, k, hay_b, hay_e)) {
+                    uint32_t progress = 0, v;
+                    do
+                        v = pieces_visit(R, t, val, progress, m, k);
+                    while (v == 1);
+                    live = v == 2;
+                }
+            }
+            through = live;
+        }
+        n_pairs += through ? 1u : 0u;
+        const uint32_t pat = val >> 11;
+        const int64_t d = (int64_t)t - (int64_t)(val & 0x7FF);
+        if (R.exact_hits) {
+            const int64_t e = d + (through ? (int64_t)R.m[pat] : 0);
+            const bool fresh = through && e >= (int64_t)R.scan_begin + 1 && e <= (int64_t)R.scan_end &&
+                               (!R.seen || seen_insert_raw(R.seen, R.seen_mask, R.overflow, pat, e));
+            const unsigned long long idx = wave_reserve_hits(R.hit_counter, fresh ? 1u : 0u);
+            if (fresh && idx < R.hit_cap) {
+                spm_hit h;
+                h.pos = (R.report_begin ? (uint64_t)(e - (int64_t)R.m[pat]) : (uint64_t)e) + R.pos_offset;
+                h.pattern = pat;
+                h.score = 0;
+                R.hits[idx] = h;
+            }
+            continue;
+        }
+        const uint64_t live_mask = __ballot(through);
+        if (live_mask == 0)
+            continue;
+        int64_t g_lo = d, g_hi = d;
+        for (;;) {
+            bool grew = false;
+            for (uint64_t mm = live_mask; mm != 0; mm &= mm - 1) {
+                const int o = __ffsll((unsigned long long)mm) - 1;
+                const uint32_t o_pat = (uint32_t)__shfl((int)pat, o);
+                const int64_t o_d = shfl_i64(d, o);
+                if (through && o_pat == pat && inline_group_joins(g_lo, g_hi, o_d, R.Bw)) {
+                    grew = grew || o_d < g_lo || o_d > g_hi;
+                    g_lo = o_d < g_lo ? o_d : g_lo;
+                    g_hi = o_d > g_hi ? o_d : g_hi;
+                }
+            }
+            if (__ballot(grew) == 0)
+                break;
+        }
+        bool head = through;
+        for (uint64_t mm = live_mask; mm != 0; mm &= mm - 1) {
+            const int o = __ffsll((unsigned long long)mm) - 1;
+            const uint32_t o_pat = (uint32_t)__shfl((int)pat, o);
+            const int64_t o_lo = shfl_i64(g_lo, o);
+            if ((uint32_t)o < lane && o_pat == pat && o_lo == g_lo)
+                head = false;
+        }
+        const int64_t m = head ? (int64_t)R.m[pat] : 1, k = head ? (int64_t)R.k[pat] : 0;
+        inline_range rg;
+        const bool active = inline_end_range(g_lo, g_hi, m, k, (int64_t)R.scan_begin, (int64_t)R.scan_end, hay_b, rg) && head;
+        n_groups += active ? 1u : 0u;
+        const int64_t e_lo = rg.e_lo, e_hi = active ? rg.e_hi : rg.ws, ws = rg.ws;
+        constexpr int NWI = (int)kInlineMaxWords;
+        uint32_t E[5][NWI];
+#pragma unroll
+        for (int r = 0; r < 5; ++r)
+#pragma unroll
+            for (int w = 0; w < NWI; ++w) {
+                const int32_t tw = (int32_t)P.fin_nw_table - NWI + w;
+                E[r][w] = 0xFFFFFFFFu;
+                if (active && tw >= 0)
+                    E[r][w] = P.fin_peq32[(((size_t)(pat >> 6) * 5 + r) * P.fin_nw_table + (uint32_t)tw) * 64 + (pat & 63)];
+            }
+        myers_lane<NWI, false> L;
+        {
+            const int32_t off = NWI * 32 - (int32_t)m;
+#pragma unroll
+            for (int w = 0; w < NWI; ++w) {
+                const int32_t lo = off - w * 32;
+                L.VP[w] = lo <= 0 ? 0xFFFFFFFFu : (lo >= 32 ? 0u : (0xFFFFFFFFu << lo));
+                L.VN[w] = 0;
+            }
+            L.score = (int32_t)m;
+        }
+        const int64_t blk0 = ws & ~15ll;
+        uint4 nxt = make_uint4(0, 0, 0, 0);
+        if (active)
+            nxt = load_text16(R.text, (uint64_t)blk0, R.text_alloc);
+        const uint32_t n_cols = (uint32_t)(e_hi - ws);
+        const uint32_t rel_lo = (uint32_t)(e_lo - 1 - ws);
+        uint32_t rel0 = (uint32_t)(blk0 - ws);
+        const uint32_t my_blocks = active ? (uint32_t)((e_hi - blk0 + 15) >> 4) : 0u;
+        const uint32_t max_blocks = wave_max_u32(my_blocks);
+        for (uint32_t bi = 0; bi < max_blocks; ++bi, rel0 += 16) {
+            const int64_t blk = blk0 + 16 * (int64_t)bi;
+            uint32_t hitmask = 0;
+            uint64_t scores = 0;
+            if (bi < my_blocks) {
+                const uint4 cur = nxt;
+                if (bi + 1 < my_blocks)
+                    nxt = load_text16(R.text, (uint64_t)(blk + 16), R.text_alloc);
+                const uint32_t words[4] = {cur.x, cur.y, cur.z, cur.w};
+#pragma unroll
+                for (int i = 0; i < 16; ++i) {
+                    const uint32_t rel = rel0 + (uint32_t)i;
+                    if (rel >= n_cols)
+                        continue;
+                    const uint32_t sym = (words[i >> 2] >> (8 * (i & 3))) & 0xFF;
+                    const uint32_t s0 = 0u - (sym & 1u), s1 = 0u - ((sym >> 1) & 1u), s4 = sym < 4 ? 0xFFFFFFFFu : 0u;
+                    uint32_t eq[NWI];
+#pragma unroll
+                    for (int w = 0; w < NWI; ++w) {
+                        const uint32_t lo2 = (E[1][w] & s0) | (E[0][w] & ~s0), hi2 = (E[3][w] & s0) | (E[2][w] & ~s0);
+                        eq[w] = (((hi2 & s1) | (lo2 & ~s1)) & s4) | (E[4][w] & ~s4);
+                    }
+                    L.step_strided(eq, 1);
+                    if (L.score <= (int32_t)k && rel >= rel_lo) {
+                        hitmask |= 1u << i;
+                        scores |= (uint64_t)(uint32_t)L.score << (4 * i);
+                    }
+                }
+            }
+            if (__ballot(hitmask != 0) == 0)
+                continue;
+            uint32_t keep = 0;
+            for (uint32_t mm = hitmask; mm != 0; mm &= mm - 1) {
+                const uint32_t i = (uint32_t)__ffs(mm) - 1u;
+                if (seen_insert_raw(R.seen, R.seen_mask, R.overflow, pat, blk + (int64_t)i + 1))
+                    keep |= 1u << i;
+            }
+            unsigned long long idx = wave_reserve_hits(R.hit_counter, (uint32_t)__popc(keep));
+            for (uint32_t mm = keep; mm != 0; mm &= mm - 1, ++idx) {
+                const uint32_t i = (uint32_t)__ffs(mm) - 1u;
+                const int64_t e = blk + (int64_t)i + 1;
+                if (idx < R.hit_cap) {
+                    spm_hit h;
+                    h.pos = (R.report_begin ? (uint64_t)(e - m) : (uint64_t)e) + R.pos_offset;
+                    h.pattern = pat;
+                    h.score = (int32_t)((scores >> (4 * i)) & 0xF);
+                    R.hits[idx] = h;
+                }
+            }
+        }
+    }
+    wave_count_add(R.counters + kCntPairs, n_pairs);
+    wave_count_add(R.counters + kCntInline, n_pairs);
+    wave_count_add(R.counters + kCntBandsVerified, n_groups);
+    if (mine)
+        P.surv[slot].t_hi = kSurvInvalid;
 }
 
 struct resolve_wave
diff --git a/libspm_amd/csrc/hits.hip b/libspm_amd/csrc/hits.hip
--- a/libspm_amd/csrc/hits.hip
+++ b/libspm_amd/csrc/hits.hip
@@ -184,6 +184,18 @@
     return SPM_OK;
 }
 
+extern "C" int spm_hip_hits_inline_pairs(const spm_hits *hc, uint64_t *out)
+{
+    if (!hc || !out)
+        return SPM_E_INVALID;
+    spm_hits *h = const_cast<spm_hits *>(hc);
+    const int rc = hits_count(h);
+    if (rc != SPM_OK && rc != SPM_E_OVERFLOW)
+        return rc;
+    *out = h->n_inline;
+    return SPM_OK;
+}
+
 extern "C" uint64_t spm_hip_hits_checksum(spm_hits *h)
 {
     const spm_hit *r = nullptr;
diff --git a/libspm_amd/csrc/internal.hpp b/libspm_amd/csrc/internal.hpp
--- a/libspm_amd/csrc/internal.hpp
+++ b/libspm_amd/csrc/internal.hpp
@@ -109,6 +109,7 @@
     uint64_t n_segments = 0;
     const uint64_t *d_seg_offsets = nullptr;
     const uint32_t *d_seg_owned = nullptr;
+    bool stateful = false;
 };
 
 struct scan_state
diff --git a/libspm_amd/csrc/scan.hip b/libspm_amd/csrc/scan.hip
--- a/libspm_amd/csrc/scan.hip
+++ b/libspm_amd/csrc/scan.hip
@@ -99,6 +99,7 @@
 {
     h->stats.n_candidates = c[kCntPairs];
     h->stats.n_bands = (uint32_t)std::min<unsigned long long>(c[kCntBandsVerified], 0xFFFFFFFFull);
+    h->n_inline = c[kCntInline];
 }
 
 struct scan_call
@@ -154,6 +155,7 @@
             SPM_HIP_CHECK(ctx, hipHostMalloc(&H->h_c, kCntBlock * sizeof(unsigned long long), hipHostMallocDefault));
         if (!H->ev_done)
             SPM_HIP_CHECK(ctx, hipEventCreateWithFlags(&H->ev_done, hipEventDisableTiming));
+        H->h_c[kCntInline] = 0;
         H->pending = true;
         H->c_on_the_way = false;
         H->d_count_cleared = false;
@@ -209,7 +211,7 @@
             }
             if (after_launch && !stateful)
                 SPM_TRY((*after_launch)(H));
-            SPM_HIP_CHECK(ctx, hipMemcpyAsync(c, H->d_count, kCntReadBack * sizeof(unsigned long long), hipMemcpyDeviceToHost, ctx->stream));
+            SPM_HIP_CHECK(ctx, hipMemcpyAsync(c, H->d_count, kCntReadBackHost * sizeof(unsigned long long), hipMemcpyDeviceToHost, ctx->stream));
             SPM_HIP_CHECK(ctx, hipStreamSynchronize(ctx->stream));
             if (c[kCntVoid] == 0)
                 ctx->band_dirty = false;
@@ -381,7 +383,7 @@
     SPM_TRY(choose_engine(ctx, patterns, opts, end - begin, stateful, segmented, state_prefix, use_filter));
     const bool chunk = use_filter && has_state;
     const scan_args A{ctx, text, chunk ? begin + state_prefix : begin, end, chunk || !opts.left_context ? begin : 0, patterns, opts,
-                      H.get(), scan_tuning::from_env(), seg_offsets, n_segments, d_seg_offsets, d_seg_owned};
+                      H.get(), scan_tuning::from_env(), seg_offsets, n_segments, d_seg_offsets, d_seg_owned, stateful};
     const uint64_t tail_len = 2ull * patterns->max_m + 4;
     const uint64_t tail_begin = std::max(has_state ? begin : A.ctx_begin, end > tail_len ? end - tail_len : 0);
     scan_call C{A, ctx, patterns, H.get(), begin, end, state_in, state_out, has_state, stateful, segmented, state_prefix, tail_begin,
@@ -424,7 +426,7 @@
     spm_ctx *ctx = h->ctx;
     h->pending = false;
     if (!h->c_on_the_way) {
-        SPM_HIP_CHECK(ctx, hipMemcpyAsync(h->h_c, h->d_count, kCntReadBack * sizeof(unsigned long long), hipMemcpyDeviceToHost, ctx->stream));
+        SPM_HIP_CHECK(ctx, hipMemcpyAsync(h->h_c, h->d_count, kCntReadBackHost * sizeof(unsigned long long), hipMemcpyDeviceToHost, ctx->stream));
         SPM_HIP_CHECK(ctx, hipEventRecord(h->ev_done, ctx->stream));
         h->c_on_the_way = true;
     }
diff --git a/libspm_amd/csrc/scan_filter.hip b/libspm_amd/csrc/scan_filter.hip
--- a/libspm_amd/csrc/scan_filter.hip
+++ b/libspm_amd/csrc/scan_filter.hip
@@ -11,6 +11,7 @@
 }
 
 using filter_kernel = void (*)(filter_params);
+using inline_kernel = void (*)(filter_params_inline);
 using packed_kernel = void (*)(filter_params, const uint4 *);
 
 template <int S, int U, bool KM>
@@ -22,10 +23,19 @@
         return seed_filter_kernel<S, U, 2, 15, KM>;
     if (hv == 1 && sigma == 4)
         return seed_filter_kernel<S, U, 1, 4, KM>;
-    if constexpr (S >= 4)
-        if (hv == 2 && sigma == 4)
-            return seed_filter_kernel<S, U, 2, 4, KM>;
     return nullptr;
+}
+
+inline_kernel select_inline_kernel(const filter_index &F, uint32_t sigma, bool km)
+{
+    if (F.dense || F.hash_variant != 2 || sigma != 4 || km)
+        return nullptr;
+    switch (F.stride) {
+    case 16: return seed_filter_kernel<16, 8, 2, 4, false>;
+    case 8: return seed_filter_kernel<8, 8, 2, 4, false>;
+    case 4: return seed_filter_kernel<4, 8, 2, 4, false>;
+    default: return nullptr;
+    }
 }
 
 filter_kernel select_filter_kernel(const filter_index &F, uint32_t sigma, bool km)
@@ -167,6 +177,8 @@
     uint64_t n_seg = 0;
     uint32_t seg_bits = 0;
     bool exact_hits = false, skip_seen = false;
+    bool runs = false;
+    resolve_params R{};
 
     int lay_out()
     {
@@ -248,6 +260,28 @@
             P.dynamic = span.dynamic;
             P.hash_variant = F.hash_variant;
             H->stats.span_symbols = P.span_chunks * P.span_unit;
+            bool inline_on = false;
+            {
+                inline_gate g;
+                g.stride = F.stride;
+                g.hash_variant = F.hash_variant;
+                g.sigma = ps->sigma;
+                g.key_len = F.key_len;
+                g.threads = threads;
+                g.dense = F.dense;
+                g.packed = use_packed;
+                g.passes = ps->fidx.size();
+                g.segmented = d_seg != nullptr;
+                g.stateful = A.stateful;
+                g.overlap = Z.overlap;
+                g.myers = ps->is_myers();
+                g.exact_hits = exact_hits;
+                g.nwn = Z.nwn;
+                g.max_k = ps->max_k;
+                g.runs = runs;
+                g.band_cap_pinned = A.tune.band_cap > 0;
+                inline_on = inline_finish_applies(g);
+            }
             if (use_packed) {
                 filter_params Q = P;
                 const span_plan pspan = plan_span(stream_geometry_of(Q.lo, Q.hi, 4096).n_chunks, n_waves, 4096);
@@ -263,6 +297,14 @@
                     return SPM_E_UNSUPPORTED;
                 }
                 launch(k, dim3(grid), threads, lds, ctx->stream, Q, reinterpret_cast<const uint4 *>(A.text->d_packed));
+            } else if (const inline_kernel ik = select_inline_kernel(F, ps->sigma, km)) {
+                filter_params_inline Q{};
+                static_cast<filter_params &>(Q) = P;
+                Q.inline_finish = inline_on ? 1u : 0u;
+                Q.fin_peq32 = ps->d_peq_verify ? ps->d_peq_verify : ps->d_peq;
+                Q.fin_nw_table = ps->NW;
+                Q.fin = R;
+                launch(ik, dim3(grid), threads, lds, ctx->stream, Q);
             } else {
                 const filter_kernel k = select_filter_kernel(F, ps->sigma, km);
                 if (!k) {
@@ -308,7 +350,7 @@
         X.seg_owned = A.d_seg_owned;
     }
 
-    int launch_resolve()
+    int prepare_resolve()
     {
         if (A.d_seg_offsets) {
             d_seg = A.d_seg_offsets;
@@ -325,7 +367,6 @@
         }
         while (n_seg && (1ull << seg_bits) < n_seg + 1)
             ++seg_bits;
-        resolve_params R{};
         fill_shared(R);
         R.surv = surv;
         R.surv_cap = Z.surv_cap;
@@ -344,6 +385,11 @@
         R.exact_hits = exact_hits ? 1u : 0u;
         R.seen = skip_seen ? nullptr : seen;
         R.table_poison = ctx->d_table_poison;
+        return SPM_OK;
+    }
+
+    int launch_resolve()
+    {
         const uint64_t surv_expect = ps->cand_hint ? 2 * ps->cand_hint : Z.surv_cap;
         const uint64_t rmax = (uint64_t)ctx->n_cu * 5;
         const uint64_t per_wg = (surv_expect + 255) / 256 <= rmax ? 256 : 1024;
@@ -353,7 +399,7 @@
         return SPM_OK;
     }
 
-    int launch_bands(bool runs)
+    int launch_bands()
     {
         verify_params V{};
         fill_shared(V);
@@ -408,14 +454,15 @@
     filter_run F{A, R, ctx, A.ps, H, size_filter(*A.ps, A.tune, A.end - A.begin, (uint64_t)ctx->n_cu, H->cap, R)};
     const filter_sizes &Z = F.Z;
     SPM_TRY(F.lay_out());
-    const bool runs = !Z.overlap && !F.exact_hits && !Z.use_wave && Z.Bw <= 32 && !R.need_seen && A.tune.verify_runs != 0 &&
+    const bool runs = F.runs = !Z.overlap && !F.exact_hits && !Z.use_wave && Z.Bw <= 32 && !R.need_seen && A.tune.verify_runs != 0 &&
                       A.ps->band_hint >= (uint64_t)std::max(0, A.tune.verify_runs_min_bands);
     out = {F.seen, (uint32_t)(Z.seen_slots - 1), F.ovf, F.skip_seen || runs, Z.surv_cap, Z.band_cap};
+    SPM_TRY(F.prepare_resolve());
     SPM_HIP_CHECK(ctx, hipEventRecord(H->ev[1], ctx->stream));
     SPM_TRY(F.launch_passes());
     SPM_HIP_CHECK(ctx, hipEventRecord(H->ev[2], ctx->stream));
     SPM_TRY(F.launch_resolve());
-    SPM_TRY(F.launch_bands(runs));
+    SPM_TRY(F.launch_bands());
     SPM_HIP_CHECK(ctx, hipEventRecord(H->ev[3], ctx->stream));
     return SPM_OK;
 }
diff --git a/libspm_amd/csrc/scan_plan.hpp b/libspm_amd/csrc/scan_plan.hpp
--- a/libspm_amd/csrc/scan_plan.hpp
+++ b/libspm_amd/csrc/scan_plan.hpp
@@ -28,10 +28,12 @@
     kCntRunHeads = 11,
     kCntFanOut = 12,
     kCntStateOnly = 13,
+    kCntInline = 14,
     kCntTicket = 15,
 };
 constexpr int kCntBlock = 16;
 constexpr int kCntReadBack = 13;
+constexpr int kCntReadBackHost = 15;
 constexpr int kCntReadBackRescan = 8;
 constexpr int kCntReadBackCount = 4;
 constexpr int kLandFanOut = 13;
@@ -288,4 +290,52 @@
     return Z;
 }
 
-}
+constexpr uint32_t kInlineMaxSurvivors = 64;
+constexpr uint32_t kInlineMaxEntries = 8;
+constexpr uint32_t kInlineMaxWords = 4;
+
+struct inline_gate
+{
+    uint32_t stride = 0, hash_variant = 0, sigma = 0, key_len = 0, threads = 0;
+    bool dense = false, packed = false;
+    uint64_t passes = 0;
+    bool segmented = false, stateful = false;
+    bool overlap = false;
+    bool myers = false, exact_hits = false;
+    uint32_t nwn = 0, max_k = 0;
+    bool runs = false;
+    bool band_cap_pinned = false;
+};
+inline bool inline_finish_applies(const inline_gate &g)
+{
+    const bool kernel = !g.dense && !g.packed && g.threads == 512 && g.stride >= 4 && g.hash_variant == 2 && g.sigma == 4 && g.key_len == 16;
+    const bool scan = g.passes == 1 && !g.segmented && !g.stateful && !g.overlap && !g.runs && !g.band_cap_pinned;
+    const bool set = g.exact_hits || (g.myers && g.nwn <= kInlineMaxWords && g.max_k <= 15);
+    return kernel && scan && set;
+}
+
+SPM_HD inline bool inline_group_joins(int64_t g_lo, int64_t g_hi, int64_t d, uint32_t W)
+{
+    return d >= g_lo - (int64_t)W && d <= g_hi + (int64_t)W;
+}
+
+struct inline_range
+{
+    int64_t e_lo, e_hi, ws;
+};
+SPM_HD inline bool inline_end_range(int64_t d_lo, int64_t d_hi, int64_t m, int64_t k, int64_t own_b, int64_t own_e, int64_t hay_b,
+                                    inline_range &r)
+{
+    r.e_lo = d_lo + m - k;
+    r.e_hi = d_hi + m + k;
+    if (r.e_lo < own_b + 1)
+        r.e_lo = own_b + 1;
+    if (r.e_hi > own_e)
+        r.e_hi = own_e;
+    r.ws = r.e_lo - (m + k);
+    if (r.ws < hay_b)
+        r.ws = hay_b;
+    return r.e_lo <= r.e_hi;
+}
+
+}
diff --git a/libspm_amd/engine.py b/libspm_amd/engine.py
--- a/libspm_amd/engine.py
+++ b/libspm_amd/engine.py
@@ -236,6 +236,11 @@
         _check(capi.lib().spm_hip_hits_stats(self._h, C.byref(s)), self.ctx._h)
         return s
 
+    def inline_pairs(self) -> int:
+        n = C.c_uint64()
+        _check(capi.lib().spm_hip_hits_inline_pairs(self._h, C.byref(n)), self.ctx._h)
+        return int(n.value)
+
     def checksum(self) -> int:
         return int(capi.lib().spm_hip_hits_checksum(self._h))
 
```

After: 4120. -36.0%, worse.
